# jhuldr/BrainFM

Measured on AMD Instinct MI355X. Metric: voxels/sec whole-volume multi-task inference, 256^3 tiled, higher is better.
Workload: dtype f16x3-split (fp32-grade); 1 GPU; 256^3 volume, reference tiling win160/stride80 -> 27 tiles, UNet3D f64 x6 levels, 9 heads (69 ch), fused tail + deformed atlas + on-device stitch of 17 keys; stitched_keys=17, mfma_passes=3, submission=hipGraph replay per tile shape, parallelism=tiles sharded over 1 rank(s), gather to rank 0, tiles_in_flight_per_gpu=2

## Files before the change

brainfm_amd/_lib.py:

```python
import ctypes as C
import os

_HERE = os.path.dirname(os.path.abspath(__file__))
LIB_PATH = os.path.join(_HERE, "libbrainfm_hip.so")

ERR = {0: "BFM_OK", -1: "BFM_E_ARG", -2: "BFM_E_SHAPE", -3: "BFM_E_WORKSPACE", -4: "BFM_E_LAUNCH"}

ROLE_PLAIN, ROLE_CT, ROLE_BIAS_LOG, ROLE_SEG, ROLE_DIST, ROLE_SR, ROLE_PATHOL = range(7)
(EW_EXP, EW_AFFINE, EW_CLAMP, EW_CLAMP_MIN, EW_GAMMA, EW_SIGMOID, EW_DIV, EW_NONZERO, EW_SUB_DIV, EW_GE,
 EW_NAN_TO_NUM) = range(11)
(EW_ADD, EW_MUL, EW_MUL_EXP, EW_AXPY_CLAMP0, EW_AXPY, EW_DIV2, EW_ZERO_WHERE_ZERO) = range(7)


class BfmError(RuntimeError):
    pass


class Upsample(C.Structure):
    _fields_ = [("d", C.c_int), ("h", C.c_int), ("w", C.c_int),
                ("mapD", C.c_void_p), ("mapH", C.c_void_p), ("mapW", C.c_void_p),
                ("repD", C.c_void_p), ("repH", C.c_void_p), ("repW", C.c_void_p)]


CLASS_STATS_BLOCKS = 1024
# ... 45 lines not shown
                ("D", C.c_void_p * 6), ("G", C.c_void_p * 3), ("divV", C.c_void_p)]


class AgeParams(C.Structure):
    _fields_ = [(n, C.c_void_p) for n in ("c1w", "c1b", "c2w", "c2b", "l1w", "l1b", "l2w", "l2b", "l3w", "l3b")]


class AgeGrads(C.Structure):
    _fields_ = [(n, C.c_void_p) for n in ("c1w", "c1b", "c2w", "c2b", "l1w", "l1b", "l2w", "l2b", "l3w", "l3b")]


GATHER_MAX_JOBS = 12


VERTEX_SETS_MAX = 4


class VertexSet(C.Structure):
    _fields_ = [("V", C.c_void_p), ("n", C.c_int64)]


class GatherJob(C.Structure):
    _fields_ = [("src", C.c_void_p), ("out", C.c_void_p), ("mean", C.c_float), ("scale", C.c_float), ("pre", C.c_int),
                ("default_max", C.c_int), ("post_div", C.c_float), ("clamp", C.c_int), ("clamp_lo", C.c_float),
                ("clamp_hi", C.c_float), ("sign", C.c_float), ("want_minmax", C.c_int)]


_P = C.c_void_p
_I = C.c_int
_F = C.c_float
_L = C.c_int64
_Z = C.c_size_t
_UP = C.POINTER(Upsample)

SIGNATURES = {
    "bfm_version": (C.c_char_p, []),
    "bfm_gn_stats_workspace": (_Z, [_I, _I, _I, _I, _I, _UP]),
    "bfm_gn_stats": (_I, [_P, _I, _P, _I, _I, _I, _I, _UP, _P, _P, _I, _F, _P, _P, _P, _P, _Z, _P]),
    "bfm_pack_conv_weights_direct": (_I, [_P, _I, _I, _P, _P]),
    "bfm_pack_conv_weights_mfma_bytes": (_Z, [_I, _I]),
    "bfm_pack_conv_weights_mfma": (_I, [_P, _I, _I, _F, _P, C.POINTER(_I), _P]),
    "bfm_pack_conv_weights_mfma16_bytes": (_Z, [_I, _I]),
    "bfm_pack_conv_weights_mfma16": (_I, [_P, _I, _I, _F, _P, C.POINTER(_I), _P]),
    "bfm_conv3x3x3_direct": (_I, [_P, _I, _P, _I, _I, _I, _I, _UP, _P, _P, _P, _I, _F, _P, _P]),
    "bfm_pack_conv_weights_upfold_bytes": (C.c_size_t, [_I, _I, _I]),
    "bfm_pack_conv_weights_upfold": (_I, [_P, _I, _I, _I, _F, _I, _P, _P, _P]),
    "bfm_conv3x3x3_upfold": (_I, [_P, _I, _I, _I, _I, _P, _P, _P, _I, _P, _I, _I, _I, _P, _P]),
    "bfm_conv3x3x3_upfold_workspace": (_Z, [_I, _I, _I, _I, _I]),
    "bfm_conv3x3x3_upfold_ex": (_I, [_P, _I, _I, _I, _I, _P, _P, _P, _I, _P, _I, _I, _I, _P, _P, _Z, _P]),
    "bfm_conv3x3x3_upfold_batch_workspace": (_Z, [_I, _I, _I, _I, _I, _I]),
    "bfm_conv3x3x3_upfold_batch": (_I, [_P, _I, _I, _I, _I, _I, _P, _P, _P, _I, _P, _I, _I, _I, _P, _P, _Z, _I, _P]),
    "bfm_conv3x3x3_tap_batch_workspace": (_Z, [_I, _I, _I, _I]),
    "bfm_conv3x3x3_tap_batch": (_I, [_P, _I, _I, _I, _P, _P, _P, _I, _P, _I, _I, _I, _I, _I, _P, _Z, _I, _P]),
    "bfm_tap_sum_rows": (_I, [_I, _I]),
    "bfm_tap_sum_batch": (_I, [_P, _I, _I, _I, _I, _P, _I, _F, _I, _I, _P, _P, _P]),
    "bfm_moment_rows_bytes": (_Z, [_I, _I]),
    "bfm_conv3x3x3_mfma_rows": (_I, [_I, _I, _I, _I, _I, C.POINTER(_I)]),
    "bfm_conv3x3x3_mfma_ex": (_I, [_P, _I, _P, _I, _I, _I, _I, _UP, _P, _P, _P, _I, _P, _I, _I, _F, _I,
                                   C.POINTER(_I), _P, _P, _Z, _P, _P]),
    "bfm_conv3x3x3_mfma_batch_workspace": (_Z, [_I, _I, _I, _I, _I, _I, _I]),
    "bfm_conv3x3x3_mfma_batch": (_I, [_P, _I, _P, _I, _I, _I, _I, _I, _UP, _P, _P, _P, _I, _P, _I, _I, _F, _I,
                                      C.POINTER(_I), _P, _P, _Z, _P, _I, _P]),
    "bfm_gn_stats_batch_workspace": (_Z, [_I, _I, _I, _I, _I, _I, _UP]),
    "bfm_gn_stats_batch": (_I, [_P, _I, _P, _I, _I, _I, _I, _I, _UP, _P, _P, _I, _F, _P, _P, _P, _P, _Z, _P]),
    "bfm_gn_stats_rows_batch": (_I, [_P, _I, _I, _P, _I, _I, C.c_double, _L, _I, _P, _P, _I, _F, _P, _P, _P, _P]),
    "bfm_conv3x3x3_stem_rows": (_I, [_I, _I, _I]),
    "bfm_conv3x3x3_stem_ex": (_I, [_P, _I, _I, _I, _P, _P, _P, _P, _I, _F, _P, _P, _P]),
    "bfm_conv3x3x3_stem_mc_ex": (_I, [_P, _I, _I, _I, _I, _P, _P, _P, _P, _I, _F, _P, _P, _P]),
    "bfm_gn_stats_rows_workspace": (_Z, [_I, _I, _I, _I]),
    "bfm_gn_stats_plan": (_I, [_I, _L, _I, C.POINTER(_I), C.POINTER(_I), C.POINTER(_L), C.POINTER(_I)]),
    "bfm_gn_stats_rows_route": (_I, [_I, _I, _I, _I, _I, _I]),
    "bfm_gn_stats_rows": (_I, [_P, _I, _I, _P, _I, _I, C.c_double, _L, _P, _P, _I, _F, _P, _P, _P, _P, _Z, _P, _P]),
    "bfm_gn_stats_rows_sliced": (_I, [_P, _I, _I, _I, _I, _P, _I, _I, _I, _I, C.c_double, _L, _P, _P, _I, _F, _P, _P, _P, _P, _Z,
                                      _P, _P]),
    "bfm_gn_stats_rows_train": (_I, [_P, _I, _I, _P, _I, _I, C.c_double, _L, _P, _P, _I, _F, _P, _P, _P, _P, _P, _P, _Z, _P, _P]),
    "bfm_crop3d": (_I, [_P, _I, _I, _I, _I, _I, _I, _I, _I, _I, _P, _P]),
    "bfm_pack_conv_weights_wino4_bytes": (_Z, [_I, _I, _I]),
    "bfm_pack_conv_weights_wino4": (_I, [_P, _I, _I, _F, _I, _P, C.POINTER(_I), _P]),
    "bfm_conv3x3x3_wino4_rows": (_I, [_I, _I, _I, _I]),
    "bfm_conv3x3x3_wino4_box": (_I, [_I, _I, _I, _I, _P]),
    "bfm_conv3x3x3_wino4_masked_workspace": (_Z, [_I, _I, _I, _I]),
    "bfm_conv3x3x3_wino4_uniform_scratch": (_Z, [_I]),
    "bfm_conv3x3x3_wino4_uniform": (_I, [_P, _I, _I, _I, _I, _P, _P, _P, _I, _P, _I, _I, _F, _I, _I, _P, _P, _P, _P, _P]),
    "bfm_conv3x3x3_wino4": (_I, [_P, _I, _I, _I, _I, _P, _P, _P, _I, _P, _I, _I, _F, _I, _I, _P, _P, _P]),
    "bfm_conv3x3x3_wino4_batch": (_I, [_P, _I, _I, _I, _I, _I, _P, _P, _P, _I, _P, _I, _I, _F, _I, _I, _P, _P, _I, _P]),
    "bfm_conv3x3x3_wino_b5_rows": (_I, [_I, _I, _I, _I]),
    "bfm_conv3x3x3_wino_b5_splitk": (_I, [_I, _I, _I, _I, _I]),
    "bfm_conv3x3x3_wino_b5_workspace": (_Z, [_I, _I, _I, _I, _I, _I]),
    "bfm_conv3x3x3_wino_b5_batch": (_I, [_P, _I, _I, _I, _I, _I, _P, _P, _P, _I, _P, _I, _I, _F, _I, _I, _P, _P, _I, _P, _Z,
                                         _P]),
    "bfm_conv3x3x3_wino4_masked": (_I, [_P, _I, _I, _I, _I, _P, _P, _P, _I, _P, _I, _I, _F, _I, _I, _P, _P, _P, _Z, _P]),
    "bfm_permute_flip3d": (_I, [_P, _I, _I, _I, C.POINTER(_I), C.POINTER(_I), _P, _P]),
    "bfm_bbox_nonzero": (_I, [_P, _I, _I, _I, _F, _P, _P]),
    "bfm_mean_lastdim": (_I, [_P, _L, _I, _P, _P]),
    "bfm_pack_conv_weights_wino_bytes": (_Z, [_I, _I, _I]),
    "bfm_pack_conv_weights_wino": (_I, [_P, _I, _I, _F, _I, _P, C.POINTER(_I), _P]),
    "bfm_bspline3_prefilter_axis": (_I, [_P, _I, _I, _I, _I, _I, _F, _F, _P, _F, _F, _F, _I, _P]),
    "bfm_bspline3_resample_axis": (_I, [_P, _I, _I, _I, _I, _P, _I, _I, _P, _P]),
    "bfm_conv3x3x3_wino_rows": (_I, [_I, _I, _I, _I]),
    "bfm_conv3x3x3_wino_ex": (_I, [_P, _I, _I, _I, _I, _P, _P, _P, _I, _P, _I, _I, _F, _I, _I, _P, _P, _P]),
    "bfm_conv3x3x3_wino_box": (_I, [_I, _I, _I, _I, _P]),
    "bfm_uniform_boxes": (_I, [_P, _I, _I, _I, _I, _I, _P, _P]),
    "bfm_uniform_boxes_level": (_I, [_P, _I, _I, _I, _I, _I, _I, _P, _P]),
    "bfm_uniform_boxes_levels": (_I, [_P, _I, _I, _I, _I, C.POINTER(_I), C.POINTER(_I), _I, C.POINTER(_P), _P, _P]),
    "bfm_uniform_boxes_bytes": (_Z, [_I, _I, _I, _I]),
    "bfm_conv3x3x3_wino_uniform_scratch": (_Z, [_I]),
    "bfm_conv3x3x3_wino_uniform": (_I, [_P, _I, _I, _I, _I, _P, _P, _P, _I, _P, _I, _I, _F, _I, _I, _P, _P, _P, _P, _P]),
    "bfm_conv3x3x3_wino_pool_ok": (_I, [_I, _I, _I, _I]),
    "bfm_conv3x3x3_wino_pool": (_I, [_P, _I, _I, _I, _I, _P, _P, _P, _I, _P, _I, _I, _F, _I, _I, _P, _P, _P, _P, _P]),
    "bfm_conv3x3x3_wino_uniform_pool": (_I, [_P, _I, _I, _I, _I, _P, _P, _P, _I, _P, _I, _I, _F, _I, _I, _P, _P, _P, _P, _P, _P,
                                             _P]),
    "bfm_conv3x3x3_wino_masked_workspace": (_Z, [_I, _I, _I, _I]),
    "bfm_conv3x3x3_wino_masked": (_I, [_P, _I, _I, _I, _I, _P, _P, _P, _I, _P, _I, _I, _F, _I, _I, _P, _P, _P, _Z, _P]),
    "bfm_maxpool2_rows": (_I, [_I, _I, _I, _I]),
    "bfm_maxpool2_ex": (_I, [_P, _I, _I, _I, _I, _P, _P, _P]),
    "bfm_maxpool2_batch_rows": (_I, [_I, _I, _I, _I]),
    "bfm_maxpool2_batch": (_I, [_P, _I, _I, _I, _I, _I, _P, _P, _P]),
    "bfm_grid_push3d_linear": (_I, [_P, _I, _I, _I, _I, _I, _P, _I, _I, _I, _I, C.POINTER(_I), _I, _P, _P]),
    "bfm_grid_grad3d_linear": (_I, [_P, _I, _I, _I, _I, _I, _P, _I, _I, _I, _I, C.POINTER(_I), _I, _P, _P]),
    "bfm_grid_pull3d_spline": (_I, [_P, _I, _I, _I, _I, _I, _P, _I, _I, _I, _I, C.POINTER(_I), C.POINTER(_I), _I, _P, _P]),
    "bfm_grid_push3d_spline": (_I, [_P, _I, _I, _I, _I, _I, _P, _I, _I, _I, _I, C.POINTER(_I), C.POINTER(_I), _I, _P, _P]),
    "bfm_grid_grad3d_spline": (_I, [_P, _I, _I, _I, _I, _I, _P, _I, _I, _I, _I, C.POINTER(_I), C.POINTER(_I), _I, _P, _P]),
    "bfm_grid_pull2d_spline": (_I, [_P, _I, _I, _I, _I, _P, _I, _I, _I, C.POINTER(_I), C.POINTER(_I), _I, _P, _P]),
    "bfm_grid_push2d_spline": (_I, [_P, _I, _I, _I, _I, _P, _I, _I, _I, C.POINTER(_I), C.POINTER(_I), _I, _P, _P]),
    "bfm_grid_grad2d_spline": (_I, [_P, _I, _I, _I, _I, _P, _I, _I, _I, C.POINTER(_I), C.POINTER(_I), _I, _P, _P]),
    "bfm_grid_hess3d": (_I, [_P, _I, _I, _I, _I, _I, _P, _I, _I, _I, _I, C.POINTER(_I), C.POINTER(_I), _I, _P, _P, _P]),
    "bfm_grid_pushgrad3d": (_I, [_P, _I, _I, _I, _I, _I, _P, _I, _I, _I, _I, C.POINTER(_I), C.POINTER(_I), _I, _P, _P]),
    "bfm_grid_push_fixed_bits": (_I, [_L, C.POINTER(_I), _I, _I]),
    "bfm_grid_push_fixed_workspace": (_Z, [_I, _I, _L]),
    "bfm_grid_push3d_spline_fixed": (_I, [_P, _I, _I, _I, _I, _I, _P, _I, _I, _I, _I, C.POINTER(_I), C.POINTER(_I), _I, _P,
                                          _P, _Z, _P]),
    "bfm_grid_push2d_spline_fixed": (_I, [_P, _I, _I, _I, _I, _P, _I, _I, _I, C.POINTER(_I), C.POINTER(_I), _I, _P, _P, _Z,
                                          _P]),
    "bfm_grid_push3d_linear_fixed": (_I, [_P, _I, _I, _I, _I, _I, _P, _I, _I, _I, _I, C.POINTER(_I), _I, _P, _P, _Z, _P]),
    "bfm_grid_pushgrad3d_fixed": (_I, [_P, _I, _I, _I, _I, _I, _P, _I, _I, _I, _I, C.POINTER(_I), C.POINTER(_I), _I, _P, _P,
                                       _Z, _P]),
    "bfm_spline_axis_table_workspace": (_Z, [_I, _I, _I]),
    "bfm_spline_axis_table": (_I, [_P, _I, _I, _I, _I, _I, _I, _I, _P, _P, _P, _P, _Z, _P]),
    "bfm_spline_axis_pass": (_I, [_P, _L, _I, _I, _I, _I, _P, _P, _P, _I, _P, _P]),
    "bfm_label_pull3d": (_I, [_P, _I, _I, _I, _I, _I, _I, _P, _I, _I, _I, _I, C.POINTER(_I), C.POINTER(_I), _I, _I, _P, _P]),
    "bfm_affine_grid3d": (_I, [_P, _I, _L, _I, _I, _I, _P, _P]),
    "bfm_add_identity_grid3d": (_I, [_P, _I, _L, _I, _I, _I, _P]),
    "bfm_affine_pull_multi": (_I, [_P, _L, _I, _I, _I, _I, C.POINTER(C.c_double), C.POINTER(_I), _I, _I, _I, _P, _P]),
    "bfm_affine_pull_argmax": (_I, [_P, _I, _I, _I, _I, _P, C.POINTER(C.c_double), _I, _I, _I, _I, _P, _P, _P]),
    "bfm_affine_pull_route": (_I, [_I]),
    "bfm_gn_stats_train": (_I, [_P, _I, _P, _I, _I, _I, _I, _UP, _P, _P, _I, _F, _P, _P, _P, _P, _P, _P, _Z, _P]),
    "bfm_lrelu_bwd": (_I, [_P, _P, _L, _F, _P, _P]),
    "bfm_lrelu_bwd_ex": (_I, [_P, _P, _L, _F, _P, _P, _P]),
    "bfm_conv3x3x3_wgrad_workspace": (_Z, [_I, _I, _I, _I, _I]),
    "bfm_conv3x3x3_wgrad_plan": (_I, [_I, _I, _I, _I, _I, _I, _I, _I, _I, _I, _I, C.POINTER(C.c_int64), C.POINTER(_Z)]),
    "bfm_conv3x3x3_wgrad": (_I, [_P, _I, _P, _I, _P, _I, _I, _I, _I, _UP, _P, _P, _P, _P, _Z, _P]),
    "bfm_conv3x3x3_wgrad_ex": (_I, [_P, _I, _P, _I, _P, _I, _I, _I, _I, _UP, _P, _P, _P, _P, _I, _I, _P, _P, _Z, _P]),
    "bfm_stem_mc_bwd_workspace": (_Z, [_I, _I, _I, _I, _I]),
    "bfm_stem_mc_bwd": (_I, [_P, _I, _P, _I, _I, _I, _I, _P, _P, _P, _P, _P, _P, _P, _P, _P, _Z, _P]),
    "bfm_stem_mc_dgrad": (_I, [_P, _I, _P, _I, _I, _I, _I, _P, _P, _P, _P, _P, _P, _I, _P, _P, _P, _P, _L, _L, _P]),
    "bfm_mask_chain_bwd": (_I, [_P, _L, _P, _P, _L, _P, _L, _L, _P]),
    "bfm_gn_bwd_workspace": (_Z, [_I, _I, _I, _I]),
    "bfm_gn_bwd": (_I, [_P, _P, _I, _P, _I, _I, _I, _I, _UP, _P, _P, _P, _P, _P, _P, _I, _P, _P, _P, _P, _P, _Z, _P]),
    "bfm_maxpool2_bwd": (_I, [_P, _P, _I, _I, _I, _I, _P, _P]),
    "bfm_transpose_mirror_weights": (_I, [_P, _I, _I, _I, _P, _P]),
    "bfm_loss_workspace": (_Z, [_I]),
    "bfm_loss_l1_multi_workspace": (_Z, []),
    "bfm_loss_l1_multi": (_I, [_P, _L, _L, _I, _L, _I, _P, _P, _P, _P, _P, _P, _P, _P, _P, _P, _Z, _P]),
    "bfm_loss_grad_l1_multi": (_I, [_P, _L, _L, _I, _I, _P, _P, _P, _P, _I, _I, _I, _P, _P, _P, _Z, _P]),
    "bfm_loss_seg": (_I, [_P, _L, _L, _I, _I, _I, _P, _P, _P, _L, _F, _F, _P, _P, _P, _P, _Z, _P]),
    "bfm_loss_pathol_workspace": (_Z, []),
    "bfm_loss_pathol": (_I, [_P, _L, _L, _P, _L, _F, _F, _P, _P, _P, _P, _Z, _P]),
    "bfm_loss_reg_workspace": (_Z, [_I, _I, _I, _I]),
    "bfm_loss_reg_smooth": (_I, [_P, _L, _L, _L, _I, _I, _I, _I, _F, _P, _P, _P, _Z, _P]),
    "bfm_loss_reg_hessian": (_I, [_P, _L, _L, _L, _I, _I, _I, _I, _F, _P, _P, _P, _Z, _P]),
    "bfm_loss_contrastive_workspace": (_Z, []),
    "bfm_loss_contrastive": (_I, [_P, _P, _I, _L, _I, _F, _F, _F, _F, _F, _P, _P, _P, _P, _P, _P, _Z, _P]),
    "bfm_head_bwd_workspace": (_Z, [_I, _I, _L]),
    "bfm_head_bwd": (_I, [_P, _P, _P, _I, _I, _L, _P, _P, _P, _P, _Z, _P]),
    "bfm_tail_raw_rows": (_I, [_P, _L, C.POINTER(TailDesc), _P, _P, _L, _P]),
    "bfm_head_bwd_rows": (_I, [_P, _L, _P, _P, _I, _I, _L, _P, _P, _P, _P, _Z, _P]),
    "bfm_head_wgrad_workspace": (_Z, [_I, _I, _L]),
    "bfm_head_wgrad": (_I, [_P, _P, _I, _I, _L, _P, _P, _P, _Z, _P]),
    "bfm_head_wgrad_rows": (_I, [_P, _L, _P, _I, _I, _L, _P, _P, _P, _Z, _P]),
    "bfm_normalize_bwd": (_I, [_P, _P, _I, _L, _F, _P, _P]),
    "bfm_adamw_step": (_I, [_P, _P, _P, _P, _L, _F, _F, _F, _F, _F, _I, _F, _P]),
    "bfm_grad_sumsq": (_I, [_P, _L, _P, _P, _P, _Z, _P]),
    "bfm_grad_sumsq_multi": (_I, [_P, _I, _P, _I, _L, _P, _P, _P, _Z, _P]),
    "bfm_adamw_step_multi": (_I, [_P, _I, _P, _I, _L, _F, _F, _F, _F, _F, _P]),
    "bfm_adam_step_multi": (_I, [_P, _I, _P, _I, _L, _F, C.c_double, C.c_double, _F, _F, _P]),
    "bfm_sgd_step_multi": (_I, [_P, _I, _P, _I, _L, _F, _F, _F, _P]),
    "bfm_lars_sums_multi": (_I, [_P, _I, _P, _I, _L, _P, _P, _P, _Z, _P]),
    "bfm_lars_step_multi": (_I, [_P, _I, _P, _I, _L, _F, _F, _P]),
# ... 184 lines not shown
```

brainfm_amd/csrc/conv3d_wino.hip:

```cpp
#include "wino_shared.h"
#include <cstdlib>
#include <type_traits>

namespace {

typedef _Float16 half8 __attribute__((ext_vector_type(8)));
typedef _Float16 half4 __attribute__((ext_vector_type(4)));
typedef float floatx16 __attribute__((ext_vector_type(16)));

constexpr int KC = 16;
constexpr int NTHR = 256;
constexpr int MLD = 33;

struct WinoParams {
    const float* A;
    int CA, D, H, W;
    const float *scale, *shift, *bound;
    int G;
    const uint4* wp;
    int wexp, Cout;
    float slope;
    float* out;
    int accum;
    int TD, TH, TW, HT, PW;
// ... 399 lines not shown
#pragma unroll
                for (int r = 0; r < 8; ++r) {
                    S += ls[r * 32 + tid]; Q += lq[r * 32 + tid];
                    MN = fminf(MN, lmn[r * 32 + tid]); MX = fmaxf(MX, lmx[r * 32 + tid]);
                }
                const size_t o = (size_t)mt * p.Cout + nt * 64 + nb * 32 + tid;
                p.rsum[o] = S; p.rsq[o] = Q; p.rmn[o] = MN; p.rmx[o] = MX;
            }
        }
        if constexpr (POOL == 1) {
            if (interior) {
            const int POOL_OFF = UNI ? 6144 : 0;
            float* xs = reinterpret_cast<float*>(lds + POOL_OFF);
            __syncthreads();
#pragma unroll
            for (int k = 0; k < 8; ++k) xs[k * NTHR + tid] = pm[k];
            __syncthreads();
            const int hb = (row0 >> 1) & 1;
            const int te = tid & ~64, to = tid | 64;
            float ps = 0.f, pq = 0.f, pmn = INFINITY, pmx = -INFINITY;
            const int H2 = p.H >> 1, W2 = p.W >> 1;
            float* pb = p.pool_out + nt * 64 + nb * 32 + col +
                        (((int64_t)(z0 >> 1) * H2 + (y0 >> 1) + (row0 >> 2) + 2 * hb) * W2 + (x0 >> 1) + (row0 & 1)) * p.Cout;
            const unsigned zstep = (unsigned)(H2 * W2 * p.Cout);
            const float* xe = xs + hb * 4 * NTHR + te;
            const float* xo = xs + hb * 4 * NTHR + to;
#pragma unroll
            for (int dp = 0; dp < 4; ++dp) {
                const float mv = pool_max(pool_max(-INFINITY, xe[dp * NTHR]), xo[dp * NTHR]);
                pb[dp * zstep] = mv;
                ps += mv; pq = fmaf(mv, mv, pq); pmn = fminf(pmn, mv); pmx = fmaxf(pmx, mv);
            }
            if (p.prsum != nullptr) {
                double* ls2 = reinterpret_cast<double*>(lds + POOL_OFF + 8 * NTHR * sizeof(float));
                double* lq2 = ls2 + 256;
                float* lmn2 = reinterpret_cast<float*>(lq2 + 256);
                float* lmx2 = lmn2 + 256;
                ls2[row0 * 32 + col] = (double)ps; lq2[row0 * 32 + col] = (double)pq;
                lmn2[row0 * 32 + col] = pmn; lmx2[row0 * 32 + col] = pmx;
                __syncthreads();
                if (tid < 32) {
                    double S = 0.0, Q = 0.0;
                    float MN = INFINITY, MX = -INFINITY;
#pragma unroll
                    for (int r = 0; r < 8; ++r) {
                        S += ls2[r * 32 + tid]; Q += lq2[r * 32 + tid];
                        MN = fminf(MN, lmn2[r * 32 + tid]); MX = fmaxf(MX, lmx2[r * 32 + tid]);
                    }
                    const size_t o = (size_t)mt * p.Cout + nt * 64 + nb * 32 + tid;
                    p.prsum[o] = S; p.prsq[o] = Q; p.prmn[o] = MN; p.prmx[o] = MX;
                }
            }
            }
        }
    }
}

template <int NPASS>
__global__ void __launch_bounds__(NTHR, 2) conv_wino(const WinoParams p) { conv_wino_body<NPASS, 0>(p); }
template <int NPASS>
__global__ void __launch_bounds__(NTHR, 2) conv_wino_pool(const WinoParams p) { conv_wino_body<NPASS, 0, 1>(p); }
template <int NPASS>
__global__ void __launch_bounds__(NTHR, 2) conv_wino_rest_pool(const WinoParams p) { conv_wino_body<NPASS, 2, 1>(p); }
template <int NPASS>
__global__ void __launch_bounds__(NTHR, 2) conv_wino_uniform_pool(const WinoParams p) { conv_wino_body<NPASS, 3, 1>(p); }

template <int NPASS>
__global__ void __launch_bounds__(NTHR, 2) conv_wino_masked(const WinoParams p) { conv_wino_body<NPASS, 1>(p); }

template <int NPASS>
__global__ void __launch_bounds__(NTHR, 2) conv_wino_rest(const WinoParams p) { conv_wino_body<NPASS, 2>(p); }
template <int NPASS>
__global__ void __launch_bounds__(NTHR, 2) conv_wino_uniform(const WinoParams p) { conv_wino_body<NPASS, 3>(p); }

struct FillParams {
    float* out;
    int D, H, W, Cout, NT;
    int TD, TH, TW, nTy, nTx;
    int tw_shift, thw_shift;
    const unsigned char* flags;
    const int* first;
    const int* list;
    const int* list_n;
    double *rsum, *rsq;
    float *rmn, *rmx;
    float* pool_out;
    double *prsum, *prsq;
    float *prmn, *prmx;
};

__global__ void __launch_bounds__(NTHR) class_fill(const FillParams p) {
    const int bid = blockIdx.x;
    if (bid >= p.list_n[0] * p.NT) return;
    const int tid = threadIdx.x;
    const int mt = p.list[bid / p.NT], nt = bid % p.NT;
    const int rp = p.first[p.flags[mt] - 1];
    const int z0 = (mt / (p.nTx * p.nTy)) * p.TD, y0 = ((mt / p.nTx) % p.nTy) * p.TH, x0 = (mt % p.nTx) * p.TW;
    const int rz0 = (rp / (p.nTx * p.nTy)) * p.TD, ry0 = ((rp / p.nTx) % p.nTy) * p.TH, rx0 = (rp % p.nTx) * p.TW;
    const int c4 = tid & 15;
    {
        const size_t dbase = (((size_t)z0 * p.H + y0) * p.W + x0) * p.Cout + nt * 64 + c4 * 4;
        const size_t sbase = (((size_t)rz0 * p.H + ry0) * p.W + rx0) * p.Cout + nt * 64 + c4 * 4;
        for (int r = 0; r < 4; ++r) {
            float4 v[4];
            size_t off[4];
            bool in[4];
#pragma unroll
            for (int k = 0; k < 4; ++k) {
                const int vox = (r * 4 + k) * 16 + (tid >> 4);
                const int w = vox & (p.TW - 1), h = (vox >> p.tw_shift) & (p.TH - 1), d = vox >> p.thw_shift;
                in[k] = z0 + d < p.D && y0 + h < p.H && x0 + w < p.W;
                off[k] = (((size_t)d * p.H + h) * p.W + w) * p.Cout;
                v[k] = make_float4(0.f, 0.f, 0.f, 0.f);
                if (in[k]) v[k] = *reinterpret_cast<const float4*>(p.out + sbase + off[k]);
            }
#pragma unroll
            for (int k = 0; k < 4; ++k)
                if (in[k]) *reinterpret_cast<float4*>(p.out + dbase + off[k]) = v[k];
        }
    }
    if (p.pool_out != nullptr) {
        const int H2 = p.H >> 1, W2 = p.W >> 1;
        const size_t dbase = (((size_t)(z0 >> 1) * H2 + (y0 >> 1)) * W2 + (x0 >> 1)) * p.Cout + nt * 64 + c4 * 4;
        const size_t sbase = (((size_t)(rz0 >> 1) * H2 + (ry0 >> 1)) * W2 + (rx0 >> 1)) * p.Cout + nt * 64 + c4 * 4;
        const int vox = tid >> 4;
        const size_t off0 = (((size_t)(vox >> 3) * H2 + ((vox >> 1) & 3)) * W2 + (vox & 1)) * p.Cout;
        const size_t off1 = off0 + (size_t)2 * H2 * W2 * p.Cout;
        const float4 v0 = *reinterpret_cast<const float4*>(p.pool_out + sbase + off0);
        const float4 v1 = *reinterpret_cast<const float4*>(p.pool_out + sbase + off1);
        *reinterpret_cast<float4*>(p.pool_out + dbase + off0) = v0;
        *reinterpret_cast<float4*>(p.pool_out + dbase + off1) = v1;
    }
    if (tid < 64) {
        const size_t d = (size_t)mt * p.Cout + nt * 64 + tid, s = (size_t)rp * p.Cout + nt * 64 + tid;
        if (p.rsum != nullptr) { p.rsum[d] = p.rsum[s]; p.rsq[d] = p.rsq[s]; p.rmn[d] = p.rmn[s]; p.rmx[d] = p.rmx[s]; }
        if (p.prsum != nullptr) { p.prsum[d] = p.prsum[s]; p.prsq[d] = p.prsq[s]; p.prmn[d] = p.prmn[s]; p.prmx[d] = p.prmx[s]; }
    }
}

template <class Pred>
__device__ __forceinline__ int wino_compact(int nMt, Pred pred, int* __restrict__ list, int* sh) {
    const int tid = threadIdx.x, lane = tid & 63, wv = tid >> 6;
    if (tid == 0) sh[16] = 0;
    __syncthreads();
    for (int b0 = 0; b0 < nMt; b0 += 1024) {
        const int mt = b0 + tid;
        const bool keep = mt < nMt && pred(mt);
        const unsigned long long bal = __ballot(keep);
        const int before = __popcll(bal & ((1ull << lane) - 1ull));
        if (lane == 0) sh[wv] = __popcll(bal);
        __syncthreads();
        int off = sh[16];
        for (int w = 0; w < wv; ++w) off += sh[w];
        if (keep) list[off + before] = mt;
        __syncthreads();
        if (tid == 0) {
            int t = 0;
            for (int w = 0; w < 16; ++w) t += sh[w];
            sh[16] += t;
        }
        __syncthreads();
    }
    return sh[16];
}

__global__ void __launch_bounds__(256) wino_box_active_kernel(const float* __restrict__ img, int D, int H, int W, int TD,
                                                               int TH, int TW, int nTy, int nTx, int nMt,
                                                               unsigned char* __restrict__ act) {
    const int mt = blockIdx.x * 4 + (threadIdx.x >> 6), lane = threadIdx.x & 63;
    if (mt >= nMt) return;
    const int tx = mt % nTx, ty = (mt / nTx) % nTy, tz = mt / (nTx * nTy);
    const int z0 = tz * TD, y0 = ty * TH, x0 = tx * TW;
    const int thw = TH * TW;
    bool nz = false;
    for (int q = lane; q < TD * thw; q += 64) {
        const int d = q / thw, r = q - d * thw, h = r / TW, w = r - h * TW;
        const int gz = z0 + d, gy = y0 + h, gx = x0 + w;
        if (gz < D && gy < H && gx < W) nz = nz || img[((int64_t)gz * H + gy) * W + gx] != 0.f;
    }
    const bool any = __any(nz);
    if (lane == 0) act[mt] = any ? 1 : 0;
}

__global__ void __launch_bounds__(1024) wino_mask_list_kernel(const unsigned char* __restrict__ act, int nMt,
                                                               int* __restrict__ list, int* __restrict__ n_out) {
    __shared__ int sh[17];
    const int n = wino_compact(nMt, [&](int mt) { return act[mt] != 0; }, list, sh);
    if (threadIdx.x == 0) n_out[0] = n;
}

__global__ void __launch_bounds__(256) uniform_boxes_kernel(const float* __restrict__ img, int D, int H, int W, int TD, int TH,
                                                            int TW, int nTz, int nTy, int nTx, int L, int R,
                                                            unsigned char* __restrict__ flags) {
    const int mt = blockIdx.x;
    const int tx = mt % nTx, ty = (mt / nTx) % nTy, tz = mt / (nTx * nTy);
    const int z0 = max(((tz * TD) << L) - R, 0), y0 = max(((ty * TH) << L) - R, 0), x0 = max(((tx * TW) << L) - R, 0);
    const int z1 = min((((tz + 1) * TD) << L) + R, D), y1 = min((((ty + 1) * TH) << L) + R, H);
    const int x1 = min((((tx + 1) * TW) << L) + R, W);
    const int ed = z1 - z0, eh = y1 - y0, ew = x1 - x0;
    int bad = 0;
    const unsigned ref = __float_as_uint(img[((int64_t)z0 * H + y0) * W + x0]);
    for (int q = threadIdx.x; q < ed * eh * ew; q += 256) {
        const int w = q % ew, r = q / ew, h = r % eh, d = r / eh;
        bad |= __float_as_uint(img[((int64_t)(z0 + d) * H + (y0 + h)) * W + (x0 + w)]) != ref ? 1 : 0;
    }
    bad = __syncthreads_or(bad);
    if (threadIdx.x == 0) {
        const int cz = tz == 0 ? 0 : (tz == nTz - 1 ? 2 : 1), cy = ty == 0 ? 0 : (ty == nTy - 1 ? 2 : 1);
        const int cx = tx == 0 ? 0 : (tx == nTx - 1 ? 2 : 1);
        const int dl = (D >> L) << L, hl = (H >> L) << L, wl = (W >> L) << L;
        const bool far = (tz != nTz - 1 && ((((tz + 1) * TD) << L) + R > dl)) ||
                         (ty != nTy - 1 && ((((ty + 1) * TH) << L) + R > hl)) ||
                         (tx != nTx - 1 && ((((tx + 1) * TW) << L) + R > wl));
        flags[mt] = bad || far ? 0 : (unsigned char)(1 + 9 * cz + 3 * cy + cx);
    }
}

template <bool AGENT>
__device__ __forceinline__ void uniform_lists_body(const unsigned char* flags, int n, int* __restrict__ first,
                                                   int* __restrict__ cnt, int* __restrict__ rest, int* __restrict__ uni,
                                                   int* sh, int* fst) {
    auto flag = [&](int i) -> int {
        if constexpr (AGENT) return __hip_atomic_load(flags + i, __ATOMIC_RELAXED, __HIP_MEMORY_SCOPE_AGENT);
        else return flags[i];
    };
    if (threadIdx.x < 27) fst[threadIdx.x] = n;
    __syncthreads();
    for (int i = threadIdx.x; i < n; i += 1024) {
        const int f = flag(i);
        if (f != 0) atomicMin(&fst[f - 1], i);
    }
    __syncthreads();
    if (threadIdx.x < 27) first[threadIdx.x] = fst[threadIdx.x];
    const int n0 = wino_compact(n, [&](int mt) { const int f = flag(mt); return f == 0 || fst[f - 1] == mt; }, rest, sh);
    if (threadIdx.x == 0) cnt[0] = n0;
    __syncthreads();
    const int n1 = wino_compact(n, [&](int mt) { const int f = flag(mt); return f != 0 && fst[f - 1] != mt; }, uni, sh);
    if (threadIdx.x == 0) cnt[1] = n1;
}

__global__ void __launch_bounds__(1024) uniform_lists_kernel(const unsigned char* __restrict__ flags, int n,
                                                             int* __restrict__ first, int* __restrict__ cnt,
                                                             int* __restrict__ rest, int* __restrict__ uni) {
    __shared__ int sh[17];
    __shared__ int fst[27];
    uniform_lists_body<false>(flags, n, first, cnt, rest, uni, sh, fst);
}

constexpr int UL_MAX = 4;
constexpr int UL_LOADS = 8;
struct UniLevel {
    int TD, TH, TW, nTz, nTy, nTx, L, R;
    int n, per, wg0;
    unsigned char* flags;
    int* first;
};
struct UniLevels {
    const float* img;
    int D, H, W, nlev, nwg;
    int* ticket;
    UniLevel lv[UL_MAX];
};

__global__ void __launch_bounds__(1024) uniform_levels_kernel(const UniLevels p) {
    __shared__ int sh[17];
    __shared__ int fst[27];
    __shared__ int bad_w[16];
    __shared__ int is_last;
    const int tid = threadIdx.x, grp = tid >> 8, t = tid & 255;
    int li = 0;
    for (int i = 1; i < p.nlev; ++i)
        if ((int)blockIdx.x >= p.lv[i].wg0) li = i;
    const UniLevel& v = p.lv[li];
    const int D = p.D, H = p.H, W = p.W, L = v.L, R = v.R;
    const int box0 = ((int)blockIdx.x - v.wg0) * 4 * v.per;
    for (int r = 0; r < v.per; ++r) {
        const int mt = box0 + r * 4 + grp;
        const bool live = mt < v.n;
        int bad = 0;
        int tx = 0, ty = 0, tz = 0;
        if (live) {
            tx = mt % v.nTx; ty = (mt / v.nTx) % v.nTy; tz = mt / (v.nTx * v.nTy);
            const int z0 = max(((tz * v.TD) << L) - R, 0), y0 = max(((ty * v.TH) << L) - R, 0);
            const int x0 = max(((tx * v.TW) << L) - R, 0);
            const int z1 = min((((tz + 1) * v.TD) << L) + R, D), y1 = min((((ty + 1) * v.TH) << L) + R, H);
            const int x1 = min((((tx + 1) * v.TW) << L) + R, W);
            const int eh = y1 - y0, ew = x1 - x0, nq = (z1 - z0) * eh * ew;
            const unsigned ref = __float_as_uint(p.img[((int64_t)z0 * H + y0) * W + x0]);
            int w = t % ew, h = (t / ew) % eh, d = (t / ew) / eh;
            const int sw = 256 % ew, sh_ = (256 / ew) % eh, sd = (256 / ew) / eh;
            const float* const base = p.img + ((int64_t)z0 * H + y0) * W + x0;
            for (int qb = 0; qb < nq && !bad; qb += UL_LOADS * 256) {
                unsigned val[UL_LOADS];
#pragma unroll
                for (int k = 0; k < UL_LOADS; ++k) {
                    val[k] = ref;
                    if (qb + k * 256 + t < nq) val[k] = __float_as_uint(base[(unsigned)(d * H + h) * (unsigned)W + (unsigned)w]);
                    w += sw;
                    if (w >= ew) { w -= ew; ++h; }
                    h += sh_;
                    if (h >= eh) { h -= eh; ++d; }
                    d += sd;
                }
                int diff = 0;
#pragma unroll
                for (int k = 0; k < UL_LOADS; ++k) diff |= val[k] != ref ? 1 : 0;
                bad = __any(diff) ? 1 : 0;
            }
        }
        if ((tid & 63) == 0) bad_w[tid >> 6] = bad;
        __syncthreads();
        if (live && t == 0) {
            const int any_bad = bad_w[grp * 4] | bad_w[grp * 4 + 1] | bad_w[grp * 4 + 2] | bad_w[grp * 4 + 3];
            const int cz = tz == 0 ? 0 : (tz == v.nTz - 1 ? 2 : 1), cy = ty == 0 ? 0 : (ty == v.nTy - 1 ? 2 : 1);
            const int cx = tx == 0 ? 0 : (tx == v.nTx - 1 ? 2 : 1);
            const int dl = (D >> L) << L, hl = (H >> L) << L, wl = (W >> L) << L;
            const bool far = (tz != v.nTz - 1 && ((((tz + 1) * v.TD) << L) + R > dl)) ||
                             (ty != v.nTy - 1 && ((((ty + 1) * v.TH) << L) + R > hl)) ||
                             (tx != v.nTx - 1 && ((((tx + 1) * v.TW) << L) + R > wl));
            __hip_atomic_store(v.flags + mt, any_bad || far ? (unsigned char)0 : (unsigned char)(1 + 9 * cz + 3 * cy + cx),
                               __ATOMIC_RELAXED, __HIP_MEMORY_SCOPE_AGENT);
        }
        __syncthreads();
    }
    asm volatile("s_waitcnt vmcnt(0)" ::: "memory");
    __syncthreads();
    if (tid == 0) {
        const int got = __hip_atomic_fetch_add(p.ticket, 1, __ATOMIC_RELEASE, __HIP_MEMORY_SCOPE_AGENT);
        is_last = got == p.nwg - 1;
        if (is_last) __hip_atomic_store(p.ticket, 0, __ATOMIC_RELAXED, __HIP_MEMORY_SCOPE_AGENT);
    }
    __syncthreads();
    if (!is_last) return;
    __builtin_amdgcn_fence(__ATOMIC_ACQUIRE, "agent");
    for (int i = 0; i < p.nlev; ++i) {
        const int n = p.lv[i].n;
        int* const first = p.lv[i].first;
        uniform_lists_body<true>(p.lv[i].flags, n, first, first + 27, first + 29, first + 29 + n, sh, fst);
        __syncthreads();
    }
}

__global__ void pack_wino(const float* __restrict__ w, int Cin, int Cout, int wexp, int npl, uint4* __restrict__ out) {
    const int KCN = Cin / KC;
    const int nf = 2 * npl;
    const int64_t n = (int64_t)(Cout / 64) * 4 * KCN * 9 * nf * 64;
    const float s = ldexpf(1.0f, wexp);
    for (int64_t i = (int64_t)blockIdx.x * blockDim.x + threadIdx.x; i < n; i += (int64_t)gridDim.x * blockDim.x) {
        const int lane = (int)(i & 63);
        int64_t r = i >> 6;
        const int f = (int)(r % nf); r /= nf;
        const int t = (int)(r % 9); r /= 9;
        const int kc = (int)(r % KCN); r /= KCN;
        const int ps = (int)(r & 3); r >>= 2;
        const int ntile = (int)r;
        const int nb = f / npl, hl = f - nb * npl;
        const int co = ntile * 64 + nb * 32 + (lane & 31);
        const int ci0 = kc * KC + 8 * (lane >> 5);
        half8 v;
#pragma unroll
        for (int j = 0; j < 8; ++j) {
            const float* g = w + ((size_t)co * Cin + ci0 + j) * 27 + t * 3;
            const float g0 = g[0], g1 = g[1], g2 = g[2];
            const float u = ps == 0 ? g0 : ps == 1 ? ((g0 + g1) + g2) * 0.5f : ps == 2 ? ((g0 - g1) + g2) * 0.5f : g2;
            const float x = u * s;
            const _Float16 hh = (_Float16)x;
            v[j] = hl == 0 ? hh : (_Float16)(x - (float)hh);
        }
        out[i] = __builtin_bit_cast(uint4, v);
    }
}

constexpr int PKW_ROW = KC * 27 + 1;
__global__ void __launch_bounds__(256) pack_wino_tiled(const float* __restrict__ w, int Cin, int Cout, int wexp, int npl,
                                                       uint4* __restrict__ out) {
    extern __shared__ float pkw_lds[];
    const int KCN = Cin / KC;
    const int nf = 2 * npl;
    const int nb = blockIdx.x & 1;
    const int kc = (blockIdx.x >> 1) % KCN, ntile = (blockIdx.x >> 1) / KCN;
    const float s = ldexpf(1.0f, wexp);
    const float* src0 = w + ((int64_t)(ntile * 64 + nb * 32) * Cin + kc * KC) * 27;
    bfm_stage_rows<32, KC * 27, PKW_ROW, 256>(src0, (int64_t)Cin * 27, pkw_lds, 1.0f,
                                              ((reinterpret_cast<uintptr_t>(w) & 15) == 0) && (Cin & 3) == 0);
    __syncthreads();
    const int lane = threadIdx.x & 63, wave = threadIdx.x >> 6;
    for (int q = wave; q < 4 * 9; q += 4) {
        const int t = q % 9;
        const int ps = q / 9;
        const float* src = pkw_lds + (lane & 31) * PKW_ROW + (8 * (lane >> 5)) * 27 + t * 3;
        half8 vh, vl;
#pragma unroll
        for (int j = 0; j < 8; ++j) {
            const float g0 = src[j * 27], g1 = src[j * 27 + 1], g2 = src[j * 27 + 2];
            const float u = ps == 0 ? g0 : ps == 1 ? ((g0 + g1) + g2) * 0.5f : ps == 2 ? ((g0 - g1) + g2) * 0.5f : g2;
            const float x = u * s;
            const _Float16 hh = (_Float16)x;
            vh[j] = hh;
            vl[j] = (_Float16)(x - (float)hh);
        }
        uint4* dst = out + ((((int64_t)(ntile * 4 + ps) * KCN + kc) * 9 + t) * nf + nb * npl) * 64 + lane;
        dst[0] = __builtin_bit_cast(uint4, vh);
        if (npl == 2) dst[64] = __builtin_bit_cast(uint4, vl);
    }
}

int ilog2i(int v) { int r = 0; while ((1 << r) < v) ++r; return r; }

bool choose_box(int D, int H, int W, int npl, int& TD, int& TH, int& TW) {
    static const int opts[][3] = {{4, 4, 16}, {4, 8, 8}, {8, 4, 8}, {8, 8, 4}, {2, 4, 32}, {4, 2, 32}, {2, 8, 16},
                                  {8, 2, 16}, {16, 4, 4}, {4, 16, 4}};
    int64_t best = -1;
    for (auto& o : opts) {
        const int pw = o[2] / 2;
        const int64_t npos = (int64_t)(o[0] + 2) * (o[1] + 2) * pw;
        if (npos * 4 > 5 * NTHR) continue;
        const int64_t plane = ((npos * 16 + 255) / 256) * 256 + 16;
        if (8 * npl * plane > 80 * 1024) continue;
        int64_t cost = (int64_t)bfm_cdiv(D, o[0]) * bfm_cdiv(H, o[1]) * bfm_cdiv(W, o[2]);
        cost = cost * 1024 + npos;
        if (best < 0 || cost < best) { best = cost; TD = o[0]; TH = o[1]; TW = o[2]; }
// ... 10 lines not shown
    const MaskListBuf b{ws, (size_t)nMt};
    hipLaunchKernelGGL(wino_box_active_kernel, dim3((unsigned)bfm_cdiv(nMt, 4)), dim3(256), 0, bfm_s(stream), mask_img, D, H, W,
                       TD, TH, TW, nTy, nTx, nMt, b.act());
    hipLaunchKernelGGL(wino_mask_list_kernel, dim3(1), dim3(1024), 0, bfm_s(stream), b.act(), nMt, b.list(), b.count());
    return bfm_launch_status();
}

extern "C" size_t bfm_pack_conv_weights_wino_bytes(int Cin, int Cout, int passes) {
    if (Cin <= 0 || Cout <= 0 || Cin % KC || Cout % 64) return 0;
    const int npl = passes == 3 ? 2 : 1;
    return (size_t)(Cout / 64) * 4 * (Cin / KC) * 9 * 2 * npl * 64 * sizeof(uint4);
}

extern "C" int bfm_pack_conv_weights_wino(const float* w_oidhw, int Cin, int Cout, float wmax_abs_host, int passes,
                                          void* wpacked, int* wexp_host, bfm_stream_t stream) {
    if (!w_oidhw || !wpacked || !wexp_host || Cin <= 0 || Cout <= 0) return BFM_E_ARG;
    if (Cin % KC || Cout % 64 || (passes != 1 && passes != 3)) return BFM_E_SHAPE;
    int wexp = 0;
    if (wmax_abs_host > 0.f && wmax_abs_host < INFINITY) {
        int ex;
        (void)frexpf(2.f * wmax_abs_host, &ex);
        wexp = 14 - ex;
        wexp = wexp > 60 ? 60 : (wexp < -60 ? -60 : wexp);
    }
    *wexp_host = wexp;
    const int npl = passes == 3 ? 2 : 1;
    const int64_t nblk = (int64_t)(Cout / 64) * (Cin / KC) * 2;
    const size_t smem = (size_t)32 * PKW_ROW * sizeof(float);
    static bool attr = false;
    if (const int rc = bfm_raise_lds_limit(attr, {bfm_kernel(&pack_wino_tiled)}, (int)smem)) return rc;
    if (nblk <= 0x7fffffff) {
        hipLaunchKernelGGL(pack_wino_tiled, dim3((unsigned)nblk), dim3(256), smem, bfm_s(stream), w_oidhw, Cin, Cout, wexp, npl,
                           static_cast<uint4*>(wpacked));
    } else {
        const int64_t n = (nblk / 2) * 4 * 9 * 2 * npl * 64;
        int nb = (int)std::min<int64_t>(4096, bfm_cdiv64(n, 256));
        hipLaunchKernelGGL(pack_wino, dim3(nb), dim3(256), 0, bfm_s(stream), w_oidhw, Cin, Cout, wexp, npl,
                           static_cast<uint4*>(wpacked));
    }
    return bfm_launch_status();
}

extern "C" int bfm_conv3x3x3_wino_rows(int D, int H, int W, int passes) {
    int TD, TH, TW;
    if (D <= 0 || H <= 0 || W <= 0 || !choose_box(D, H, W, passes == 3 ? 2 : 1, TD, TH, TW)) return 0;
    return (int)bfm_box_count(D, H, W, TD, TH, TW);
}

extern "C" int bfm_conv3x3x3_wino_box(int D, int H, int W, int passes, int* box) {
    int TD, TH, TW;
    if (!box || D <= 0 || H <= 0 || W <= 0 || !choose_box(D, H, W, passes == 3 ? 2 : 1, TD, TH, TW)) return BFM_E_ARG;
    box[0] = TD; box[1] = TH; box[2] = TW;
    return BFM_OK;
}

static bool pool_ok_box(int TD, int TH, int TW, int D, int H, int W) {
    return TD == 8 && TH == 8 && TW == 4 && D % 8 == 0 && H % 8 == 0 && W % 4 == 0;
}

extern "C" int bfm_conv3x3x3_wino_pool_ok(int D, int H, int W, int passes) {
    int TD, TH, TW;
    if (D <= 0 || H <= 0 || W <= 0 || !choose_box(D, H, W, passes == 3 ? 2 : 1, TD, TH, TW)) return 0;
    return pool_ok_box(TD, TH, TW, D, H, W) ? 1 : 0;
}

extern "C" size_t bfm_uniform_boxes_bytes(int D, int H, int W, int passes) {
    int TD, TH, TW;
    if (D <= 0 || H <= 0 || W <= 0 || !choose_box(D, H, W, passes == 3 ? 2 : 1, TD, TH, TW)) return 0;
    return UniformFlagBuf::bytes((size_t)bfm_box_count(D, H, W, TD, TH, TW));
}

extern "C" int bfm_uniform_boxes_level(const float* image, int D, int H, int W, int level, int radius, int passes,
                                       unsigned char* flags, bfm_stream_t stream) {
    if (!image || !flags || D <= 0 || H <= 0 || W <= 0 || radius < 0 || radius > 64 || level < 0 || level > 4) return BFM_E_ARG;
    if (reinterpret_cast<uintptr_t>(flags) & 3) return BFM_E_ARG;
    const int d = D >> level, h = H >> level, w = W >> level;
    int TD, TH, TW;
    if (d <= 0 || h <= 0 || w <= 0 || !choose_box(d, h, w, passes == 3 ? 2 : 1, TD, TH, TW)) return BFM_E_SHAPE;
    const int nTz = bfm_cdiv(d, TD), nTy = bfm_cdiv(h, TH), nTx = bfm_cdiv(w, TW);
    const UniformFlagBuf fb{flags, (size_t)nTz * nTy * nTx};
    if ((TD << level) < radius || (TH << level) < radius || (TW << level) < radius) return BFM_E_SHAPE;
    hipLaunchKernelGGL(uniform_boxes_kernel, dim3((unsigned)fb.n), dim3(256), 0, bfm_s(stream), image, D, H, W, TD, TH, TW, nTz,
                       nTy, nTx, level, radius, flags);
    hipLaunchKernelGGL(uniform_lists_kernel, dim3(1), dim3(1024), 0, bfm_s(stream), flags, (int)fb.n, fb.first(), fb.counts(),
                       fb.rest_list(), fb.uniform_list());
    return bfm_launch_status();
}

extern "C" int bfm_uniform_boxes(const float* image, int D, int H, int W, int radius, int passes, unsigned char* flags,
                                 bfm_stream_t stream) {
    return bfm_uniform_boxes_level(image, D, H, W, 0, radius, passes, flags, stream);
}

extern "C" int bfm_uniform_boxes_levels(const float* image, int D, int H, int W, int nlevels, const int* levels,
                                        const int* radii, int passes, unsigned char* const* flags, int* ticket,
                                        bfm_stream_t stream) {
    if (!image || !levels || !radii || !flags || !ticket || D <= 0 || H <= 0 || W <= 0 || nlevels < 1 || nlevels > UL_MAX)
        return BFM_E_ARG;
    if (reinterpret_cast<uintptr_t>(ticket) & 3) return BFM_E_ARG;
    if ((int64_t)D * H * W > 0x7fffffffLL) return BFM_E_SHAPE;
    UniLevels p{};
    p.img = image; p.D = D; p.H = H; p.W = W; p.nlev = nlevels; p.ticket = ticket;
    int64_t nwg = 0;
    for (int i = 0; i < nlevels; ++i) {
        const int level = levels[i], radius = radii[i];
        if (!flags[i] || radius < 0 || radius > 64 || level < 0 || level > 4) return BFM_E_ARG;
        if (reinterpret_cast<uintptr_t>(flags[i]) & 3) return BFM_E_ARG;
        const int d = D >> level, h = H >> level, w = W >> level;
        UniLevel& v = p.lv[i];
        if (d <= 0 || h <= 0 || w <= 0 || !choose_box(d, h, w, passes == 3 ? 2 : 1, v.TD, v.TH, v.TW)) return BFM_E_SHAPE;
        if ((v.TD << level) < radius || (v.TH << level) < radius || (v.TW << level) < radius) return BFM_E_SHAPE;
        v.nTz = bfm_cdiv(d, v.TD); v.nTy = bfm_cdiv(h, v.TH); v.nTx = bfm_cdiv(w, v.TW);
        v.L = level; v.R = radius; v.flags = flags[i];
        const int64_t n = (int64_t)v.nTz * v.nTy * v.nTx;
        if (n > 0x7fffffff) return BFM_E_SHAPE;
        v.n = (int)n;
        v.first = UniformFlagBuf{flags[i], (size_t)n}.first();
        v.per = level == 0 ? 4 : 1;
        v.wg0 = (int)nwg;
        nwg += bfm_cdiv64(n, 4 * v.per);
    }
    p.nwg = (int)nwg;
    hipStream_t st = bfm_s(stream);
    hipLaunchKernelGGL(uniform_levels_kernel, dim3((unsigned)nwg), dim3(1024), 0, st, p);
    const int rc = bfm_launch_status();
    if (rc != BFM_OK) (void)hipMemsetAsync(ticket, 0, sizeof(int), st);
    return rc;
}

extern "C" size_t bfm_conv3x3x3_wino_uniform_scratch(int Cout) {
    return Cout > 0 && Cout % 64 == 0 ? (size_t)27 * (Cout / 64) * 2 * 16 * NTHR * 2 * sizeof(float) : 0;
}

extern "C" size_t bfm_conv3x3x3_wino_masked_workspace(int D, int H, int W, int passes) {
    int TD, TH, TW;
    if (D <= 0 || H <= 0 || W <= 0 || !choose_box(D, H, W, passes == 3 ? 2 : 1, TD, TH, TW)) return 0;
    return MaskListBuf::bytes((size_t)bfm_box_count(D, H, W, TD, TH, TW));
}

static int wino_launch(const WinoLaunch& a) {
    if (const int rc = bfm_wino_check(a, KC)) return rc;
    const int D = a.D, H = a.H, W = a.W, Cout = a.Cout, passes = a.passes;
    const int npl = passes == 3 ? 2 : 1;
    WinoParams p{};
    p.A = a.A; p.CA = a.CA; p.D = D; p.H = H; p.W = W;
    p.scale = a.scale; p.shift = a.shift; p.bound = a.bound; p.G = a.G;
    p.wp = static_cast<const uint4*>(a.wpacked);
    p.wexp = a.wexp; p.Cout = Cout; p.slope = a.slope; p.out = a.out; p.accum = a.flags & 1;
    p.mask_img = a.mask.img;
    p.uni_flags = a.uniform.flags;
    p.uni_acc = a.uniform.scratch;
    if (!choose_box(D, H, W, npl, p.TD, p.TH, p.TW)) return BFM_E_SHAPE;
    p.HT = p.TH + 2; p.PW = p.TW / 2;
    p.pw_shift = ilog2i(p.PW); p.thp_shift = ilog2i(p.TH * p.PW);
    const int nTz = bfm_cdiv(D, p.TD);
    p.nTy = bfm_cdiv(H, p.TH); p.nTx = bfm_cdiv(W, p.TW);
    p.nMt = nTz * p.nTy * p.nTx;
    const UniformFlagBuf fb{a.uniform.flags, (size_t)p.nMt};
    p.uni_first = fb.flags ? fb.first() : nullptr;
    p.NT = Cout / 64;
    p.KCN = a.CA / KC;
    p.npos_lds = (p.TD + 2) * p.HT * p.PW;
    p.plane_stride = ((p.npos_lds * 16 + 255) / 256) * 256 + 16;
    size_t smem = (size_t)8 * npl * p.plane_stride;
    const size_t epi = (size_t)4 * 128 * MLD * sizeof(float) + 6144;
    if (smem < epi) smem = epi;
    MomentRows rows, prows;
    if (a.moment_rows && !rows.carve(a.moment_rows, (size_t)p.nMt * Cout)) return BFM_E_ARG;
    rows.into(p);
    if (a.pool.out) {
        if (a.mask.img || !pool_ok_box(p.TD, p.TH, p.TW, D, H, W)) return BFM_E_SHAPE;
        if (reinterpret_cast<uintptr_t>(a.pool.out) & 15) return BFM_E_ARG;
        p.pool_out = a.pool.out;
        if (a.pool.rows && !prows.carve(a.pool.rows, (size_t)p.nMt * Cout)) return BFM_E_ARG;
        p.prsum = prows.rsum; p.prsq = prows.rsq; p.prmn = prows.rmn; p.prmx = prows.rmx;
    } else if (a.pool.rows) return BFM_E_ARG;
    if ((int64_t)p.nMt * p.NT > 0x7fffffff) return BFM_E_SHAPE;
    if (smem > 80 * 1024) return BFM_E_SHAPE;
    static bool attr_done = false;
    if (const int rc = bfm_raise_lds_limit(
            attr_done,
            {bfm_kernel(&conv_wino_pool<3>), bfm_kernel(&conv_wino_pool<1>), bfm_kernel(&conv_wino_rest_pool<3>),
             bfm_kernel(&conv_wino_rest_pool<1>), bfm_kernel(&conv_wino<3>), bfm_kernel(&conv_wino<1>),
             bfm_kernel(&conv_wino_masked<3>), bfm_kernel(&conv_wino_masked<1>), bfm_kernel(&conv_wino_uniform<3>),
             bfm_kernel(&conv_wino_uniform<1>), bfm_kernel(&conv_wino_rest<3>), bfm_kernel(&conv_wino_rest<1>)},
            80 * 1024))
        return rc;
    const dim3 grid((unsigned)(p.nMt * p.NT)), block(NTHR);
    hipStream_t st = bfm_s(a.stream);
    if (a.mask.img) {
        if (!a.mask.ws) return BFM_E_ARG;
        const MaskListBuf mb{a.mask.ws, (size_t)p.nMt};
        if (const int rc = bfm_wino_mask_list(a.mask.img, D, H, W, p.TD, p.TH, p.TW, p.nTy, p.nTx, p.nMt, a.mask.ws, a.stream))
            return rc;
        p.list = mb.list(); p.list_n = mb.count();
        bfm_launch_by_passes(passes, conv_wino_masked<3>, conv_wino_masked<1>, grid, block, smem, st, p);
        return bfm_launch_status();
    }
    if (fb.flags) {
        p.list = fb.rest_list(); p.list_n = fb.counts();
        if (a.pool.out) bfm_launch_by_passes(passes, conv_wino_rest_pool<3>, conv_wino_rest_pool<1>, grid, block, smem, st, p);
        else bfm_launch_by_passes(passes, conv_wino_rest<3>, conv_wino_rest<1>, grid, block, smem, st, p);
        p.list = fb.uniform_list(); p.list_n = fb.counts() + 1;
        if (!p.accum) {
            FillParams f{};
            f.out = p.out; f.D = D; f.H = H; f.W = W; f.Cout = Cout; f.NT = p.NT;
            f.TD = p.TD; f.TH = p.TH; f.TW = p.TW; f.nTy = p.nTy; f.nTx = p.nTx;
            f.tw_shift = ilog2i(p.TW); f.thw_shift = ilog2i(p.TH * p.TW);
            f.flags = fb.flags; f.first = fb.first(); f.list = p.list; f.list_n = p.list_n;
            f.rsum = p.rsum; f.rsq = p.rsq; f.rmn = p.rmn; f.rmx = p.rmx;
            f.pool_out = p.pool_out; f.prsum = p.prsum; f.prsq = p.prsq; f.prmn = p.prmn; f.prmx = p.prmx;
            hipLaunchKernelGGL(class_fill, grid, block, 0, st, f);
            return bfm_launch_status();
        }
        if (a.pool.out) bfm_launch_by_passes(passes, conv_wino_uniform_pool<3>, conv_wino_uniform_pool<1>, grid, block, 20480, st, p);
        else bfm_launch_by_passes(passes, conv_wino_uniform<3>, conv_wino_uniform<1>, grid, block, 6144, st, p);
        return bfm_launch_status();
    }
    if (a.pool.out) bfm_launch_by_passes(passes, conv_wino_pool<3>, conv_wino_pool<1>, grid, block, smem, st, p);
    else bfm_launch_by_passes(passes, conv_wino<3>, conv_wino<1>, grid, block, smem, st, p);
    return bfm_launch_status();
}

extern "C" int bfm_conv3x3x3_wino_ex(const float* A, int CA, int D, int H, int W, const float* scale,
                                     const float* shift, const float* bound, int G, const void* wpacked, int wexp,
                                     int Cout, float slope, int passes, int flags, float* out, void* moment_rows,
                                     bfm_stream_t stream) {
    return wino_launch({A, CA, D, H, W, scale, shift, bound, G, wpacked, wexp, Cout, slope, passes, flags, out, moment_rows, stream});
}

extern "C" int bfm_conv3x3x3_wino_pool(const float* A, int CA, int D, int H, int W, const float* scale, const float* shift,
                                       const float* bound, int G, const void* wpacked, int wexp, int Cout, float slope,
                                       int passes, int flags, float* out, void* moment_rows, float* pooled,
                                       void* pooled_rows, bfm_stream_t stream) {
    if (!pooled) return BFM_E_ARG;
    WinoLaunch a{A, CA, D, H, W, scale, shift, bound, G, wpacked, wexp, Cout, slope, passes, flags, out, moment_rows, stream};
    a.pool = {pooled, pooled_rows};
    return wino_launch(a);
}

extern "C" int bfm_conv3x3x3_wino_uniform(const float* A, int CA, int D, int H, int W, const float* scale,
                                          const float* shift, const float* bound, int G, const void* wpacked, int wexp,
                                          int Cout, float slope, int passes, int flags, float* out, void* moment_rows,
                                          const unsigned char* uniform_flags, void* scratch, bfm_stream_t stream) {
    if (!uniform_flags || !scratch || (flags & ~1)) return BFM_E_ARG;
    if ((reinterpret_cast<uintptr_t>(uniform_flags) & 3) || (reinterpret_cast<uintptr_t>(scratch) & 15)) return BFM_E_ARG;
    WinoLaunch a{A, CA, D, H, W, scale, shift, bound, G, wpacked, wexp, Cout, slope, passes, flags, out, moment_rows, stream};
    a.uniform = {uniform_flags, static_cast<float*>(scratch)};
    return wino_launch(a);
}

extern "C" int bfm_conv3x3x3_wino_uniform_pool(const float* A, int CA, int D, int H, int W, const float* scale,
                                               const float* shift, const float* bound, int G, const void* wpacked,
                                               int wexp, int Cout, float slope, int passes, int flags, float* out,
                                               void* moment_rows, const unsigned char* uniform_flags, void* scratch,
                                               float* pooled, void* pooled_rows, bfm_stream_t stream) {
    if (!uniform_flags || !scratch || !pooled || (flags & ~1)) return BFM_E_ARG;
    if ((reinterpret_cast<uintptr_t>(uniform_flags) & 3) || (reinterpret_cast<uintptr_t>(scratch) & 15)) return BFM_E_ARG;
    WinoLaunch a{A, CA, D, H, W, scale, shift, bound, G, wpacked, wexp, Cout, slope, passes, flags, out, moment_rows, stream};
    a.uniform = {uniform_flags, static_cast<float*>(scratch)};
    a.pool = {pooled, pooled_rows};
    return wino_launch(a);
}

extern "C" int bfm_conv3x3x3_wino_masked(const float* A, int CA, int D, int H, int W, const float* scale,
                                         const float* shift, const float* bound, int G, const void* wpacked, int wexp,
                                         int Cout, float slope, int passes, int flags, float* out,
                                         const float* mask_image, void* workspace, size_t workspace_bytes,
                                         bfm_stream_t stream) {
    if (!mask_image || (flags & ~1)) return BFM_E_ARG;
    if (!workspace || (reinterpret_cast<uintptr_t>(workspace) & 3) ||
        workspace_bytes < bfm_conv3x3x3_wino_masked_workspace(D, H, W, passes))
        return BFM_E_ARG;
    WinoLaunch a{A, CA, D, H, W, scale, shift, bound, G, wpacked, wexp, Cout, slope, passes, flags, out, nullptr, stream};
    a.mask = {mask_image, workspace};
    return wino_launch(a);
}
```

brainfm_amd/csrc/conv3d_wino4.hip:

```cpp
#include "wino_shared.h"
#include <cstdlib>
#include <type_traits>

namespace {

typedef _Float16 half8 __attribute__((ext_vector_type(8)));
typedef float floatx16 __attribute__((ext_vector_type(16)));
typedef __fp16 fp16x2_t __attribute__((ext_vector_type(2)));

constexpr int KC = 16;
constexpr int NPOS = 6;
constexpr int NTHR = 256;
constexpr int NRG = NTHR / 32;
constexpr int MLD = 33;

struct W4Params {
    const float* A;
    int CA, D, H, W;
    const float *scale, *shift, *bound;
    int G;
    const uint4* wp;
    int wexp, Cout;
    float slope;
    float* out;
    int accum;
    int TD, TH, TW, HT, QW;
    int qw_shift, thq_shift;
    int nTy, nTx, nMt, NT, KCN;
    int npos_lds, plane_stride;
    double *rsum, *rsq;
    float *rmn, *rmx;
    const int* list;
    const int* list_n;
    const unsigned char* uni_flags;
    float* uni_acc;
    int nMtS, saff;
    int64_t sA, sO;
    int dbg_sleep;
};

__device__ __forceinline__ void quad_coords(const W4Params& p, int q, int& d, int& h, int& j) {
    d = q >> p.thq_shift;
    const int rem = q & ((1 << p.thq_shift) - 1);
    h = rem >> p.qw_shift;
    j = rem & ((1 << p.qw_shift) - 1);
}

template <bool LO>
__device__ __forceinline__ void split_store4(const float (&t)[4], unsigned char* dp, int plane_stride) {
    const fp16x2_t h01 = __builtin_amdgcn_cvt_pkrtz(t[0], t[1]);
    const fp16x2_t h23 = __builtin_amdgcn_cvt_pkrtz(t[2], t[3]);
    uint2 hv;
    hv.x = __builtin_bit_cast(unsigned, h01);
    hv.y = __builtin_bit_cast(unsigned, h23);
    *reinterpret_cast<uint2*>(dp) = hv;
    if constexpr (LO) {
        const fp16x2_t l01 = __builtin_amdgcn_cvt_pkrtz(t[0] - (float)h01[0], t[1] - (float)h01[1]);
        const fp16x2_t l23 = __builtin_amdgcn_cvt_pkrtz(t[2] - (float)h23[0], t[3] - (float)h23[1]);
        uint2 lv;
        lv.x = __builtin_bit_cast(unsigned, l01);
        lv.y = __builtin_bit_cast(unsigned, l23);
        *reinterpret_cast<uint2*>(dp + plane_stride) = lv;
    }
}

template <int NPASS, int MODE, int ABL = 0>
__device__ __forceinline__ void conv_wino4_body(const W4Params& pin) {
    W4Params p = pin;
    constexpr bool LIST = MODE != 0;
    constexpr int NPL = (NPASS == 3) ? 2 : 1;
    constexpr int NF = 2 * NPL;
    extern __shared__ __attribute__((aligned(16))) unsigned char lds[];

    const int tid = threadIdx.x;
    const int lane = tid & 63;
    const int wv = __builtin_amdgcn_readfirstlane(tid >> 6);
    const int posA = wv;
    const int posB = 4 + (wv >> 1), mbB = wv & 1;
    const int l32 = lane & 31, khalf = lane >> 5;
    int item;
    {
        const int nblk = LIST ? p.list_n[0] * p.NT : p.nMt * p.NT;
        const int bid = blockIdx.x;
        if (LIST && bid >= nblk) return;
        const int q = nblk >> 3, r = nblk & 7;
        const int xcd = bid & 7, idx = bid >> 3;
        item = (xcd < r ? xcd * (q + 1) : r * (q + 1) + (xcd - r) * q) + idx;
    }
    const int mt = LIST ? p.list[item / p.NT] : item / p.NT;
    const int nt = item % p.NT;
    int mtl = mt;
    if (!LIST && p.nMtS > 0) {
        const int smp = mt / p.nMtS;
        mtl = mt - smp * p.nMtS;
        p.A += smp * p.sA;
        p.out += smp * p.sO;
        p.scale += smp * p.saff;
        p.shift += smp * p.saff;
        p.bound += smp * p.G;
    }
    const int tx = mtl % p.nTx;
    const int ty = (mtl / p.nTx) % p.nTy;
    const int tz = mtl / (p.nTx * p.nTy);
    const int z0 = tz * p.TD, y0 = ty * p.TH, x0 = tx * p.TW;

    float bmax = 0.f;
    for (int g = 0; g < p.G; ++g) bmax = fmaxf(bmax, p.bound[g]);
    int aexp = 0;
    if (bmax > 0.f && bmax < INFINITY) {
        int ex;
        (void)frexpf(bmax, &ex);
        aexp = 10 - ex;
        aexp = aexp > 60 ? 60 : (aexp < -60 ? -60 : aexp);
    }
    const float a_scale = ldexpf(1.0f, aexp);
    const float dq = ldexpf(1.0f, -(aexp + p.wexp));

    int a_off[3];
// ... 289 lines not shown
__global__ void __launch_bounds__(NTHR, 2) conv_wino4_masked(const W4Params p) { conv_wino4_body<NPASS, 1>(p); }

constexpr int DB_TD = 8, DB_TH = 8, DB_HT = 10, DB_NROW = 100;
constexpr int DB_PLANE = DB_NROW * 16;
constexpr int DB_RAWROW = 6 * 64;
constexpr int DB_RAW = DB_NROW * DB_RAWROW;
constexpr int DB_NDMA = DB_NROW / 2;
constexpr int DB_NDMA_WAVE = (DB_NDMA + 3) / 4;

template <bool LO>
__device__ __forceinline__ void split_store4_mix(const float (&t)[4], unsigned char* dp, int plane_stride) {
    const fp16x2_t h01 = __builtin_amdgcn_cvt_pkrtz(t[0], t[1]);
    const fp16x2_t h23 = __builtin_amdgcn_cvt_pkrtz(t[2], t[3]);
    uint2 hv;
    hv.x = __builtin_bit_cast(unsigned, h01);
    hv.y = __builtin_bit_cast(unsigned, h23);
    *reinterpret_cast<uint2*>(dp) = hv;
    if constexpr (LO) {
        uint2 lv;
        asm("v_fma_mixlo_f16 %0, %1, -1.0, %2 op_sel_hi:[1,0,0]" : "=v"(lv.x) : "v"(hv.x), "v"(t[0]));
        asm("v_fma_mixhi_f16 %0, %1, -1.0, %2 op_sel:[1,0,0] op_sel_hi:[1,0,0]" : "+v"(lv.x) : "v"(hv.x), "v"(t[1]));
        asm("v_fma_mixlo_f16 %0, %1, -1.0, %2 op_sel_hi:[1,0,0]" : "=v"(lv.y) : "v"(hv.y), "v"(t[2]));
        asm("v_fma_mixhi_f16 %0, %1, -1.0, %2 op_sel:[1,0,0] op_sel_hi:[1,0,0]" : "+v"(lv.y) : "v"(hv.y), "v"(t[3]));
        *reinterpret_cast<uint2*>(dp + plane_stride) = lv;
    }
}

template <int NPASS, int MODE, int ABL = 0>
__device__ __forceinline__ void conv_wino4d_body(const W4Params& pin) {
    W4Params p = pin;
    constexpr bool LIST = MODE != 0;
    constexpr bool UNI = MODE == 3;
    constexpr bool BY_FLAG = MODE == 2 || MODE == 3;
    constexpr int NPL = (NPASS == 3) ? 2 : 1;
    constexpr int NF = 2 * NPL;
    constexpr int NWF = 3 * NPL;
    constexpr int RAW_OFF = 2 * NPOS * NPL * DB_PLANE;
    extern __shared__ __attribute__((aligned(16))) unsigned char lds[];

    const int tid = threadIdx.x;
    const int lane = tid & 63;
    const int wv = __builtin_amdgcn_readfirstlane(tid >> 6);
    const int posA = wv;
    const int posB = 4 + (wv >> 1), nbB = wv & 1;
    const int l32 = lane & 31, khalf = lane >> 5;
#ifdef BFM_W4_ABLATE
    if (p.dbg_sleep > 0 && blockIdx.x < 512) {
        unsigned hwid;
        asm volatile("s_getreg_b32 %0, hwreg(HW_REG_HW_ID)" : "=s"(hwid));
        if (hwid & 1)
            for (int i = 0; i < p.dbg_sleep; ++i) __builtin_amdgcn_s_sleep(16);
    }
#endif
    int item;
    {
        const int nblk = LIST ? p.list_n[0] * p.NT : p.nMt * p.NT;
        const int bid = blockIdx.x;
        if (LIST && bid >= nblk) return;
        const int q = nblk >> 3, r = nblk & 7;
        const int xcd = bid & 7, idx = bid >> 3;
        item = (xcd < r ? xcd * (q + 1) : r * (q + 1) + (xcd - r) * q) + idx;
    }
    const int mt = LIST ? p.list[item / p.NT] : item / p.NT;
    const int nt = item % p.NT;
    int mtl = mt;
    if (!LIST && p.nMtS > 0) {
        const int smp = mt / p.nMtS;
        mtl = mt - smp * p.nMtS;
        p.A += smp * p.sA;
        p.out += smp * p.sO;
        p.scale += smp * p.saff;
        p.shift += smp * p.saff;
        p.bound += smp * p.G;
    }
    const int tx = mtl % p.nTx;
    const int ty = (mtl / p.nTx) % p.nTy;
    const int tz = mtl / (p.nTx * p.nTy);
    const int z0 = tz * DB_TD, y0 = ty * DB_TH, x0 = tx * 4;
    int cls = 0;
    if constexpr (BY_FLAG) cls = __builtin_amdgcn_readfirstlane((int)p.uni_flags[mt]);
    const bool rep = MODE == 2 && cls != 0;
    float4* const ybuf = BY_FLAG && cls ? reinterpret_cast<float4*>(p.uni_acc) + ((size_t)(cls - 1) * p.NT + nt) * (2 * 8 * NTHR) + tid
                                        : nullptr;

    float bmax = 0.f;
    for (int g = 0; g < p.G; ++g) bmax = fmaxf(bmax, p.bound[g]);
    int aexp = 0;
    if (bmax > 0.f && bmax < INFINITY) {
        int ex;
        (void)frexpf(bmax, &ex);
        aexp = 10 - ex;
        aexp = aexp > 60 ? 60 : (aexp < -60 ? -60 : aexp);
    }
    const float a_scale = ldexpf(1.0f, aexp);
    const float dq = ldexpf(1.0f, -(aexp + p.wexp));

    floatx16 acc[2][2];
    floatx16 accB[2];
    if constexpr (!UNI) {
    int a_off[4];
#pragma unroll
    for (int u = 0; u < 4; ++u) {
        const int pos = u < 2 ? posA : posB, mb = u & 1;
        const int pr = row_perm(l32);
        const int d = mb * 2 + (pr >> 4) + 4 * ((pr & 15) >> 3), h = pr & 7;
        a_off[u] = ((pos * 2 + khalf) * NPL) * DB_PLANE + (d * DB_HT + h) * 16;
    }

    const int q4 = tid & 3;
    int msk[2];
#pragma unroll
    for (int it = 0; it < 2; ++it) {
        const int r = (tid >> 2) + 64 * it;
        msk[it] = -1;
        if (r < DB_NROW) {
            const int hz = r / DB_HT, hy = r - hz * DB_HT;
            const int gz = z0 + hz - 1, gy = y0 + hy - 1;
            int m = 0;
            if (gz >= 0 && gz < p.D && gy >= 0 && gy < p.H) {
#pragma unroll
                for (int i = 0; i < 6; ++i)
                    if (x0 - 1 + i >= 0 && x0 - 1 + i < p.W) m |= 1 << i;
            }
            msk[it] = m;
        }
    }
    const bool inner = z0 >= 1 && z0 + DB_TD < p.D && y0 >= 1 && y0 + DB_TH < p.H && x0 >= 1 && x0 + 4 < p.W;
    const int st_plane = ((q4 >> 1) * NPL) * DB_PLANE + (q4 & 1) * 8;

    const int slot = lane >> 2;
    const int sb = slot >= 6 ? 1 : 0;
    int gxc = x0 + (slot - 6 * sb) - 1;
    gxc = gxc < 0 ? 0 : (gxc > p.W - 1 ? p.W - 1 : gxc);
    const int lane_el = gxc * p.CA + (lane & 3) * 4;
    const bool dma_lane = slot < 12;
    const unsigned raw_lds = (unsigned)(__UINTPTR_TYPE__)((__attribute__((address_space(3))) unsigned char*)(lds + RAW_OFF));
    const int zs = z0 > 0 ? z0 - 1 : 0;
    const float* slab = p.A + (int64_t)zs * p.H * p.W * p.CA;
    auto issue_dma = [&](int kc) __attribute__((always_inline)) {
        if constexpr ((ABL & 8) != 0) return;
        if (dma_lane) {
            int wvo = wv;
            asm volatile("" : "+s"(wvo));
#pragma unroll
            for (int n = 0; n < DB_NDMA_WAVE; ++n) {
                const int i = wvo + 4 * n;
                if (n < DB_NDMA_WAVE - 1 || i < DB_NDMA) {
                    const int hz = i / 5, hp = i - 5 * hz;
                    int gz = z0 + hz - 1;
                    gz = gz < 0 ? 0 : (gz > p.D - 1 ? p.D - 1 : gz);
                    int gy0 = y0 + 2 * hp - 1, gy1 = gy0 + 1;
                    gy0 = gy0 < 0 ? 0 : (gy0 > p.H - 1 ? p.H - 1 : gy0);
                    gy1 = gy1 > p.H - 1 ? p.H - 1 : gy1;
                    const unsigned ro0 = (unsigned)((((gz - zs) * p.H + gy0) * p.W) * p.CA);
                    const unsigned ro1 = (unsigned)((((gz - zs) * p.H + gy1) * p.W) * p.CA);
                    const unsigned vo = ((sb ? ro1 : ro0) + (unsigned)lane_el) * 4u;
                    const unsigned la = raw_lds + (unsigned)(i * (2 * DB_RAWROW));
                    asm volatile("s_mov_b32 m0, %2\n\ts_nop 0\n\tglobal_load_lds_dwordx4 %0, %1" ::"v"(vo), "s"(slab + kc * KC), "s"(la)
                                 : "memory");
                }
            }
        }
    };

#pragma unroll
    for (int u = 0; u < 2; ++u) {
// ... 142 lines not shown
    if constexpr ((ABL & 16) != 0) {
        float sm = 0.f;
#pragma unroll
        for (int u = 0; u < 2; ++u)
#pragma unroll
            for (int i = 0; i < 16; ++i) sm += acc[u][0][i] + acc[u][1][i] + accB[u][i];
        if (sm == 12345.678f) p.out[tid] = sm;
        return;
    }
    float* m = reinterpret_cast<float*>(lds);
    const int col = tid & 31, rg = tid >> 5;
    const bool interior = z0 + DB_TD <= p.D && y0 + DB_TH <= p.H && x0 + 4 <= p.W;
    int un[4];
#pragma unroll
    for (int c = 0; c < 4; ++c) un[c] = row_unperm(16 * (c >> 1) + 8 * (c & 1) + rg);
    const unsigned off_t = (unsigned)((rg * p.W) * p.Cout + col);
#pragma unroll
    for (int nb = 0; nb < 2; ++nb) {
        if constexpr (!UNI && (ABL & 256) == 0) {
        __syncthreads();
#pragma unroll
        for (int u = 0; u < 2; ++u) {
            float* mw = m + (posA * 64 + u * 32 + khalf * 4) * MLD + l32;
#pragma unroll
            for (int i = 0; i < 16; ++i)
                mw[((i >> 2) * 8 + (i & 3)) * MLD] = acc[u][nb][i];
        }
        if (nbB == nb) {
#pragma unroll
            for (int u = 0; u < 2; ++u) {
                float* mw = m + (posB * 64 + u * 32 + khalf * 4) * MLD + l32;
#pragma unroll
                for (int i = 0; i < 16; ++i)
                    mw[((i >> 2) * 8 + (i & 3)) * MLD] = accB[u][i];
            }
        }
        __syncthreads();
        } else if (nb == 1 && p.rsum != nullptr) __syncthreads();
        float fs = 0.f, fq = 0.f, fmn = INFINITY, fmx = -INFINITY;
        float* ob = p.out + nt * 64 + nb * 32 + ((int64_t)(z0 * p.H + y0) * p.W + x0) * p.Cout;
        if constexpr ((ABL & 512) != 0) ob = p.out + nt * 64 + nb * 32 + (mt & 127) * 16384;
        const float* mc = m + col;
        if (interior) {
            float prev[8][4];
            if (p.accum) {
#pragma unroll
                for (int it = 0; it < 8; ++it) {
                    const float* o = ob + (int64_t)it * p.H * p.W * p.Cout;
#pragma unroll
                    for (int k = 0; k < 4; ++k) prev[it][k] = o[off_t + (unsigned)(k * p.Cout)];
                }
            }
#pragma unroll
            for (int it = 0; it < 8; ++it) {
                float* o = ob + (int64_t)it * p.H * p.W * p.Cout;
                if constexpr ((ABL & 512) != 0) o = ob + it * 2048 - (int)off_t + (rg * 256 + col);
                float y[4];
                if constexpr (UNI) {
                    const float4 yy = ybuf[(nb * 8 + it) * NTHR];
                    y[0] = yy.x; y[1] = yy.y; y[2] = yy.z; y[3] = yy.w;
                } else {
                    const int qr = 32 * ((it & 3) >> 1) + un[2 * (it & 1) + (it >> 2)];
                    const float* mr = mc + qr * MLD;
                    float m0, m1, m2, m3, m4, m5;
                    if constexpr ((ABL & 256) != 0) {
                        m0 = acc[0][nb][it]; m1 = acc[1][nb][it]; m2 = accB[0][it]; m3 = accB[1][it];
                        m4 = acc[0][nb][it + 8]; m5 = acc[1][nb][it + 8];
                    } else {
                        m0 = mr[0 * 64 * MLD]; m1 = mr[1 * 64 * MLD]; m2 = mr[2 * 64 * MLD];
                        m3 = mr[3 * 64 * MLD]; m4 = mr[4 * 64 * MLD]; m5 = mr[5 * 64 * MLD];
                    }
                    const float s1 = m1 + m2, d1 = m1 - m2, s2 = m3 + m4, d2 = m3 - m4;
                    y[0] = ((m0 + s1) + s2) * dq;
                    y[1] = fmaf(2.f, d2, d1) * dq;
                    y[2] = fmaf(4.f, s2, s1) * dq;
                    y[3] = (fmaf(8.f, d2, d1) + m5) * dq;
                    if (MODE == 2 && rep) ybuf[(nb * 8 + it) * NTHR] = make_float4(y[0], y[1], y[2], y[3]);
                }
#pragma unroll
                for (int k = 0; k < 4; ++k) {
                    float r = y[k];
                    if (p.accum) r = r + prev[it][k];
                    r = r >= 0.f ? r : r * p.slope;
                    if constexpr ((ABL & 128) == 0) o[off_t + (unsigned)(k * p.Cout)] = r;
                    fs += r; fq = fmaf(r, r, fq); fmn = fminf(fmn, r); fmx = fmaxf(fmx, r);
                }
            }
            if constexpr ((ABL & 128) != 0) { if (fs == 12345.678f) p.out[tid] = fs + fq + fmn + fmx; }
        } else if (y0 + rg < p.H) {
#pragma unroll 2
            for (int it = 0; it < 8; ++it) {
                if (z0 + it >= p.D) break;
                float* o = ob + (int64_t)it * p.H * p.W * p.Cout;
                float y[4];
                if constexpr (UNI) {
                    const float4 yy = ybuf[(nb * 8 + it) * NTHR];
                    y[0] = yy.x; y[1] = yy.y; y[2] = yy.z; y[3] = yy.w;
                } else {
                    const int qr = 32 * ((it & 3) >> 1) + row_unperm(16 * (it & 1) + 8 * (it >> 2) + rg);
                    const float* mr = mc + qr * MLD;
                    const float m0 = mr[0 * 64 * MLD], m1 = mr[1 * 64 * MLD], m2 = mr[2 * 64 * MLD];
                    const float m3 = mr[3 * 64 * MLD], m4 = mr[4 * 64 * MLD], m5 = mr[5 * 64 * MLD];
                    const float s1 = m1 + m2, d1 = m1 - m2, s2 = m3 + m4, d2 = m3 - m4;
                    y[0] = ((m0 + s1) + s2) * dq;
                    y[1] = fmaf(2.f, d2, d1) * dq;
                    y[2] = fmaf(4.f, s2, s1) * dq;
                    y[3] = (fmaf(8.f, d2, d1) + m5) * dq;
                    if (MODE == 2 && rep) ybuf[(nb * 8 + it) * NTHR] = make_float4(y[0], y[1], y[2], y[3]);
                }
#pragma unroll
                for (int k = 0; k < 4; ++k) {
                    if (x0 + k < p.W) {
                        float r = y[k];
                        if (p.accum) r = r + o[off_t + (unsigned)(k * p.Cout)];
                        r = r >= 0.f ? r : r * p.slope;
                        o[off_t + (unsigned)(k * p.Cout)] = r;
                        fs += r; fq = fmaf(r, r, fq); fmn = fminf(fmn, r); fmx = fmaxf(fmx, r);
                    }
                }
            }
        }
        if (p.rsum != nullptr) {
            double* ls = reinterpret_cast<double*>(lds + (UNI ? (size_t)0 : (size_t)NPOS * 64 * MLD * sizeof(float)));
            double* lq = ls + NRG * 32;
            float* lmn = reinterpret_cast<float*>(lq + NRG * 32);
            float* lmx = lmn + NRG * 32;
            ls[rg * 32 + col] = (double)fs; lq[rg * 32 + col] = (double)fq;
            lmn[rg * 32 + col] = fmn; lmx[rg * 32 + col] = fmx;
            __syncthreads();
            if (tid < 32) {
                double Ssum = 0.0, Q = 0.0;
                float MN = INFINITY, MX = -INFINITY;
#pragma unroll
                for (int r = 0; r < NRG; ++r) {
                    Ssum += ls[r * 32 + tid]; Q += lq[r * 32 + tid];
                    MN = fminf(MN, lmn[r * 32 + tid]); MX = fmaxf(MX, lmx[r * 32 + tid]);
                }
                const size_t o = (size_t)mt * p.Cout + nt * 64 + nb * 32 + tid;
                p.rsum[o] = Ssum; p.rsq[o] = Q; p.rmn[o] = MN; p.rmx[o] = MX;
            }
        }
    }
}

template <int NPASS>
__global__ void __launch_bounds__(NTHR, 2) conv_wino4d(const W4Params p) { conv_wino4d_body<NPASS, 0>(p); }
template <int NPASS>
__global__ void __launch_bounds__(NTHR, 2) conv_wino4d_masked(const W4Params p) { conv_wino4d_body<NPASS, 1>(p); }
template <int NPASS>
__global__ void __launch_bounds__(NTHR, 2) conv_wino4d_rest(const W4Params p) { conv_wino4d_body<NPASS, 2>(p); }
template <int NPASS>
__global__ void __launch_bounds__(NTHR, 2) conv_wino4d_uniform(const W4Params p) { conv_wino4d_body<NPASS, 3>(p); }
#ifdef BFM_W4_ABLATE
template <int ABL>
__global__ void __launch_bounds__(NTHR, 2) conv_wino4d_abl(const W4Params p) { conv_wino4d_body<3, 0, ABL>(p); }
#endif

__global__ void pack_wino4(const float* __restrict__ w, int Cin, int Cout, int wexp, int npl, uint4* __restrict__ out) {
    const int KCN = Cin / KC;
    const int nf = 2 * npl;
    const int64_t n = (int64_t)(Cout / 64) * NPOS * KCN * 9 * nf * 64;
    const double s = ldexp(1.0, wexp);
    for (int64_t i = (int64_t)blockIdx.x * blockDim.x + threadIdx.x; i < n; i += (int64_t)gridDim.x * blockDim.x) {
        const int lane = (int)(i & 63);
        int64_t r = i >> 6;
        const int f = (int)(r % nf); r /= nf;
        const int t = (int)(r % 9); r /= 9;
        const int kc = (int)(r % KCN); r /= KCN;
        const int ps = (int)(r % NPOS); r /= NPOS;
        const int ntile = (int)r;
        const int nb = f / npl, hl = f - nb * npl;
        const int co = ntile * 64 + nb * 32 + (lane & 31);
        const int ci0 = kc * KC + 8 * (lane >> 5);
        half8 v;
#pragma unroll
        for (int j = 0; j < 8; ++j) {
            const float* g = w + ((size_t)co * Cin + ci0 + j) * 27 + t * 3;
            const double g0 = g[0], g1 = g[1], g2 = g[2];
            const double u = ps == 0 ? g0 / 4.0
                           : ps == 1 ? -((g0 + g1) + g2) / 6.0
                           : ps == 2 ? -((g0 - g1) + g2) / 6.0
                           : ps == 3 ? g0 / 24.0 + g1 / 12.0 + g2 / 6.0
                           : ps == 4 ? g0 / 24.0 - g1 / 12.0 + g2 / 6.0
                                     : g2;
            const float x = (float)(u * s);
            const _Float16 hh = (_Float16)x;
            v[j] = hl == 0 ? hh : (_Float16)(x - (float)hh);
        }
        out[i] = __builtin_bit_cast(uint4, v);
    }
}

int ilog2i(int v) { int r = 0; while ((1 << r) < v) ++r; return r; }

bool choose_box4(int D, int H, int W, int npl, int& TD, int& TH, int& TW) {
    if (!bfm_wino_choose_box(D, H, W, npl, TD, TH, TW)) return false;
    if (TW % 4 || TD * TH * (TW / 4) != 64) return false;
    const int64_t npos = (int64_t)(TD + 2) * (TH + 2) * (TW / 4);
    if (npos * 4 > 3 * NTHR) return false;
// ... 21 lines not shown
    return (size_t)(Cout / 64) * NPOS * (Cin / KC) * 9 * 2 * npl * 64 * sizeof(uint4);
}

extern "C" int bfm_pack_conv_weights_wino4(const float* w_oidhw, int Cin, int Cout, float wmax_abs_host, int passes,
                                           void* wpacked, int* wexp_host, bfm_stream_t stream) {
    if (!w_oidhw || !wpacked || !wexp_host || Cin <= 0 || Cout <= 0) return BFM_E_ARG;
    if (Cin % KC || Cout % 64 || (passes != 1 && passes != 3)) return BFM_E_SHAPE;
    int wexp = 0;
    if (wmax_abs_host > 0.f && wmax_abs_host < INFINITY) {
        int ex;
        (void)frexpf(wmax_abs_host, &ex);
        wexp = 14 - ex;
        wexp = wexp > 60 ? 60 : (wexp < -60 ? -60 : wexp);
    }
    *wexp_host = wexp;
    const int npl = passes == 3 ? 2 : 1;
    const int64_t n = (int64_t)(Cout / 64) * NPOS * (Cin / KC) * 9 * 2 * npl * 64;
    const int nb = (int)std::min<int64_t>(8192, bfm_cdiv64(n, 256));
    hipLaunchKernelGGL(pack_wino4, dim3(nb), dim3(256), 0, bfm_s(stream), w_oidhw, Cin, Cout, wexp, npl,
                       static_cast<uint4*>(wpacked));
    return bfm_launch_status();
}

extern "C" int bfm_conv3x3x3_wino4_rows(int D, int H, int W, int passes) {
    int TD, TH, TW;
    if (D <= 0 || H <= 0 || W <= 0 || !choose_box_any(D, H, W, passes == 3 ? 2 : 1, TD, TH, TW)) return 0;
    return (int)bfm_box_count(D, H, W, TD, TH, TW);
}

extern "C" int bfm_conv3x3x3_wino4_box(int D, int H, int W, int passes, int* box) {
    int TD, TH, TW;
    if (!box || D <= 0 || H <= 0 || W <= 0 || !choose_box_any(D, H, W, passes == 3 ? 2 : 1, TD, TH, TW)) return BFM_E_ARG;
    box[0] = TD; box[1] = TH; box[2] = TW;
    return BFM_OK;
}

extern "C" size_t bfm_conv3x3x3_wino4_masked_workspace(int D, int H, int W, int passes) {
    const int n = bfm_conv3x3x3_wino4_rows(D, H, W, passes);
    if (n <= 0) return 0;
    return MaskListBuf::bytes((size_t)n);
}

static int w4_launch(const WinoLaunch& a) {
    if (const int rc = bfm_wino_check(a, KC)) return rc;
    const int D = a.D, H = a.H, W = a.W, CA = a.CA, Cout = a.Cout, passes = a.passes;
    const int S = a.batch.S, affine_stride = a.batch.affine_stride;
    const int npl = passes == 3 ? 2 : 1;
    W4Params p{};
    p.A = a.A; p.CA = CA; p.D = D; p.H = H; p.W = W;
    p.scale = a.scale; p.shift = a.shift; p.bound = a.bound; p.G = a.G;
    p.wp = static_cast<const uint4*>(a.wpacked);
    p.wexp = a.wexp; p.Cout = Cout; p.slope = a.slope; p.out = a.out; p.accum = a.flags & 1;
    if (!choose_box_any(D, H, W, npl, p.TD, p.TH, p.TW)) return BFM_E_SHAPE;
    const bool dma = use_dma_kernel(D, H, W);
    if (dma && (int64_t)(DB_TD + 2) * H * W * CA >= (int64_t)1 << 30) return BFM_E_SHAPE;
    p.HT = p.TH + 2; p.QW = p.TW / 4;
    p.qw_shift = ilog2i(p.QW); p.thq_shift = ilog2i(p.TH * p.QW);
    const int nTz = bfm_cdiv(D, p.TD);
    p.nTy = bfm_cdiv(H, p.TH); p.nTx = bfm_cdiv(W, p.TW);
    p.nMt = nTz * p.nTy * p.nTx;
    if (S > 1 || affine_stride > 0) {
        if (a.mask.img || S < 1 || (affine_stride != 0 && (affine_stride < CA || (affine_stride & 3)))) return BFM_E_ARG;
        p.nMtS = p.nMt;
        p.nMt = S * p.nMtS;
        p.saff = affine_stride > 0 ? affine_stride : CA;
        p.sA = (int64_t)D * H * W * CA;
        p.sO = (int64_t)D * H * W * Cout;
    }
    p.NT = Cout / 64;
    p.KCN = CA / KC;
    p.npos_lds = (p.TD + 2) * p.HT * p.QW;
    p.plane_stride = ((p.npos_lds * 16 + 255) / 256) * 256 + 16;
    size_t smem = dma ? (size_t)2 * NPOS * npl * DB_PLANE + DB_RAW : (size_t)2 * NPOS * npl * p.plane_stride;
    const size_t epi = (size_t)NPOS * 64 * MLD * sizeof(float) + (size_t)NRG * 32 * 24;
    if (smem < epi) smem = epi;
    if (smem > (dma ? 80u : 64u) * 1024) return BFM_E_SHAPE;
    const UniformFlagBuf fb{a.uniform.flags, (size_t)p.nMt};
    if (fb.flags) {
        int bd, bh, bw;
        if (!dma || a.mask.img || S > 1 || affine_stride > 0 || !a.uniform.scratch) return BFM_E_ARG;
        if (!bfm_wino_choose_box(D, H, W, npl, bd, bh, bw) || bd != p.TD || bh != p.TH || bw != p.TW) return BFM_E_SHAPE;
        p.uni_flags = fb.flags;
        p.uni_acc = a.uniform.scratch;
    }
    if (dma) {
        static bool attr = false;
        if (const int rc = bfm_raise_lds_limit(
                attr,
                {bfm_kernel(&conv_wino4d_rest<3>), bfm_kernel(&conv_wino4d_rest<1>), bfm_kernel(&conv_wino4d<3>),
                 bfm_kernel(&conv_wino4d<1>), bfm_kernel(&conv_wino4d_masked<3>), bfm_kernel(&conv_wino4d_masked<1>)},
                80 * 1024))
            return rc;
    }
    MomentRows rows;
    if (a.moment_rows && !rows.carve(a.moment_rows, (size_t)p.nMt * Cout)) return BFM_E_ARG;
    rows.into(p);
    if ((int64_t)p.nMt * p.NT > 0x7fffffff) return BFM_E_SHAPE;
    const dim3 grid((unsigned)(p.nMt * p.NT)), block(NTHR);
    hipStream_t st = bfm_s(a.stream);
    if (a.mask.img) {
        if (!a.mask.ws) return BFM_E_ARG;
        const MaskListBuf mb{a.mask.ws, (size_t)p.nMt};
        if (const int rc = bfm_wino_mask_list(a.mask.img, D, H, W, p.TD, p.TH, p.TW, p.nTy, p.nTx, p.nMt, a.mask.ws, a.stream))
            return rc;
        p.list = mb.list(); p.list_n = mb.count();
        if (dma) bfm_launch_by_passes(passes, conv_wino4d_masked<3>, conv_wino4d_masked<1>, grid, block, smem, st, p);
        else bfm_launch_by_passes(passes, conv_wino4_masked<3>, conv_wino4_masked<1>, grid, block, smem, st, p);
        return bfm_launch_status();
    }
    if (fb.flags) {
        p.list = fb.rest_list(); p.list_n = fb.counts();
        bfm_launch_by_passes(passes, conv_wino4d_rest<3>, conv_wino4d_rest<1>, grid, block, smem, st, p);
        p.list = fb.uniform_list(); p.list_n = fb.counts() + 1;
        bfm_launch_by_passes(passes, conv_wino4d_uniform<3>, conv_wino4d_uniform<1>, grid, block, 6144, st, p);
        return bfm_launch_status();
    }
#ifdef BFM_W4_ABLATE
    if (const char* e = getenv("BFM_W4_SLEEP")) p.dbg_sleep = atoi(e);
    if (const char* e = getenv("BFM_W4_ABL")) {
        const int abl = atoi(e);
        if (dma) {
#define W4D_ATTR(N) (void)hipFuncSetAttribute(reinterpret_cast<const void*>(&conv_wino4d_abl<N>), hipFuncAttributeMaxDynamicSharedMemorySize, 80 * 1024)
            W4D_ATTR(0); W4D_ATTR(1); W4D_ATTR(2); W4D_ATTR(3); W4D_ATTR(4); W4D_ATTR(8); W4D_ATTR(12); W4D_ATTR(15); W4D_ATTR(16); W4D_ATTR(31); W4D_ATTR(64); W4D_ATTR(28); W4D_ATTR(128); W4D_ATTR(256); W4D_ATTR(384); W4D_ATTR(512);
            switch (abl) {
#define W4D_CASE(N) case N: hipLaunchKernelGGL(conv_wino4d_abl<N>, grid, dim3(NTHR), smem, st, p); return bfm_launch_status()
                W4D_CASE(0); W4D_CASE(1); W4D_CASE(2); W4D_CASE(3); W4D_CASE(4); W4D_CASE(8); W4D_CASE(12); W4D_CASE(15); W4D_CASE(16); W4D_CASE(31); W4D_CASE(64); W4D_CASE(28); W4D_CASE(128); W4D_CASE(256); W4D_CASE(384); W4D_CASE(512);
                default: return BFM_E_ARG;
            }
        }
    }
#endif
    if (dma) bfm_launch_by_passes(passes, conv_wino4d<3>, conv_wino4d<1>, grid, block, smem, st, p);
    else bfm_launch_by_passes(passes, conv_wino4<3>, conv_wino4<1>, grid, block, smem, st, p);
    return bfm_launch_status();
}

extern "C" int bfm_conv3x3x3_wino4(const float* A, int CA, int D, int H, int W, const float* scale, const float* shift,
                                   const float* bound, int G, const void* wpacked, int wexp, int Cout, float slope,
                                   int passes, int flags, float* out, void* moment_rows, bfm_stream_t stream) {
    return w4_launch({A, CA, D, H, W, scale, shift, bound, G, wpacked, wexp, Cout, slope, passes, flags, out, moment_rows, stream});
}

extern "C" int bfm_conv3x3x3_wino4_batch(const float* A, int CA, int S, int D, int H, int W, const float* scale,
                                         const float* shift, const float* bound, int G, const void* wpacked, int wexp,
                                         int Cout, float slope, int passes, int flags, float* out, void* moment_rows,
                                         int affine_stride, bfm_stream_t stream) {
    if (S < 1) return BFM_E_ARG;
    WinoLaunch a{A, CA, D, H, W, scale, shift, bound, G, wpacked, wexp, Cout, slope, passes, flags, out, moment_rows, stream};
    a.batch = {S, affine_stride > 0 ? affine_stride : CA};
    return w4_launch(a);
}

extern "C" int bfm_conv3x3x3_wino4_masked(const float* A, int CA, int D, int H, int W, const float* scale, const float* shift,
                                          const float* bound, int G, const void* wpacked, int wexp, int Cout, float slope,
                                          int passes, int flags, float* out, const float* mask_image, void* workspace,
                                          size_t workspace_bytes, bfm_stream_t stream) {
    if (!mask_image || (flags & ~1)) return BFM_E_ARG;
    if (!workspace || (reinterpret_cast<uintptr_t>(workspace) & 3) ||
        workspace_bytes < bfm_conv3x3x3_wino4_masked_workspace(D, H, W, passes))
        return BFM_E_ARG;
    WinoLaunch a{A, CA, D, H, W, scale, shift, bound, G, wpacked, wexp, Cout, slope, passes, flags, out, nullptr, stream};
    a.mask = {mask_image, workspace};
    return w4_launch(a);
}

extern "C" size_t bfm_conv3x3x3_wino4_uniform_scratch(int Cout) {
    if (Cout <= 0 || Cout % 64) return 0;
    return (size_t)27 * (Cout / 64) * 2 * 8 * NTHR * sizeof(float4);
}

extern "C" int bfm_conv3x3x3_wino4_uniform(const float* A, int CA, int D, int H, int W, const float* scale, const float* shift,
                                           const float* bound, int G, const void* wpacked, int wexp, int Cout, float slope,
                                           int passes, int flags, float* out, void* moment_rows,
                                           const unsigned char* uniform_flags, void* scratch, bfm_stream_t stream) {
    if (!uniform_flags || !scratch || (reinterpret_cast<uintptr_t>(uniform_flags) & 3) || (reinterpret_cast<uintptr_t>(scratch) & 15))
        return BFM_E_ARG;
    WinoLaunch a{A, CA, D, H, W, scale, shift, bound, G, wpacked, wexp, Cout, slope, passes, flags, out, moment_rows, stream};
    a.uniform = {uniform_flags, static_cast<float*>(scratch)};
    return w4_launch(a);
}
```

brainfm_amd/csrc/wino_shared.h:

```cpp
#pragma once
#include "conv_shared.h"

bool bfm_wino_choose_box(int D, int H, int W, int npl, int& TD, int& TH, int& TW);

static inline size_t bfm_pad4(size_t n) { return (n + 3) & ~(size_t)3; }

struct MaskListBuf {
    void* ws;
    size_t n;
    static size_t bytes(size_t n) { return bfm_pad4(n) + 4 + n * 4; }
    unsigned char* act() const { return static_cast<unsigned char*>(ws); }
    int* count() const { return reinterpret_cast<int*>(act() + bfm_pad4(n)); }
    int* list() const { return count() + 1; }
};

struct UniformFlagBuf {
    const unsigned char* flags;
    size_t n;
    static size_t bytes(size_t n) { return bfm_pad4(n) + 27 * 4 + 2 * 4 + 2 * n * 4; }
    int* first() const { return reinterpret_cast<int*>(const_cast<unsigned char*>(flags) + bfm_pad4(n)); }
    int* counts() const { return first() + 27; }
    int* rest_list() const { return counts() + 2; }
    int* uniform_list() const { return rest_list() + n; }
};

int bfm_wino_mask_list(const float* mask_img, int D, int H, int W, int TD, int TH, int TW, int nTy, int nTx, int nMt, void* ws,
                       bfm_stream_t stream);

struct WinoLaunch {
    const float* A;
    int CA, D, H, W;
    const float *scale, *shift, *bound;
    int G;
    const void* wpacked;
    int wexp, Cout;
    float slope;
    int passes, flags;
    float* out;
    void* moment_rows;
    bfm_stream_t stream;
    struct { const float* img = nullptr; void* ws = nullptr; } mask;
    struct { const unsigned char* flags = nullptr; float* scratch = nullptr; } uniform;
    struct { float* out = nullptr; void* rows = nullptr; } pool;
    struct { int S = 1, affine_stride = 0; } batch;
};

static inline int bfm_wino_check(const WinoLaunch& a, int KC) {
    if (a.flags & ~1) return BFM_E_ARG;
    if (!a.A || a.CA <= 0 || a.D <= 0 || a.H <= 0 || a.W <= 0 || !a.scale || !a.shift || !a.bound || a.G <= 0 || !a.wpacked ||
        !a.out)
        return BFM_E_ARG;
    if (a.CA % KC || a.Cout % 64 || a.Cout <= 0) return BFM_E_SHAPE;
    if (a.passes != 1 && a.passes != 3) return BFM_E_ARG;
    if ((reinterpret_cast<uintptr_t>(a.A) & 15) || (reinterpret_cast<uintptr_t>(a.scale) & 15) ||
        (reinterpret_cast<uintptr_t>(a.shift) & 15) || (reinterpret_cast<uintptr_t>(a.wpacked) & 15) ||
        (reinterpret_cast<uintptr_t>(a.out) & 15))
        return BFM_E_ARG;
    if ((int64_t)a.D * a.H * a.W * a.CA > 0x7fffffffLL) return BFM_E_SHAPE;
    return BFM_OK;
}
```

brainfm_amd/engine.py:

```python
import ctypes as C
import os
from collections import OrderedDict, namedtuple

import numpy as np
import torch

from . import _lib as L

LABELS_LEFT = [0, 1, 2, 3, 4, 7, 8, 9, 10, 14, 15, 17, 31, 34, 36, 38, 40, 42]
LABELS_FULL = [0, 11, 12, 13, 16, 31, 32, 33, 34, 35, 36, 37, 38, 39, 40, 41, 42, 43, 44, 46,
               1, 2, 3, 4, 5, 6, 7, 8, 9, 10, 14, 15, 17, 47, 49, 51, 53, 55,
               18, 19, 20, 21, 22, 23, 24, 25, 26, 27, 28, 29, 30, 48, 50, 52, 54, 56]


def features_per_level(f_maps, num_levels):
    return [f_maps * 2 ** k for k in range(num_levels)]


def nearest_index_map(n_in, n_out):
    scale = np.float32(n_in) / np.float32(n_out)
    idx = np.floor(np.arange(n_out, dtype=np.float32) * scale).astype(np.int64)
    return np.minimum(idx, n_in - 1).astype(np.int32)


# ... 301 lines not shown
                    if wm is None:
                        wm = absmax(ly.w_raw)
                    visit(dg, wm)
                elif layout == "upfold":
                    jobs.append((ly, layout, absmax(ly.w_raw[:, ly.skip.cin:])))
                elif layout == "direct":
                    jobs.append((ly, layout, None))
                else:
                    if wm is None:
                        wm = absmax(ly.w_raw)
                    jobs.append((ly, layout, wm))
            ly.used = set()
            ly.wpacked, ly.kind = None, None
            if ly.skip is not None:
                ly.skip.w_raw.copy_(ly.w_raw[:, :ly.skip.cin])
                visit(ly.skip)

        for pair in (self.enc + self.dec if backbone else []) + [hidden]:
            for ly in pair:
                visit(ly)
        host = slots[:nslot[0]].cpu().tolist() if nslot[0] else []
        for ly, layout, m in jobs:
            wmax = host[m] if m is not None else None
            if layout == "upfold":
                self._make_upfold_pack(ly, ly.skip.cin, ly.cin - ly.skip.cin, wmax)
            else:
                self._make_pack(ly, layout, wmax)

    def _upsample_desc(self, lo, hi):
        key = (tuple(lo), tuple(hi))
        if key not in self._up_cache:
            maps = [nearest_index_map(lo[a], hi[a]) for a in range(3)]
            reps = [np.bincount(maps[a], minlength=lo[a]).astype(np.int32) for a in range(3)]
            dev = [torch.from_numpy(m).to(self.device) for m in maps + reps]
            up = L.Upsample(lo[0], lo[1], lo[2], *[t.data_ptr() for t in dev])
            self._up_cache[key] = (up, dev)
        return self._up_cache[key][0]

    def _tap_table(self, lo, hi):
        key = (tuple(lo), tuple(hi))
        if self._tap_cache is None:
            self._tap_cache = {}
        if key not in self._tap_cache:
            self._tap_cache[key] = torch.from_numpy(tap_row_table(key[0], key[1])).to(self.device)
        return self._tap_cache[key]

    def _workspace(self, nbytes):
        nbytes = max(int(nbytes), 256)
        if self._ws_lanes is None:
            self._ws_lanes, self._ws_retired = {}, []
        ws = self._ws_lanes.get(self.lane)
        if ws is None or ws.numel() < nbytes:
            if ws is not None:
                self._ws_retired.append(ws)
            ws = self._ws_lanes[self.lane] = torch.empty(int(nbytes * 1.25) + 1024, dtype=torch.uint8, device=self.device)
        return ws

    def _uf_ticket(self):
        t = self._uf_tickets
        if self.lane not in t:
            t[self.lane] = torch.zeros(1, dtype=torch.int32, device=self.device)
        return t[self.lane]

    def _gn_ticket(self):
        t = self._gn_tickets
        if self.lane not in t:
            t[self.lane] = torch.zeros(16, dtype=torch.int32, device=self.device)
        return t[self.lane]

    def _plan(self, cin, cout, dims, two_src=False, accum=False):
        key = (cin, cout, tuple(dims), bool(two_src), bool(accum))
        if key not in self._plan_cache:
            cfg = (C.c_int * 8)()
            L.check(self.lib.bfm_conv3x3x3_mfma_plan(cin, cout, dims[0], dims[1], dims[2], cfg), "mfma_plan")
            if two_src and cfg[6] in (3, 4):
                cfg[6] = 0
            if cfg[6] == 5:
                cfg[6] = 0
            self._plan_cache[key] = cfg
        return self._plan_cache[key]

    def _autotune(self, ly, key, launch, vers=None):
        cfg = self._plan_cache[key]
        if key in self._tuned or os.environ.get("BFM_CONV_VER") or os.environ.get("BFM_CONV_TUNE", "1") == "0":
            return cfg
        gkey = (torch.cuda.current_device(), getattr(self, "passes", None), key)
        if gkey not in _TUNE_CHOICES:
            saved = _tune_lookup(gkey[0], gkey[1], key)
            if saved is not None and not (key[3] and saved in (3, 4)) and (vers is None or saved in vers):
                _TUNE_CHOICES[gkey] = int(saved)
        if gkey in _TUNE_CHOICES and (vers is None or _TUNE_CHOICES[gkey] in vers or (_TUNE_CHOICES[gkey] == 4 and 3 in vers)):
            c = _TUNE_CHOICES[gkey]
            if vers is None or c in vers:
                cfg[6] = c
                self._tuned.add(key)
                return cfg
            narrowed = (C.c_int * 8)(*list(cfg))
            narrowed[6] = 3
            return narrowed
        best, best_ms = cfg[6], None
        single = (0, 1, 2, 3, 4) if os.environ.get("BFM_CONV_TUNE", "1") == "retune" else (0, 1, 2, 3)
        if hasattr(self, "enc") and self._needs_f23(ly):
            single = (0, 1, 2, 3)
        for ver in (vers if vers is not None else ((0, 1, 2) if key[3] else single)):
            if ver == 4 and 4 not in single and cfg[6] != 4:
                continue
            trial = (C.c_int * 8)(*list(cfg))
            trial[6] = ver
            try:
                self._pack(ly, True, ver)
                launch(trial)
                ms = None
                for _ in range(2):
                    ev = [torch.cuda.Event(enable_timing=True) for _ in range(2)]
                    ev[0].record()
                    launch(trial)
                    launch(trial)
                    launch(trial)
                    ev[1].record()
                    ev[1].synchronize()
                    t = ev[0].elapsed_time(ev[1])
                    ms = t if ms is None else min(ms, t)
            except L.BfmError:
                continue
            if ver == 4:
                ms = ms / 0.97
            if ver == 5:
                ms = ms / 0.97
            if best_ms is None or ms < best_ms:
                best, best_ms = ver, ms
        cfg[6] = best
        self._tuned.add(key)
        _TUNE_CHOICES[gkey] = best
        _tune_store(gkey[0], gkey[1], key, best)
        return cfg

    def conv_choices(self):
        dev, ps = torch.cuda.current_device(), getattr(self, "passes", None)
        return {k[2]: v for k, v in _TUNE_CHOICES.items() if k[0] == dev and k[1] == ps}

    def adopt_conv_choices(self, table):
        dev, ps = torch.cuda.current_device(), getattr(self, "passes", None)
        changed = False
        for key, ver in table.items():
            _TUNE_CHOICES[(dev, ps, key)] = ver
            if key in self._tuned and self._plan_cache[key][6] != ver:
                self._plan_cache[key][6] = ver
                changed = True
        return changed

    def _gn_stats(self, ly, A, ca, B, cb, dims, lo_dims, upp, scale, shift, bound, ws_min):
        D, H, W = dims
        st = L.stream_ptr()
        ra = getattr(A, "_bfm_rows", None) if self.fuse_stats else None
        rb = getattr(B, "_bfm_rows", None) if (self.fuse_stats and B is not None) else None
        if self.tape is not None and ((ra is not None and len(ra) > 2) or (rb is not None and len(rb) > 2)):
            ra = rb = None
        exact2 = B is None or tuple(dims) == tuple(2 * v for v in lo_dims)
        mean = rstd = None
        if self.tape is not None:
            mean = torch.empty(ly.groups, dtype=torch.float32, device=self.device)
            rstd = torch.empty(ly.groups, dtype=torch.float32, device=self.device)
            self._last_moments = (mean, rstd)
        if ra is not None and (B is None or (rb is not None and exact2)):
            need = self.lib.bfm_gn_stats_rows_workspace(ra[1], ca, rb[1] if rb is not None else 0, cb)
            ws = self._workspace(max(need, ws_min))
            if (len(ra) > 2 or (rb is not None and len(rb) > 2)) and self.tape is None:
                ta, fa = (ra[2], ra[3]) if len(ra) > 2 else (ra[1], 0)
                tb, fb = ((rb[2], rb[3]) if len(rb) > 2 else (rb[1], 0)) if rb is not None else (0, 0)
                L.check(self.lib.bfm_gn_stats_rows_sliced(L.ptr(ra[0]), ta, fa, ra[1], ca,
                                                          L.ptr(rb[0]) if rb is not None else None, tb, fb,
                                                          rb[1] if rb is not None else 0, cb, 8.0, D * H * W, L.ptr(ly.gamma),
                                                          L.ptr(ly.beta), ly.groups, self.eps, L.ptr(scale), L.ptr(shift),
                                                          L.ptr(bound), L.ptr(ws), ws.numel(),
                                                          L.ptr(self._gn_ticket()) if self.gn_one_launch else None, st),
                        "gn_stats_rows(slice) " + ly.name)
                return ws
            L.check(self.lib.bfm_gn_stats_rows_train(L.ptr(ra[0]), ra[1], ca, L.ptr(rb[0]) if rb is not None else None,
                                                     rb[1] if rb is not None else 0, cb, 8.0, D * H * W, L.ptr(ly.gamma),
                                                     L.ptr(ly.beta), ly.groups, self.eps, L.ptr(scale), L.ptr(shift),
                                                     L.ptr(bound), L.ptr(mean), L.ptr(rstd), L.ptr(ws), ws.numel(),
                                                     L.ptr(self._gn_ticket()) if self.gn_one_launch else None, st),
                    "gn_stats_rows " + ly.name)
            return ws
        wsb = self.lib.bfm_gn_stats_workspace(ca, cb, D, H, W, upp)
        ws = self._workspace(max(wsb, ws_min))
        L.check(self.lib.bfm_gn_stats_train(L.ptr(A), ca, L.ptr(B), cb, D, H, W, upp, L.ptr(ly.gamma), L.ptr(ly.beta),
                                            ly.groups, self.eps, L.ptr(scale), L.ptr(shift), L.ptr(bound), L.ptr(mean),
                                            L.ptr(rstd), L.ptr(ws), ws.numel(), st), "gn_stats " + ly.name)
        return ws

    def _record(self, ly, A, B, dims, lo_dims, scale, shift, bound, out):
        if self.tape is not None:
            mean, rstd = self._last_moments
            self.tape.append(dict(ly=ly, A=A, B=B, dims=tuple(dims), lo_dims=tuple(lo_dims) if lo_dims is not None else None,
                                  scale=scale, shift=shift, bound=bound, mean=mean, rstd=rstd, out=out))

    def _conv_launch(self, ly, A, ca, B, cb, dims, upp, scale, shift, bound, groups, cfg, out, ws, rows=None, slope=None,
                     mask_img=None, uni_flags=None, pool=None):
        D, H, W = dims
        st = L.stream_ptr()
        slope = self.slope if slope is None else float(slope)
        self._pack(ly, True, cfg[6])
        v = self._variant(cfg[6])
        if mask_img is not None:
            if v.masked is None or cb or rows is not None:
                raise L.BfmError("a masked launch is a one-source Winograd kernel without moment rows")
            nws = v.masked_workspace(D, H, W, self.passes)
            mws = torch.empty(nws, dtype=torch.uint8, device=self.device)
            L.check(v.masked(L.ptr(A), ca, D, H, W, L.ptr(scale), L.ptr(shift), L.ptr(bound), groups, L.ptr(ly.wpacked),
                             ly.wexp, ly.cout, slope, self.passes, cfg[7] & 1, L.ptr(out), L.ptr(mask_img), L.ptr(mws), nws,
                             st), "conv_wino(masked) " + ly.name)
            return
        if pool is not None:
            if cfg[6] != 3 or cb or mask_img is not None:
                raise L.BfmError("the fused pooling is the one-source F(2,3) kernel's")
            pooled, prow = pool
            if uni_flags is not None:
                scratch = torch.empty(self.lib.bfm_conv3x3x3_wino_uniform_scratch(ly.cout), dtype=torch.uint8,
                                      device=self.device)
                L.check(self.lib.bfm_conv3x3x3_wino_uniform_pool(
                    L.ptr(A), ca, D, H, W, L.ptr(scale), L.ptr(shift), L.ptr(bound), groups, L.ptr(ly.wpacked), ly.wexp,
                    ly.cout, slope, self.passes, cfg[7] & 1, L.ptr(out), L.ptr(rows[0]) if rows is not None else None,
                    L.ptr(uni_flags), L.ptr(scratch), L.ptr(pooled), L.ptr(prow[0]) if prow is not None else None, st),
                        "conv_wino(uniform, pool) " + ly.name)
            else:
                L.check(self.lib.bfm_conv3x3x3_wino_pool(
                    L.ptr(A), ca, D, H, W, L.ptr(scale), L.ptr(shift), L.ptr(bound), groups, L.ptr(ly.wpacked), ly.wexp,
                    ly.cout, slope, self.passes, cfg[7] & 1, L.ptr(out), L.ptr(rows[0]) if rows is not None else None,
                    L.ptr(pooled), L.ptr(prow[0]) if prow is not None else None, st), "conv_wino(pool) " + ly.name)
            return
        if uni_flags is not None and cfg[6] == 4 and not self._same_boxes(dims):
            uni_flags = None
        if uni_flags is not None and v.uniform is not None and not cb:
            scratch = torch.empty(v.uniform_scratch(ly.cout), dtype=torch.uint8, device=self.device)
            L.check(v.uniform(L.ptr(A), ca, D, H, W, L.ptr(scale), L.ptr(shift), L.ptr(bound), groups, L.ptr(ly.wpacked),
                              ly.wexp, ly.cout, slope, self.passes, cfg[7] & 1, L.ptr(out),
                              L.ptr(rows[0]) if rows is not None else None, L.ptr(uni_flags), L.ptr(scratch), st),
                    "conv_wino(uniform) " + ly.name)
            return
        if v.dense is not None:
            if cb:
                raise L.BfmError("the Winograd variant takes one source" if cfg[6] == 3 else
                                 "the Winograd variants take one source")
            L.check(v.dense(L.ptr(A), ca, D, H, W, L.ptr(scale), L.ptr(shift), L.ptr(bound), groups, L.ptr(ly.wpacked),
                            ly.wexp, ly.cout, slope, self.passes, cfg[7] & 1, L.ptr(out),
                            L.ptr(rows[0]) if rows is not None else None, st), "conv_%s %s" % (v.layout, ly.name))
            return
        L.check(self.lib.bfm_conv3x3x3_mfma_ex(L.ptr(A), ca, L.ptr(B) if cb else None, cb, D, H, W, upp if cb else None,
                                               L.ptr(scale), L.ptr(shift), L.ptr(bound), groups, L.ptr(ly.wpacked),
                                               ly.wexp, ly.cout, slope, self.passes, cfg, L.ptr(out), L.ptr(ws),
                                               ws.numel(), L.ptr(rows[0]) if rows is not None else None, st),
                "conv_mfma " + ly.name)

    def _needs_f23(self, ly):
        if self._f23_ids is None:
            self._f23_ids = {id(self.enc[i][j]) for i, j in ((0, 1), (1, 0), (1, 1)) if i < len(self.enc)}
        return id(ly) in self._f23_ids

    def _same_boxes(self, dims):
        if self._same_box_cache is None:
            self._same_box_cache = {}
        cache, key = self._same_box_cache, tuple(dims)
        if key not in cache:
            b3, b4 = (C.c_int * 3)(), (C.c_int * 3)()
            ok = (self._variant(3).box(dims[0], dims[1], dims[2], self.passes, b3) == 0 and
                  self._variant(4).box(dims[0], dims[1], dims[2], self.passes, b4) == 0)
            cache[key] = ok and list(b3) == list(b4)
        return cache[key]

    def _f23_cfg(self, ly, cfg):
        if cfg[6] == 4 and ((self.tape is not None and not TRAIN_F43) or self._needs_f23(ly)):
            cfg = (C.c_int * 8)(*list(cfg))
            cfg[6] = 3
        return cfg

    def _rows_for(self, cin, cout, dims, cfg, S=1):
        v = self._variant(cfg[6])
        if v.rows is not None:
            return self._rows_buf(cout, S, v.rows, dims[0], dims[1], dims[2], self.passes)
        return self._rows_buf(cout, S, self.lib.bfm_conv3x3x3_mfma_rows, cin, cout, dims[0], dims[1], dims[2], cfg)

    def _rows_buf(self, cout, S, rows_fn, *args):
        if not self.fuse_stats:
            return None
        n = rows_fn(*args)
        if n <= 0:
            return None
        return (torch.empty(self.lib.bfm_moment_rows_bytes(S * n, cout), dtype=torch.uint8, device=self.device), n)

    @staticmethod
    def _tag(ly):
        return ly.name.replace("backbone.", "").replace(".basic_module.SingleConv", ".")

    def _bracket(self, launch, record):
        if self.prof is None:
            launch()
            return
        reps = max(1, int(self.prof_reps))
        ev = (torch.cuda.Event(enable_timing=True), torch.cuda.Event(enable_timing=True))
        ev[0].record()
        for _ in range(reps):
            launch()
        ev[1].record()
        flops, nbytes, tag, cin, cout, dims, cfg = record()
        self.prof.append((ev[0], ev[1], flops, nbytes, reps, (tag, cin, cout, tuple(dims), tuple(cfg))))

    def single_conv(self, ly, A, dims, B=None, lo_dims=None, mask_img=None, uni_flags=None, pool=False):
        D, H, W = dims
        ca = A.shape[-1]
        cb = 0 if B is None else B.shape[-1]
        assert ca + cb == ly.cin, (ly.name, ca, cb, ly.cin)
        st = L.stream_ptr()
        up = self._upsample_desc(lo_dims, dims) if B is not None else None
        upp = C.byref(up) if up is not None else None
        scale = torch.empty(ly.cin, dtype=torch.float32, device=self.device)
        shift = torch.empty(ly.cin, dtype=torch.float32, device=self.device)
        bound = torch.empty(ly.groups, dtype=torch.float32, device=self.device)
        mfma = self._mfma_ok(ly, ca, cb)
        if (mfma and B is not None and self.use_upfold and tuple(dims) == tuple(2 * v for v in lo_dims)
                and lo_dims[0] * lo_dims[1] * lo_dims[2] >= self.upfold_min):
            return self._single_conv_upfold(ly, A, dims, B, lo_dims, upp, scale, shift, bound, uni_flags=uni_flags)
        cfg = None
        wsc = 0
        if mfma:
            cfg = self._plan(ly.cin, ly.cout, dims, B is not None)
            wsc = self.lib.bfm_conv3x3x3_mfma_workspace(ly.cin, ly.cout, D, H, W, cfg[5])
        ws = self._gn_stats(ly, A, ca, B, cb, dims, lo_dims, upp, scale, shift, bound, wsc)
        out = torch.empty((D, H, W, ly.cout), dtype=torch.float32, device=self.device)
        if mfma:
            def _launch(c):
                self._conv_launch(ly, A, ca, B, cb, dims, upp, scale, shift, bound, ly.groups, c, out, ws)
            cfg = self._f23_cfg(ly, self._autotune(ly, (ly.cin, ly.cout, tuple(dims), B is not None, False), _launch))
        self._pack(ly, mfma, cfg[6] if cfg is not None else 0)
        if mfma:
            if mask_img is not None and not (cfg[6] in (3, 4) and B is None and self.tape is None):
                mask_img = None
            if uni_flags is not None and not (cfg[6] in (3, 4) and B is None and mask_img is None):
                uni_flags = None
            rows = self._rows_for(ly.cin, ly.cout, dims, cfg) if mask_img is None else None
            pl = None
            if (pool and cfg[6] == 3 and B is None and mask_img is None and self.tape is None and self.fuse_pool
                    and min(dims) >= 2 and self.lib.bfm_conv3x3x3_wino_pool_ok(D, H, W, self.passes)):
                pooled = torch.empty((D // 2, H // 2, W // 2, ly.cout), dtype=torch.float32, device=self.device)
                pl = (pooled, self._rows_buf(ly.cout, 1, self.lib.bfm_conv3x3x3_wino_rows, D, H, W, self.passes))

            def _record():
                nv = D * H * W
                if mask_img is not None:
                    nv = self.masked_voxels(mask_img, dims, cfg[6])
                if uni_flags is not None:
                    nv = self.uniform_voxels(uni_flags, dims)
                lo = 0 if B is None else lo_dims[0] * lo_dims[1] * lo_dims[2]
                return (2.0 * 27 * ly.cin * ly.cout * nv, 4.0 * (nv * ca + lo * cb + nv * ly.cout + 27 * ly.cin * ly.cout),
                        self._tag(ly) + ("[masked]" if mask_img is not None else "[uniform]" if uni_flags is not None else ""),
                        ly.cin, ly.cout, dims, cfg)
            self._bracket(lambda: self._conv_launch(ly, A, ca, B, cb, dims, upp, scale, shift, bound, ly.groups, cfg, out, ws,
                                                    rows, mask_img=mask_img, uni_flags=uni_flags, pool=pl), _record)
            if rows is not None:
                out._bfm_rows = rows
            if pl is not None:
                if pl[1] is not None:
                    pl[0]._bfm_rows = pl[1]
                out._bfm_pooled = (pl[0], (D // 2, H // 2, W // 2))
        elif ca == 1 and cb == 0 and ly.cout in (32, 64) and not self.force_direct:
            rows = self._rows_buf(ly.cout, 1, self.lib.bfm_conv3x3x3_stem_rows, D, H, W)
            L.check(self.lib.bfm_conv3x3x3_stem_ex(L.ptr(A), D, H, W, L.ptr(scale), L.ptr(shift), L.ptr(bound),
                                                   L.ptr(ly.wpacked), ly.cout, self.slope, L.ptr(out),
                                                   L.ptr(rows[0]) if rows is not None else None, st),
                    "conv_stem " + ly.name)
            if rows is not None:
                out._bfm_rows = rows
        elif ca in (2, 3, 4) and cb == 0 and ly.cout in (32, 64) and not self.force_direct and self.stem_mc:
            rows = self._rows_buf(ly.cout, 1, self.lib.bfm_conv3x3x3_stem_rows, D, H, W)
            L.check(self.lib.bfm_conv3x3x3_stem_mc_ex(L.ptr(A), ca, D, H, W, L.ptr(scale), L.ptr(shift), L.ptr(bound),
                                                      L.ptr(ly.wpacked), ly.cout, self.slope, L.ptr(out),
                                                      L.ptr(rows[0]) if rows is not None else None, st),
                    "conv_stem_mc " + ly.name)
            ly.kind = "stem_mc"
            if rows is not None:
                out._bfm_rows = rows
        else:
            L.check(self.lib.bfm_conv3x3x3_direct(L.ptr(A), ca, L.ptr(B), cb, D, H, W, upp, L.ptr(scale),
                                                  L.ptr(shift), L.ptr(ly.wpacked), ly.cout, self.slope, L.ptr(out),
                                                  st), "conv_direct " + ly.name)
        self._record(ly, A, B, dims, lo_dims, scale, shift, bound, out)
        return out

    def masked_voxels(self, mask_img, dims, ver=None):
        D, H, W = dims
        if ver is None:
            ly = self.dec[-1][-1] if self.dec else self.enc[0][-1]
            key = (ly.cin, ly.cout, tuple(dims), False, False)
            ver = _TUNE_CHOICES.get((torch.cuda.current_device(), getattr(self, "passes", None), key))
            if ver is None:
                ver = _tune_lookup(torch.cuda.current_device(), getattr(self, "passes", None), key)
            if os.environ.get("BFM_CONV_VER"):
                ver = int(os.environ["BFM_CONV_VER"])
        box = (C.c_int * 3)()
        L.check(self._variant(4 if ver == 4 else 3).box(D, H, W, self.passes, box), "wino_box")
        td, th, tw = box[0], box[1], box[2]
        m = (mask_img.reshape(D, H, W) != 0)
        m = torch.nn.functional.pad(m, (0, -W % tw, 0, -H % th, 0, -D % td))
        m = m.reshape(m.shape[0] // td, td, m.shape[1] // th, th, m.shape[2] // tw, tw)
        act = m.any(dim=5, keepdim=True).any(dim=3, keepdim=True).any(dim=1, keepdim=True).expand_as(m)
        act = act.reshape(m.shape[0] * td, m.shape[2] * th, m.shape[4] * tw)[:D, :H, :W]
        n = int(act.sum().item())
        self.last_mask_fraction = n / float(D * H * W)
        return n

    def uniform_flags(self, x_cl, dims, radius, level=0):
        if not self.uniform_skip or x_cl is None or x_cl.shape[-1] != 1 or self.tape is not None:
            return None
        radius = max([radius] + [r for k, r in self.UNIFORM_RADIUS.items() if k[1] == level])
        ckey = (x_cl.data_ptr(), tuple(dims), int(level), int(radius), torch.cuda.current_stream(self.device).cuda_stream)
        if self._uf_cache is None:
            self._uf_cache = {}
        cache = self._uf_cache
        if ckey in cache:
            return cache[ckey]
        D, H, W = dims
        lv = sorted({k[1] for k in self.UNIFORM_RADIUS})
        rad = [max(r for k, r in self.UNIFORM_RADIUS.items() if k[1] == l) for l in lv]
        if level in lv and radius == rad[lv.index(level)]:
            nb = [self.lib.bfm_uniform_boxes_bytes(D >> l, H >> l, W >> l, self.passes) for l in lv]
            if min(nb) > 0:
                bufs = [torch.empty(n, dtype=torch.uint8, device=self.device) for n in nb]
                rc = self.lib.bfm_uniform_boxes_levels(L.ptr(x_cl), D, H, W, len(lv), (C.c_int * len(lv))(*lv),
                                                       (C.c_int * len(lv))(*rad), self.passes,
                                                       (C.c_void_p * len(lv))(*[b.data_ptr() for b in bufs]),
                                                       L.ptr(self._uf_ticket()), L.stream_ptr())
                if rc != -2:
                    L.check(rc, "uniform_boxes_levels")
                    for l, r, b in zip(lv, rad, bufs):
                        cache[ckey[:2] + (int(l), int(r)) + ckey[4:]] = b
                    return cache[ckey]
        n = self.lib.bfm_uniform_boxes_bytes(D >> level, H >> level, W >> level, self.passes)
        if n <= 0:
            return None
        flags = torch.empty(n, dtype=torch.uint8, device=self.device)
        rc = self.lib.bfm_uniform_boxes_level(L.ptr(x_cl), D, H, W, int(level), int(radius), self.passes, L.ptr(flags),
                                              L.stream_ptr())
        if rc == -2:
            flags = None
        else:
            L.check(rc, "uniform_boxes")
        cache[ckey] = flags
        return flags

    UNIFORM_RADIUS = {("enc", 0, 1): 2, ("dec", 0): 3}
    if os.environ.get("BFM_UNIFORM_LEVELS", "1") != "0":
        UNIFORM_RADIUS.update({("enc", 1, 0): 4, ("enc", 1, 1): 6, ("dec", 1): 8})

    def uniform_voxels(self, flags, dims):
        nb = self.lib.bfm_conv3x3x3_wino_rows(dims[0], dims[1], dims[2], self.passes)
        f = flags[:nb]
        k = int((f != 0).sum().item())
        reused = k - int(torch.unique(f[f != 0]).numel())
        self.last_uniform_fraction = k / float(nb)
        return int(round(dims[0] * dims[1] * dims[2] * (1.0 - max(reused, 0) / float(nb))))

    def _skip_layer(self, ly, ca):
        if ly.skip is None:
            sk = _Layer()
            sk.name, sk.cin, sk.cout, sk.groups = ly.name + "[skip]", ca, ly.cout, ly.groups
            sk.gamma, sk.beta = ly.gamma, ly.beta
            sk.w_raw = ly.w_raw[:, :ca].contiguous()
            sk.kind, sk.wpacked, sk.wexp, sk.packs, sk.skip = None, None, 0, {}, None
            ly.skip = sk
        return ly.skip

    def _single_conv_upfold(self, ly, A, dims, B, lo_dims, upp, scale, shift, bound, uni_flags=None):
        D, H, W = dims
        ca, cb = A.shape[-1], B.shape[-1]
        st = L.stream_ptr()
        sk = self._skip_layer(ly, ca)
        key = (ca, ly.cout, tuple(dims), False, True)
        cfg0 = self._plan(ca, ly.cout, dims, False, True)
        cfg0[7] = 1
        wsc = self.lib.bfm_conv3x3x3_mfma_workspace(ca, ly.cout, D, H, W, cfg0[5])
        wsu = self.lib.bfm_conv3x3x3_upfold_workspace(cb, lo_dims[0], lo_dims[1], lo_dims[2], ly.cout)
        ws = self._gn_stats(ly, A, ca, B, cb, dims, lo_dims, upp, scale, shift, bound, max(wsc, wsu))
        out = torch.empty((D, H, W, ly.cout), dtype=torch.float32, device=self.device)
        if "upfold" not in ly.packs:
            self._make_upfold_pack(ly, ca, cb)
        ly.touch("upfold")
        wup, wexp_up = ly.packs["upfold"]

        def _launch_skip(c):
            self._conv_launch(sk, A, ca, None, 0, dims, None, scale, shift, bound, ly.groups, c, out, ws)
        cfg = self._f23_cfg(ly, self._autotune(sk, key, _launch_skip))
        self._pack(sk, True, cfg[6])
        sc_b, sh_b = scale[ca:], shift[ca:]
        nv = D * H * W
        lo = lo_dims[0] * lo_dims[1] * lo_dims[2]

        def _launch_up():
            L.check(self.lib.bfm_conv3x3x3_upfold_ex(L.ptr(B), cb, lo_dims[0], lo_dims[1], lo_dims[2], L.ptr(sc_b),
                                                     L.ptr(sh_b), L.ptr(bound), ly.groups, L.ptr(wup), wexp_up, ly.cout,
                                                     self.passes, L.ptr(out), L.ptr(ws) if wsu else None, ws.numel(), st),
                    "conv_upfold " + ly.name)
        self._bracket(_launch_up, lambda: (2.0 * 27 * cb * ly.cout * nv, 4.0 * (lo * cb + nv * ly.cout),
                                           self._tag(ly) + "up", cb, ly.cout, dims, (0,) * 8))
        rows = self._rows_for(ca, ly.cout, dims, cfg)
        if uni_flags is not None and (cfg[6] not in (3, 4) or (cfg[6] == 4 and not self._same_boxes(dims))):
            uni_flags = None
        self._bracket(lambda: self._conv_launch(sk, A, ca, None, 0, dims, None, scale, shift, bound, ly.groups, cfg, out, ws,
                                                rows, uni_flags=uni_flags),
                      lambda: (2.0 * 27 * ca * ly.cout * (nv if uni_flags is None else self.uniform_voxels(uni_flags, dims)),
                               4.0 * (nv * ca + 2 * nv * ly.cout),
                               self._tag(ly) + ("sk[uniform]" if uni_flags is not None else "sk"), ca, ly.cout, dims, cfg))
        if rows is not None:
            out._bfm_rows = rows
        self._record(ly, A, B, dims, lo_dims, scale, shift, bound, out)
        return out

    def maxpool(self, X, dims, out=None):
        D, H, W = dims
        c = X.shape[-1]
        fused = getattr(X, "_bfm_pooled", None)
        if fused is not None and out is None and self.tape is None:
            return fused
        if out is None:
            out = torch.empty((D // 2, H // 2, W // 2, c), dtype=torch.float32, device=self.device)
        rows = self._rows_buf(c, 1, self.lib.bfm_maxpool2_rows, c, D, H, W)
        L.check(self.lib.bfm_maxpool2_ex(L.ptr(X), c, D, H, W, L.ptr(out), L.ptr(rows[0]) if rows is not None else None,
                                         L.stream_ptr()), "maxpool2")
        if rows is not None:
            out._bfm_rows = rows
        if self.tape is not None:
            self.tape.append(dict(pool_in=X, pool_dims=tuple(dims)))
        return out, (D // 2, H // 2, W // 2)

    def maxpool_batch(self, X, dims):
        S, (D, H, W), c = X.shape[0], dims, X.shape[-1]
        out = torch.empty((S, D // 2, H // 2, W // 2, c), dtype=torch.float32, device=self.device)
        if c % 4 or self.tape is not None:
            for s_ in range(S):
                self.maxpool(X[s_], dims, out=out[s_])
            return out
        rows = self._rows_buf(c, S, self.lib.bfm_maxpool2_batch_rows, c, D, H, W)
        L.check(self.lib.bfm_maxpool2_batch(L.ptr(X), c, S, D, H, W, L.ptr(out), L.ptr(rows[0]) if rows is not None else None,
                                            L.stream_ptr()), "maxpool2_batch")
        if rows is not None:
            out._bfm_rows = rows
        return out

    deep_from = int(os.environ.get("BFM_DEEP_FROM", "3"))
    deep_batch = os.environ.get("BFM_DEEP_BATCH", "1") != "0"
    DEEP_VERS = (0, 2)
    DEEP_VERS_1SRC = (0, 2, 4)
    use_wino_b5 = os.environ.get("BFM_WINO_B5", "1")
    deep_upfold = os.environ.get("BFM_DEEP_UPFOLD", "1") != "0"
    deep_upfold_min = int(os.environ.get("BFM_DEEP_UPFOLD_MIN", "100"))
    use_tap = os.environ.get("BFM_TAP", "1") != "0"
    tap_max = 64
    mask_skip = os.environ.get("BFM_MASK_SKIP", "1") != "0"
    uniform_skip = os.environ.get("BFM_UNIFORM_SKIP", "1") != "0"

    deep_vox = int(os.environ.get("BFM_DEEP_VOX", "16000"))

    def _region_ok(self, df):
        if self._deep_ok is None:
            self._deep_ok = {}
        cache = self._deep_ok
        if df not in cache:
            ndeep = len(self.enc) - 1 - df
            layers = [ly for pair in self.enc[df:] + self.dec[:ndeep] for ly in pair]
            cache[df] = all(ly.cin % 16 == 0 and ly.cout % 64 == 0 for ly in layers) and \
                self.enc[df - 1][1].cout % 16 == 0
        return cache[df]

    def has_deep_region(self):
        if not (self.deep_batch and self.tape is None and not self.force_direct and len(self.fm) > self.deep_from >= 1):
            return False
        return self._region_ok(self.deep_from)

    def region_start(self, dims):
        df = self.deep_from
        while df - 1 >= 2:
            lv = [v >> (df - 1) for v in dims]
            if min(lv) < 1 or lv[0] * lv[1] * lv[2] > self.deep_vox or not self._region_ok(df - 1):
                break
            df -= 1
        return df

    def _batch_stats(self, ly, A, ca, B, cb, S, dims, lo_dims, upp, scale, shift, bound):
        D, H, W = dims
        st = L.stream_ptr()
        ra = getattr(A, "_bfm_rows", None) if self.fuse_stats else None
        rb = getattr(B, "_bfm_rows", None) if (self.fuse_stats and B is not None) else None
        exact2 = B is None or tuple(dims) == tuple(2 * v for v in lo_dims)
        if ra is not None and ra[1] <= 128 and (B is None or (rb is not None and exact2 and rb[1] <= 128)):
            L.check(self.lib.bfm_gn_stats_rows_batch(L.ptr(ra[0]), ra[1], ca, L.ptr(rb[0]) if rb is not None else None,
                                                     rb[1] if rb is not None else 0, cb, 8.0, D * H * W, S,
                                                     L.ptr(ly.gamma), L.ptr(ly.beta), ly.groups, self.eps, L.ptr(scale),
                                                     L.ptr(shift), L.ptr(bound), st), "gn_stats_rows_batch " + ly.name)
            return
        need = self.lib.bfm_gn_stats_batch_workspace(ca, cb, S, D, H, W, upp)
        ws = self._workspace(need)
        L.check(self.lib.bfm_gn_stats_batch(L.ptr(A), ca, L.ptr(B), cb, S, D, H, W, upp, L.ptr(ly.gamma), L.ptr(ly.beta),
                                            ly.groups, self.eps, L.ptr(scale), L.ptr(shift), L.ptr(bound), L.ptr(ws),
                                            ws.numel(), st), "gn_stats_batch " + ly.name)

    def batch_conv(self, ly, A, dims, B=None, lo_dims=None, stats=None):
        S = A.shape[0]
        D, H, W = dims
        ca = A.shape[-1]
        cb = 0 if B is None else B.shape[-1]
        assert ca + cb == ly.cin, (ly.name, ca, cb, ly.cin)
        if not self._mfma_ok(ly, ca, cb):
            raise L.BfmError("%s: the batched levels need channel counts that are multiples of 16 / 64" % ly.name)
        up = self._upsample_desc(lo_dims, dims) if B is not None else None
        upp = C.byref(up) if up is not None else None
        if stats is None:
            scale = torch.empty((S, ly.cin), dtype=torch.float32, device=self.device)
            shift = torch.empty((S, ly.cin), dtype=torch.float32, device=self.device)
            bound = torch.empty((S, ly.groups), dtype=torch.float32, device=self.device)
            self._batch_stats(ly, A, ca, B, cb, S, dims, lo_dims, upp, scale, shift, bound)
        else:
            scale, shift, bound = stats
        if self.use_tap and (lo_dims[0] * lo_dims[1] * lo_dims[2] if B is not None else D * H * W) <= self.tap_max:
            return self._batch_conv_tap(ly, A, dims, B, lo_dims, scale, shift, bound)
        if (B is not None and self.use_upfold and self.deep_upfold and tuple(dims) == tuple(2 * v for v in lo_dims)
                and lo_dims[0] * lo_dims[1] * lo_dims[2] >= self.deep_upfold_min):
            return self._batch_conv_upfold(ly, A, dims, B, lo_dims, scale, shift, bound)
        key = (ly.cin, ly.cout, tuple(dims), B is not None, False, 1)
        vers = self.DEEP_VERS if B is not None else self.DEEP_VERS_1SRC
        cfg = self._batch_plan(key, vers)
        out = torch.empty((S, D, H, W, ly.cout), dtype=torch.float32, device=self.device)
        if key not in self._tuned:
            cfg = self._autotune(ly, key, lambda c: self._batch_launch(ly, c, A[0:1], B[0:1] if B is not None else None, upp, dims,
                                                                       scale[0:1], shift[0:1], bound[0:1], out[0:1]),
                                 vers=vers)
        if B is None:
            cfg = self._deep_b5(ly, key, cfg, A, dims, scale, shift, bound)
        self._pack(ly, True, cfg[6])
        rows = self._rows_for(ly.cin, ly.cout, dims, cfg, S)
        nv = D * H * W
        lo = 0 if B is None else lo_dims[0] * lo_dims[1] * lo_dims[2]
        self._bracket(lambda: self._batch_launch(ly, cfg, A, B, upp, dims, scale, shift, bound, out, rows),
# ... 143 lines not shown
                                               L.ptr(rows[0]) if rows is not None else None, st),
                    "tap_sum_batch " + ly.name)
        self._bracket(_launch_tap, lambda: (2.0 * 27 * cx * ly.cout * nv * S,
                                            4.0 * (S * (n_lo * cx + nv * ly.cout) + 27 * cx * ly.cout),
                                            self._tag(ly) + "x%dtap" % S, cx, ly.cout, dims, (0,) * 8))
        if B is not None:
            sk = self._skip_layer(ly, ca)
            sc_a, sh_a = scale[:, :ca], shift[:, :ca]
            key = (ca, ly.cout, tuple(dims), False, True, 1, "tap")
            cfg = self._batch_plan(key, (0,))
            self._pack(sk, True, 0)
            rows = self._rows_for(ca, ly.cout, dims, cfg, S)
            self._bracket(lambda: self._batch_launch(sk, cfg, A, None, None, dims, sc_a, sh_a, bound, out, rows, aff),
                          lambda: (2.0 * 27 * ca * ly.cout * nv * S, 4.0 * S * (nv * ca + 2 * nv * ly.cout),
                                   self._tag(ly) + "x%dsk" % S, ca, ly.cout, dims, cfg))
        if rows is not None:
            out._bfm_rows = rows
        return out

    def deep_region(self, tops, df=None):
        S = len(tops)
        df = self.deep_from if df is None else df
        dims0 = tuple(tops[0][1])
        assert all(tuple(d) == dims0 for _, d in tops)
        c0 = tops[0][0].shape[-1]
        d = tuple(v // 2 for v in dims0)
        if min(dims0) < 2:
            raise L.BfmError("volume too small for %d pooling levels" % (len(self.enc) - 1))
        l1, l2 = self.enc[df]
        P = torch.empty((S,) + d + (c0,), dtype=torch.float32, device=self.device)
        scale = torch.empty((S, l1.cin), dtype=torch.float32, device=self.device)
        shift = torch.empty((S, l1.cin), dtype=torch.float32, device=self.device)
        bound = torch.empty((S, l1.groups), dtype=torch.float32, device=self.device)
        for s_, (x, dd) in enumerate(tops):
            ps, _ = self.maxpool(x, dd, out=P[s_])
            self._gn_stats(l1, ps, c0, None, 0, d, None, None, scale[s_], shift[s_], bound[s_], 0)
        x = self.batch_conv(l1, P, d, stats=(scale, shift, bound))
        x = self.batch_conv(l2, x, d)
        skips = [(x, d)]
        for i in range(df + 1, len(self.enc)):
            l1, l2 = self.enc[i]
            if min(d) < 2:
                raise L.BfmError("volume too small for %d pooling levels" % (len(self.enc) - 1))
            d2 = tuple(v // 2 for v in d)
            P = self.maxpool_batch(x, d)
            d = d2
            x = self.batch_conv(l1, P, d)
            x = self.batch_conv(l2, x, d)
            skips.insert(0, (x, d))
        feats = [(x, d)]
        skips = skips[1:]
        ndeep = len(self.enc) - 1 - df
        for (l1, l2), (skip, sd_) in zip(self.dec[:ndeep], skips):
            y = self.batch_conv(l1, skip, sd_, B=x, lo_dims=d)
            x = self.batch_conv(l2, y, sd_)
            d = sd_
            feats.append((x, d))
        return x, d, feats

    def backbone_cl(self, x_cl, dims, mask_last=False):
        if self.has_deep_region():
            return self.backbone_batch([x_cl], dims, mask_last=mask_last)[0]
        self._uf_cache = {}
        mask_last = mask_last and not self.dense_last
        mask_img = x_cl if (mask_last and self.mask_skip and x_cl.shape[-1] == 1) else None
        skips = self.encoder_top(x_cl, dims, len(self.enc))
        x, d = skips.pop()
        return [(x, d)] + self.decoder_top(skips, x, d, mask_img=mask_img, df=len(self.enc) - 1, image=x_cl)

    def _layer_flags(self, key, image, dims):
        if key not in self.UNIFORM_RADIUS:
            return None
        return self.uniform_flags(image, dims, self.UNIFORM_RADIUS[key], key[1])

    def encoder_top(self, x_cl, dims, df=None):
        skips = []
        x, d = x_cl, tuple(dims)
        nlev = self.deep_from if df is None else df
        for i, (l1, l2) in enumerate(self.enc[:nlev]):
            if i > 0:
                if min(d) < 2:
                    raise L.BfmError("volume %s too small for %d pooling levels" % (dims, len(self.enc) - 1))
                x, d = self.maxpool(x, d)
            x = self.single_conv(l1, x, d, uni_flags=self._layer_flags(("enc", i, 0), x_cl, dims))
            x = self.single_conv(l2, x, d, uni_flags=self._layer_flags(("enc", i, 1), x_cl, dims),
                                 pool=i + 1 < nlev)
            skips.append((x, d))
        return skips

    def decoder_top(self, skips, x, d, mask_img=None, df=None, image=None):
        ndeep = len(self.enc) - 1 - (self.deep_from if df is None else df)
        feats = []
        nd = len(self.dec) - ndeep
        for k, ((l1, l2), (skip, sd_)) in enumerate(zip(self.dec[ndeep:], reversed(skips))):
            lvl = nd - 1 - k
            uf = self._layer_flags(("dec", lvl), image, tuple(image.shape[:3])) if image is not None else None
            y = self.single_conv(l1, skip, sd_, B=x, lo_dims=d, uni_flags=uf)
            x = self.single_conv(l2, y, sd_, mask_img=mask_img if k == nd - 1 else None)
            d = sd_
            feats.append((x, d))
        return feats

    def backbone_batch(self, xs, dims, mask_last=False):
        self._uf_cache = {}
        mask_last = mask_last and not self.dense_last
        df = self.region_start(dims)
        tops = [self.encoder_top(x, dims, df) for x in xs]
        out, d, deep_feats = self.deep_region([t[-1] for t in tops], df)
        res = []
        for s_, skips in enumerate(tops):
            feats = [(f[s_], fd) for f, fd in deep_feats]
            mask_img = xs[s_] if (mask_last and self.mask_skip and xs[s_].shape[-1] == 1) else None
            o_s = out[s_]
            rws = getattr(out, "_bfm_rows", None)
            if rws is not None:
                o_s._bfm_rows = (rws[0], rws[1], len(tops) * rws[1], s_ * rws[1])
            feats += self.decoder_top(skips, o_s, d, mask_img=mask_img, df=df, image=xs[s_])
            res.append(feats)
        return res

    @staticmethod
    def as_ncdhw(buf):
        return buf.permute(3, 0, 1, 2).unsqueeze(0)

    def to_cl(self, x):
        if x.dim() != 5 or x.shape[0] != 1:
            raise L.BfmError("expected a (1,C,D,H,W) tensor, got %s" % (tuple(x.shape),))
        x = x.to(device=self.device, dtype=torch.float32)
        return x[0].permute(1, 2, 3, 0).contiguous()

    def head_layers(self, widths):
        key = tuple(int(w) for w in widths)
        if self._head_layers is None or self._head_layers[0] != key:
            layers = []
            for i in range(len(key) - 1):
                name = "head.layers.%d.main" % i
                hl = _HeadLayer()
                hl.name, hl.cin, hl.cout, hl.groups = name, key[i], key[i + 1], 1
                if hl.cin % 4 or hl.cout % 4:
                    raise L.BfmError("task_f_maps %s: the hidden head layers take widths that are multiples of 4" % (list(key),))
                hl.gamma = hl.beta = None
                hl.w_raw = self._dev(self.sd[name + ".weight"])
                hl.bias = self._dev(self.sd[name + ".bias"])
                if tuple(hl.w_raw.shape) != (hl.cout, hl.cin, 3, 3, 3) or tuple(hl.bias.shape) != (hl.cout,):
                    raise L.BfmError("%s has shapes %s / %s, expected %s / %s" % (name, tuple(hl.w_raw.shape), tuple(hl.bias.shape),
                                                                                 (hl.cout, hl.cin, 3, 3, 3), (hl.cout,)))
                hl.kind, hl.wpacked, hl.wexp, hl.packs, hl.skip = None, None, 0, {}, None
                layers.append(hl)
            self._head_layers = (key, layers)
        return self._head_layers[1]

    def _head_cfg(self, hl, dims):
        key = ("head", hl.cin, hl.cout, tuple(dims))
        if key not in self._plan_cache:
            cfg = (C.c_int * 8)()
            L.check(self.lib.bfm_conv3x3x3_mfma_plan(hl.cin, hl.cout, dims[0], dims[1], dims[2], cfg), "mfma_plan")
            box = (C.c_int * 3)()
            f43 = (dims[0] >= 8 and dims[1] >= 8 and dims[2] >= 4
                   and self.lib.bfm_conv3x3x3_wino4_box(dims[0], dims[1], dims[2], self.passes, box) == 0
                   and list(box) == [8, 8, 4]
                   and self.lib.bfm_pack_conv_weights_wino4_bytes(hl.cin, hl.cout, self.passes) > 0)
            cfg[6], cfg[7] = (4 if f43 else 0), 0
            self._plan_cache[key] = cfg
        return self._plan_cache[key]

    def unit_bound(self):
        if self._unit_bound is None:
            self._unit_bound = torch.ones(1, dtype=torch.float32, device=self.device)
        return self._unit_bound

    def absmax(self, x):
        out = torch.zeros(1, dtype=torch.float32, device=self.device)
        L.check(self.lib.bfm_absmax_f32(L.ptr(x), 1, x.numel(), x.numel(), L.ptr(out), L.stream_ptr()), "absmax")
        return out

    def normalize(self, feat_cl, dims):
        D, H, W = dims
        c = feat_cl.shape[-1]
        if c > 64 or c % 8:
            raise L.BfmError("unit_feat needs c_feat <= 64 and a multiple of 8 (got %d)" % c)
        if self._no_heads is None:
# ... 195 lines not shown
```

include/brainfm_hip.h:

```cpp
#ifndef BRAINFM_HIP_H
#define BRAINFM_HIP_H

#include <stddef.h>
#include <stdint.h>

#ifdef __cplusplus
extern "C" {
#endif

typedef void* bfm_stream_t;

#define BFM_OK 0
#define BFM_E_ARG (-1)
#define BFM_E_SHAPE (-2)
#define BFM_E_WORKSPACE (-3)
#define BFM_E_LAUNCH (-4)

typedef struct {
    int d, h, w;
    const int32_t* mapD; const int32_t* mapH; const int32_t* mapW;
    const int32_t* repD; const int32_t* repH; const int32_t* repW;
} bfm_upsample_t;

const char* bfm_version(void);

size_t bfm_gn_stats_workspace(int CA, int CB, int D, int H, int W, const bfm_upsample_t* up);
#define BFM_GN_ROUTE_ROWS_VEC4 0
#define BFM_GN_ROUTE_ROWS_SCALAR 1
#define BFM_GN_ROUTE_WIDE_VEC4 2
#define BFM_GN_ROUTE_WIDE_SCALAR 3
int bfm_gn_stats_plan(int C, int64_t nvox, int aligned, int* route, int* nblocks, int64_t* vox_per_block,
                      int* rows_in_flight);
int bfm_gn_stats(const float* A, int CA, const float* B, int CB, int D, int H, int W,
                 const bfm_upsample_t* up, const float* gamma, const float* beta, int G, float eps,
                 float* scale, float* shift, float* bound, void* workspace, size_t workspace_bytes,
                 bfm_stream_t stream);
int bfm_gn_stats_train(const float* A, int CA, const float* B, int CB, int D, int H, int W, const bfm_upsample_t* up,
                       const float* gamma, const float* beta, int G, float eps, float* scale, float* shift,
                       float* bound, float* mean_out, float* rstd_out, void* workspace, size_t workspace_bytes,
                       bfm_stream_t stream);

int bfm_pack_conv_weights_direct(const float* w_oidhw, int Cin, int Cout, float* wpacked, bfm_stream_t stream);
size_t bfm_pack_conv_weights_mfma_bytes(int Cin, int Cout);
int bfm_pack_conv_weights_mfma(const float* w_oidhw, int Cin, int Cout, float wmax_abs_host, void* wpacked,
                               int* wexp_host, bfm_stream_t stream);

size_t bfm_pack_conv_weights_mfma16_bytes(int Cin, int Cout);
int bfm_pack_conv_weights_mfma16(const float* w_oidhw, int Cin, int Cout, float wmax_abs_host, void* wpacked,
                                 int* wexp_host, bfm_stream_t stream);

int bfm_conv3x3x3_direct(const float* A, int CA, const float* B, int CB, int D, int H, int W,
                         const bfm_upsample_t* up, const float* scale, const float* shift,
                         const float* wpacked, int Cout, float slope, float* out, bfm_stream_t stream);


size_t bfm_pack_conv_weights_wino_bytes(int Cin, int Cout, int passes);
int bfm_pack_conv_weights_wino(const float* w_oidhw, int Cin, int Cout, float wmax_abs_host, int passes, void* wpacked,
                               int* wexp_host, bfm_stream_t stream);
int bfm_conv3x3x3_wino_rows(int D, int H, int W, int passes);
int bfm_conv3x3x3_wino_ex(const float* A, int CA, int D, int H, int W, const float* scale, const float* shift,
                          const float* bound, int G, const void* wpacked, int wexp, int Cout, float slope, int passes,
                          int flags, float* out, void* moment_rows , bfm_stream_t stream);

size_t bfm_uniform_boxes_bytes(int D, int H, int W, int passes);
int bfm_uniform_boxes(const float* image, int D, int H, int W, int radius, int passes, unsigned char* flags,
                      bfm_stream_t stream);
int bfm_uniform_boxes_level(const float* image, int D, int H, int W, int level, int radius, int passes, unsigned char* flags,
                            bfm_stream_t stream);
int bfm_uniform_boxes_levels(const float* image, int D, int H, int W, int nlevels, const int* levels, const int* radii,
                             int passes, unsigned char* const* flags, int* ticket, bfm_stream_t stream);
size_t bfm_conv3x3x3_wino_uniform_scratch(int Cout);
int bfm_conv3x3x3_wino_uniform(const float* A, int CA, int D, int H, int W, const float* scale, const float* shift,
                               const float* bound, int G, const void* wpacked, int wexp, int Cout, float slope, int passes,
                               int flags, float* out, void* moment_rows, const unsigned char* uniform_flags, void* scratch,
                               bfm_stream_t stream);
int bfm_conv3x3x3_wino_pool_ok(int D, int H, int W, int passes);
int bfm_conv3x3x3_wino_pool(const float* A, int CA, int D, int H, int W, const float* scale, const float* shift,
                            const float* bound, int G, const void* wpacked, int wexp, int Cout, float slope, int passes,
                            int flags, float* out, void* moment_rows, float* pooled, void* pooled_rows ,
                            bfm_stream_t stream);
int bfm_conv3x3x3_wino_uniform_pool(const float* A, int CA, int D, int H, int W, const float* scale, const float* shift,
                                    const float* bound, int G, const void* wpacked, int wexp, int Cout, float slope,
                                    int passes, int flags, float* out, void* moment_rows,
                                    const unsigned char* uniform_flags, void* scratch, float* pooled,
                                    void* pooled_rows , bfm_stream_t stream);
int bfm_conv3x3x3_wino_box(int D, int H, int W, int passes, int* box );
size_t bfm_conv3x3x3_wino_masked_workspace(int D, int H, int W, int passes);
int bfm_conv3x3x3_wino_masked(const float* A, int CA, int D, int H, int W, const float* scale, const float* shift,
                              const float* bound, int G, const void* wpacked, int wexp, int Cout, float slope, int passes,
                              int flags, float* out, const float* mask_image, void* workspace, size_t workspace_bytes,
                              bfm_stream_t stream);

size_t bfm_moment_rows_bytes(int nrows, int C);
int bfm_conv3x3x3_mfma_rows(int Cin, int Cout, int D, int H, int W, const int* cfg);
int bfm_conv3x3x3_mfma_ex(const float* A, int CA, const float* B, int CB, int D, int H, int W,
                          const bfm_upsample_t* up, const float* scale, const float* shift, const float* bound,
                          int G, const void* wpacked, int wexp, int Cout, float slope, int passes, const int* cfg,
                          float* out, void* workspace, size_t workspace_bytes, void* moment_rows ,
                          bfm_stream_t stream);
size_t bfm_conv3x3x3_mfma_batch_workspace(int Cin, int Cout, int S, int D, int H, int W, int splitk);
int bfm_conv3x3x3_mfma_batch(const float* A, int CA, const float* B, int CB, int S, int D, int H, int W,
                             const bfm_upsample_t* up, const float* scale, const float* shift, const float* bound, int G,
                             const void* wpacked, int wexp, int Cout, float slope, int passes, const int* cfg, float* out,
                             void* workspace, size_t workspace_bytes, void* moment_rows, int affine_stride,
                             bfm_stream_t stream);
size_t bfm_gn_stats_batch_workspace(int CA, int CB, int S, int D, int H, int W, const bfm_upsample_t* up);
int bfm_gn_stats_batch(const float* A, int CA, const float* B, int CB, int S, int D, int H, int W,
                       const bfm_upsample_t* up, const float* gamma, const float* beta, int G, float eps, float* scale,
                       float* shift, float* bound, void* workspace, size_t workspace_bytes, bfm_stream_t stream);
int bfm_gn_stats_rows_batch(const void* rowsA, int nrowsA_per_sample, int CA, const void* rowsB, int nrowsB_per_sample,
                            int CB, double weightB, int64_t nvox, int S, const float* gamma, const float* beta, int G,
                            float eps, float* scale, float* shift, float* bound, bfm_stream_t stream);

int bfm_maxpool2_rows(int C, int D, int H, int W);
int bfm_maxpool2_ex(const float* in, int C, int D, int H, int W, float* out, void* moment_rows ,
                    bfm_stream_t stream);
int bfm_maxpool2_batch_rows(int C, int D, int H, int W);
int bfm_maxpool2_batch(const float* in, int C, int S, int D, int H, int W, float* out, void* moment_rows ,
                       bfm_stream_t stream);
int bfm_conv3x3x3_stem_rows(int D, int H, int W);
int bfm_conv3x3x3_stem_ex(const float* A, int D, int H, int W, const float* scale, const float* shift,
                          const float* bound, const float* wpacked_direct, int Cout, float slope, float* out,
                          void* moment_rows , bfm_stream_t stream);
int bfm_conv3x3x3_stem_mc_ex(const float* A, int Cin, int D, int H, int W, const float* scale, const float* shift,
                             const float* bound, const float* wpacked_direct, int Cout, float slope, float* out,
                             void* moment_rows , bfm_stream_t stream);
size_t bfm_gn_stats_rows_workspace(int nrowsA, int CA, int nrowsB, int CB);
#define BFM_GN_TICKETS 16
#define BFM_GN_ROWS_DIRECT 0
#define BFM_GN_ROWS_FOLD 1
#define BFM_GN_ROWS_ONE_LAUNCH 2
int bfm_gn_stats_rows_route(int nrowsA, int CA, int nrowsB, int CB, int G, int has_ticket);
int bfm_gn_stats_rows(const void* rowsA, int nrowsA, int CA, const void* rowsB, int nrowsB, int CB, double weightB,
                      int64_t nvox, const float* gamma, const float* beta, int G, float eps, float* scale,
                      float* shift, float* bound, void* workspace, size_t workspace_bytes, void* ticket,
                      bfm_stream_t stream);
int bfm_gn_stats_rows_train(const void* rowsA, int nrowsA, int CA, const void* rowsB, int nrowsB, int CB, double weightB,
                            int64_t nvox, const float* gamma, const float* beta, int G, float eps, float* scale,
                            float* shift, float* bound, float* mean_out, float* rstd_out, void* workspace,
                            size_t workspace_bytes, void* ticket, bfm_stream_t stream);

int bfm_gn_stats_rows_sliced(const void* rowsA, int totalA, int firstA, int nrowsA, int CA, const void* rowsB, int totalB,
                             int firstB, int nrowsB, int CB, double weightB, int64_t nvox, const float* gamma,
                             const float* beta, int G, float eps, float* scale, float* shift, float* bound,
                             void* workspace, size_t workspace_bytes, void* ticket, bfm_stream_t stream);

size_t bfm_pack_conv_weights_wino4_bytes(int Cin, int Cout, int passes);
int bfm_pack_conv_weights_wino4(const float* w_oidhw, int Cin, int Cout, float wmax_abs_host, int passes, void* wpacked,
                                int* wexp_host, bfm_stream_t stream);
int bfm_conv3x3x3_wino4_rows(int D, int H, int W, int passes);
int bfm_conv3x3x3_wino4_box(int D, int H, int W, int passes, int* box );
int bfm_conv3x3x3_wino4(const float* A, int CA, int D, int H, int W, const float* scale, const float* shift,
                        const float* bound, int G, const void* wpacked, int wexp, int Cout, float slope, int passes,
                        int flags, float* out, void* moment_rows , bfm_stream_t stream);
int bfm_conv3x3x3_wino4_batch(const float* A, int CA, int S, int D, int H, int W, const float* scale, const float* shift,
                              const float* bound, int G, const void* wpacked, int wexp, int Cout, float slope, int passes,
                              int flags, float* out, void* moment_rows, int affine_stride, bfm_stream_t stream);
int bfm_conv3x3x3_wino_b5_rows(int D, int H, int W, int passes);
int bfm_conv3x3x3_wino_b5_splitk(int Cin, int Cout, int D, int H, int W);
size_t bfm_conv3x3x3_wino_b5_workspace(int Cin, int Cout, int S, int D, int H, int W);
int bfm_conv3x3x3_wino_b5_batch(const float* A, int CA, int S, int D, int H, int W, const float* scale, const float* shift,
                                const float* bound, int G, const void* wpacked, int wexp, int Cout, float slope, int passes,
                                int flags, float* out, void* moment_rows, int affine_stride, void* workspace,
                                size_t workspace_bytes, bfm_stream_t stream);
size_t bfm_conv3x3x3_wino4_masked_workspace(int D, int H, int W, int passes);
size_t bfm_conv3x3x3_wino4_uniform_scratch(int Cout);
int bfm_conv3x3x3_wino4_uniform(const float* A, int CA, int D, int H, int W, const float* scale, const float* shift,
                                const float* bound, int G, const void* wpacked, int wexp, int Cout, float slope, int passes,
                                int flags, float* out, void* moment_rows, const unsigned char* uniform_flags, void* scratch,
                                bfm_stream_t stream);
int bfm_conv3x3x3_wino4_masked(const float* A, int CA, int D, int H, int W, const float* scale, const float* shift,
                               const float* bound, int G, const void* wpacked, int wexp, int Cout, float slope, int passes,
                               int flags, float* out, const float* mask_image, void* workspace, size_t workspace_bytes,
                               bfm_stream_t stream);

size_t bfm_conv3x3x3_mfma_workspace(int Cin, int Cout, int D, int H, int W, int splitk);
int bfm_conv3x3x3_mfma_plan(int Cin, int Cout, int D, int H, int W, int* cfg_out );

size_t bfm_pack_conv_weights_upfold_bytes(int CB, int Cout, int passes);
int bfm_pack_conv_weights_upfold(const float* w_oidhw , int CA, int CB, int Cout,
                                 float wmax_abs_host, int passes, void* wpacked, int* wexp_host, bfm_stream_t stream);
int bfm_conv3x3x3_upfold(const float* B, int CB, int d, int h, int w, const float* scale_b, const float* shift_b,
                         const float* bound, int G, const void* wpacked, int wexp, int Cout, int passes, float* out,
                         bfm_stream_t stream);
size_t bfm_conv3x3x3_upfold_workspace(int CB, int d, int h, int w, int Cout);
int bfm_conv3x3x3_upfold_ex(const float* B, int CB, int d, int h, int w, const float* scale_b, const float* shift_b,
                            const float* bound, int G, const void* wpacked, int wexp, int Cout, int passes, float* out,
                            void* workspace, size_t workspace_bytes, bfm_stream_t stream);
size_t bfm_conv3x3x3_upfold_batch_workspace(int CB, int S, int d, int h, int w, int Cout);
int bfm_conv3x3x3_upfold_batch(const float* B, int CB, int S, int d, int h, int w, const float* scale_b,
                               const float* shift_b, const float* bound, int G, const void* wpacked, int wexp, int Cout,
                               int passes, float* out, void* workspace, size_t workspace_bytes, int affine_stride,
                               bfm_stream_t stream);

size_t bfm_conv3x3x3_tap_batch_workspace(int Cin, int Cout, int S, int n_lo);
int bfm_conv3x3x3_tap_batch(const float* X, int Cin, int S, int n_lo, const float* scale, const float* shift,
                            const float* bound, int G, const void* wpacked, int wexp, int Cout, int kc_first, int kc_pack,
                            int passes, void* workspace, size_t workspace_bytes, int affine_stride, bfm_stream_t stream);
int bfm_tap_sum_rows(int n_hi, int Cout);
int bfm_tap_sum_batch(const void* workspace, int Cin, int Cout, int S, int n_lo, const int* table ,
                      int n_hi, float slope, int activation, int accumulate, float* out, void* moment_rows ,
                      bfm_stream_t stream);

int bfm_conv3x3x3_mfma(const float* A, int CA, const float* B, int CB, int D, int H, int W,
                       const bfm_upsample_t* up, const float* scale, const float* shift, const float* bound,
                       int G, const void* wpacked, int wexp, int Cout, float slope, int passes,
                       const int* cfg , float* out, void* workspace,
                       size_t workspace_bytes, bfm_stream_t stream);

int bfm_maxpool2(const float* in, int C, int D, int H, int W, float* out, bfm_stream_t stream);

enum {
    BFM_ROLE_PLAIN = 0,
    BFM_ROLE_CT = 1,
    BFM_ROLE_BIAS_LOG = 2,
    BFM_ROLE_SEG = 3,
    BFM_ROLE_DIST = 4,
    BFM_ROLE_SR = 5,
    BFM_ROLE_PATHOL = 6
};
typedef struct {
    int n_out;
    int c_feat;
    const float* head_w;
    const float* head_b;
    const int32_t* roles;
    const int32_t* out_slot;
    int seg_first, n_seg;
    const int32_t* seg_lut;
    int n_dist;
    int dist_first;
    float max_dist;
    int unit_feat;
    int slot_high_res;
    int slot_fake_cortical;
    int n_maps;
    float head_wmax;
    int skip_zero_input;
} bfm_tail_desc_t;

int bfm_tail_heads(const float* feat, const float* input , int64_t nvox,
                   const bfm_tail_desc_t* desc, float* feat_norm ,
                   float* const* maps ,
                   float* seg_prob , int64_t* label ,
                   float* raw_out ,
                   bfm_stream_t stream);
int bfm_tail_heads_rows(const float* feat, const float* input , int64_t nvox,
                        const bfm_tail_desc_t* desc, float* feat_norm , float* maps_rows, int64_t row_stride,
                        float* seg_prob , int64_t* label , int flags, bfm_stream_t stream);
int bfm_tail_route(const bfm_tail_desc_t* desc);

int bfm_stitch_accumulate(const float* tile, const int64_t* tile_label, const float* tile_input,
                          int td, int th, int tw, float* full, int D, int H, int W,
// ... 436 lines not shown
```

Baseline: 213.5 million voxels/s.

## Skip writing uniform-tile conv outputs that no downstream reader needs

```diff
diff --git a/brainfm_amd/_lib.py b/brainfm_amd/_lib.py
--- a/brainfm_amd/_lib.py
+++ b/brainfm_amd/_lib.py
@@ -151,6 +151,7 @@
     "bfm_conv3x3x3_wino4_masked_workspace": (_Z, [_I, _I, _I, _I]),
     "bfm_conv3x3x3_wino4_uniform_scratch": (_Z, [_I]),
     "bfm_conv3x3x3_wino4_uniform": (_I, [_P, _I, _I, _I, _I, _P, _P, _P, _I, _P, _I, _I, _F, _I, _I, _P, _P, _P, _P, _P]),
+    "bfm_conv3x3x3_wino4_uniform_keep": (_I, [_P, _I, _I, _I, _I, _P, _P, _P, _I, _P, _I, _I, _F, _I, _I, _P, _P, _P, _P, _P, _P]),
     "bfm_conv3x3x3_wino4": (_I, [_P, _I, _I, _I, _I, _P, _P, _P, _I, _P, _I, _I, _F, _I, _I, _P, _P, _P]),
     "bfm_conv3x3x3_wino4_batch": (_I, [_P, _I, _I, _I, _I, _I, _P, _P, _P, _I, _P, _I, _I, _F, _I, _I, _P, _P, _I, _P]),
     "bfm_conv3x3x3_wino_b5_rows": (_I, [_I, _I, _I, _I]),
@@ -173,6 +174,7 @@
     "bfm_uniform_boxes_level": (_I, [_P, _I, _I, _I, _I, _I, _I, _P, _P]),
     "bfm_uniform_boxes_levels": (_I, [_P, _I, _I, _I, _I, C.POINTER(_I), C.POINTER(_I), _I, C.POINTER(_P), _P, _P]),
     "bfm_uniform_boxes_bytes": (_Z, [_I, _I, _I, _I]),
+    "bfm_uniform_fill": (_I, [_P, _I, _I, _I, _I, _I, _P, _P]),
     "bfm_conv3x3x3_wino_uniform_scratch": (_Z, [_I]),
     "bfm_conv3x3x3_wino_uniform": (_I, [_P, _I, _I, _I, _I, _P, _P, _P, _I, _P, _I, _I, _F, _I, _I, _P, _P, _P, _P, _P]),
     "bfm_conv3x3x3_wino_pool_ok": (_I, [_I, _I, _I, _I]),
diff --git a/brainfm_amd/csrc/conv3d_wino.hip b/brainfm_amd/csrc/conv3d_wino.hip
--- a/brainfm_amd/csrc/conv3d_wino.hip
+++ b/brainfm_amd/csrc/conv3d_wino.hip
@@ -505,6 +505,7 @@
     const int* first;
     const int* list;
     const int* list_n;
+    const unsigned char* need;
     double *rsum, *rsq;
     float *rmn, *rmx;
     float* pool_out;
@@ -521,7 +522,7 @@
     const int z0 = (mt / (p.nTx * p.nTy)) * p.TD, y0 = ((mt / p.nTx) % p.nTy) * p.TH, x0 = (mt % p.nTx) * p.TW;
     const int rz0 = (rp / (p.nTx * p.nTy)) * p.TD, ry0 = ((rp / p.nTx) % p.nTy) * p.TH, rx0 = (rp % p.nTx) * p.TW;
     const int c4 = tid & 15;
-    {
+    if (p.need == nullptr || p.need[mt] != 0) {
         const size_t dbase = (((size_t)z0 * p.H + y0) * p.W + x0) * p.Cout + nt * 64 + c4 * 4;
         const size_t sbase = (((size_t)rz0 * p.H + ry0) * p.W + rx0) * p.Cout + nt * 64 + c4 * 4;
         for (int r = 0; r < 4; ++r) {
@@ -639,15 +640,20 @@
     }
 }
 
+constexpr int UL_COMP_WORDS = 4096;
 template <bool AGENT>
-__device__ __forceinline__ void uniform_lists_body(const unsigned char* flags, int n, int* __restrict__ first,
-                                                   int* __restrict__ cnt, int* __restrict__ rest, int* __restrict__ uni,
-                                                   int* sh, int* fst) {
+__device__ __forceinline__ void uniform_lists_body(const unsigned char* flags, int n, int nTz, int nTy, int nTx,
+                                                   int* __restrict__ first, int* __restrict__ cnt, int* __restrict__ rest,
+                                                   int* __restrict__ uni, int* __restrict__ ncnt, int* __restrict__ nlist,
+                                                   unsigned char* __restrict__ need, int* sh, int* fst, unsigned* comp) {
     auto flag = [&](int i) -> int {
         if constexpr (AGENT) return __hip_atomic_load(flags + i, __ATOMIC_RELAXED, __HIP_MEMORY_SCOPE_AGENT);
         else return flags[i];
     };
+    const bool table = n <= UL_COMP_WORDS * 32;
     if (threadIdx.x < 27) fst[threadIdx.x] = n;
+    if (table)
+        for (int i = threadIdx.x; i < (n + 31) / 32; i += 1024) comp[i] = 0u;
     __syncthreads();
     for (int i = threadIdx.x; i < n; i += 1024) {
         const int f = flag(i);
@@ -655,19 +661,49 @@
     }
     __syncthreads();
     if (threadIdx.x < 27) first[threadIdx.x] = fst[threadIdx.x];
-    const int n0 = wino_compact(n, [&](int mt) { const int f = flag(mt); return f == 0 || fst[f - 1] == mt; }, rest, sh);
+    const int n0 = wino_compact(n, [&](int mt) {
+        const int f = flag(mt);
+        const bool c = f == 0 || fst[f - 1] == mt;
+        if (c && table) atomicOr(&comp[mt >> 5], 1u << (mt & 31));
+        return c;
+    }, rest, sh);
     if (threadIdx.x == 0) cnt[0] = n0;
     __syncthreads();
-    const int n1 = wino_compact(n, [&](int mt) { const int f = flag(mt); return f != 0 && fst[f - 1] != mt; }, uni, sh);
+    auto computed = [&](int i) -> bool {
+        if (table) return ((comp[i >> 5] >> (i & 31)) & 1u) != 0u;
+        const int f = flag(i);
+        return f == 0 || fst[f - 1] == i;
+    };
+    const int n1 = wino_compact(n, [&](int mt) { return !computed(mt); }, uni, sh);
     if (threadIdx.x == 0) cnt[1] = n1;
-}
-
-__global__ void __launch_bounds__(1024) uniform_lists_kernel(const unsigned char* __restrict__ flags, int n,
-                                                             int* __restrict__ first, int* __restrict__ cnt,
-                                                             int* __restrict__ rest, int* __restrict__ uni) {
+    __syncthreads();
+    const int n2 = wino_compact(n, [&](int mt) {
+        bool nd = false;
+        if (!computed(mt)) {
+            const int tx = mt % nTx, ty = (mt / nTx) % nTy, tz = mt / (nTx * nTy);
+            for (int dz = -1; dz <= 1; ++dz)
+                for (int dy = -1; dy <= 1; ++dy)
+                    for (int dx = -1; dx <= 1; ++dx) {
+                        const int z = tz + dz, y = ty + dy, x = tx + dx;
+                        if (z >= 0 && z < nTz && y >= 0 && y < nTy && x >= 0 && x < nTx)
+                            nd = nd || computed((z * nTy + y) * nTx + x);
+                    }
+        }
+        need[mt] = nd ? 1 : 0;
+        return nd;
+    }, nlist, sh);
+    if (threadIdx.x == 0) ncnt[0] = n2;
+}
+
+__global__ void __launch_bounds__(1024) uniform_lists_kernel(const unsigned char* __restrict__ flags, int n, int nTz, int nTy,
+                                                             int nTx, int* __restrict__ first, int* __restrict__ cnt,
+                                                             int* __restrict__ rest, int* __restrict__ uni,
+                                                             int* __restrict__ ncnt, int* __restrict__ nlist,
+                                                             unsigned char* __restrict__ need) {
     __shared__ int sh[17];
     __shared__ int fst[27];
-    uniform_lists_body<false>(flags, n, first, cnt, rest, uni, sh, fst);
+    __shared__ unsigned comp[UL_COMP_WORDS];
+    uniform_lists_body<false>(flags, n, nTz, nTy, nTx, first, cnt, rest, uni, ncnt, nlist, need, sh, fst, comp);
 }
 
 constexpr int UL_MAX = 4;
@@ -690,6 +726,7 @@
     __shared__ int fst[27];
     __shared__ int bad_w[16];
     __shared__ int is_last;
+    __shared__ unsigned comp[UL_COMP_WORDS];
     const int tid = threadIdx.x, grp = tid >> 8, t = tid & 255;
     int li = 0;
     for (int i = 1; i < p.nlev; ++i)
@@ -758,8 +795,9 @@
     __builtin_amdgcn_fence(__ATOMIC_ACQUIRE, "agent");
     for (int i = 0; i < p.nlev; ++i) {
         const int n = p.lv[i].n;
-        int* const first = p.lv[i].first;
-        uniform_lists_body<true>(p.lv[i].flags, n, first, first + 27, first + 29, first + 29 + n, sh, fst);
+        const UniformFlagBuf fb{p.lv[i].flags, (size_t)n};
+        uniform_lists_body<true>(fb.flags, n, p.lv[i].nTz, p.lv[i].nTy, p.lv[i].nTx, fb.first(), fb.counts(), fb.rest_list(),
+                                 fb.uniform_list(), fb.need_count(), fb.need_list(), fb.need(), sh, fst, comp);
         __syncthreads();
     }
 }
@@ -936,8 +974,8 @@
     if ((TD << level) < radius || (TH << level) < radius || (TW << level) < radius) return BFM_E_SHAPE;
     hipLaunchKernelGGL(uniform_boxes_kernel, dim3((unsigned)fb.n), dim3(256), 0, bfm_s(stream), image, D, H, W, TD, TH, TW, nTz,
                        nTy, nTx, level, radius, flags);
-    hipLaunchKernelGGL(uniform_lists_kernel, dim3(1), dim3(1024), 0, bfm_s(stream), flags, (int)fb.n, fb.first(), fb.counts(),
-                       fb.rest_list(), fb.uniform_list());
+    hipLaunchKernelGGL(uniform_lists_kernel, dim3(1), dim3(1024), 0, bfm_s(stream), flags, (int)fb.n, nTz, nTy, nTx, fb.first(),
+                       fb.counts(), fb.rest_list(), fb.uniform_list(), fb.need_count(), fb.need_list(), fb.need());
     return bfm_launch_status();
 }
 
@@ -1062,6 +1100,7 @@
             f.TD = p.TD; f.TH = p.TH; f.TW = p.TW; f.nTy = p.nTy; f.nTx = p.nTx;
             f.tw_shift = ilog2i(p.TW); f.thw_shift = ilog2i(p.TH * p.TW);
             f.flags = fb.flags; f.first = fb.first(); f.list = p.list; f.list_n = p.list_n;
+            f.need = (a.flags & 2) ? fb.need() : nullptr;
             f.rsum = p.rsum; f.rsq = p.rsq; f.rmn = p.rmn; f.rmx = p.rmx;
             f.pool_out = p.pool_out; f.prsum = p.prsum; f.prsq = p.prsq; f.prmn = p.prmn; f.prmx = p.prmx;
             hipLaunchKernelGGL(class_fill, grid, block, 0, st, f);
@@ -1073,6 +1112,23 @@
     }
     if (a.pool.out) bfm_launch_by_passes(passes, conv_wino_pool<3>, conv_wino_pool<1>, grid, block, smem, st, p);
     else bfm_launch_by_passes(passes, conv_wino<3>, conv_wino<1>, grid, block, smem, st, p);
+    return bfm_launch_status();
+}
+
+extern "C" int bfm_uniform_fill(float* out, int D, int H, int W, int Cout, int passes, const unsigned char* uniform_flags,
+                                bfm_stream_t stream) {
+    if (!out || !uniform_flags || D <= 0 || H <= 0 || W <= 0 || Cout <= 0 || Cout % 64) return BFM_E_ARG;
+    if ((reinterpret_cast<uintptr_t>(out) & 15) || (reinterpret_cast<uintptr_t>(uniform_flags) & 3)) return BFM_E_ARG;
+    FillParams f{};
+    if (!choose_box(D, H, W, passes == 3 ? 2 : 1, f.TD, f.TH, f.TW)) return BFM_E_SHAPE;
+    f.out = out; f.D = D; f.H = H; f.W = W; f.Cout = Cout; f.NT = Cout / 64;
+    f.nTy = bfm_cdiv(H, f.TH); f.nTx = bfm_cdiv(W, f.TW);
+    f.tw_shift = ilog2i(f.TW); f.thw_shift = ilog2i(f.TH * f.TW);
+    const int64_t nMt = (int64_t)bfm_cdiv(D, f.TD) * f.nTy * f.nTx;
+    if (nMt * f.NT > 0x7fffffff) return BFM_E_SHAPE;
+    const UniformFlagBuf fb{uniform_flags, (size_t)nMt};
+    f.flags = fb.flags; f.first = fb.first(); f.list = fb.uniform_list(); f.list_n = fb.counts() + 1;
+    hipLaunchKernelGGL(class_fill, dim3((unsigned)(nMt * f.NT)), dim3(NTHR), 0, bfm_s(stream), f);
     return bfm_launch_status();
 }
 
@@ -1097,7 +1153,7 @@
                                           const float* shift, const float* bound, int G, const void* wpacked, int wexp,
                                           int Cout, float slope, int passes, int flags, float* out, void* moment_rows,
                                           const unsigned char* uniform_flags, void* scratch, bfm_stream_t stream) {
-    if (!uniform_flags || !scratch || (flags & ~1)) return BFM_E_ARG;
+    if (!uniform_flags || !scratch || (flags & ~3)) return BFM_E_ARG;
     if ((reinterpret_cast<uintptr_t>(uniform_flags) & 3) || (reinterpret_cast<uintptr_t>(scratch) & 15)) return BFM_E_ARG;
     WinoLaunch a{A, CA, D, H, W, scale, shift, bound, G, wpacked, wexp, Cout, slope, passes, flags, out, moment_rows, stream};
     a.uniform = {uniform_flags, static_cast<float*>(scratch)};
@@ -1109,7 +1165,7 @@
                                                int wexp, int Cout, float slope, int passes, int flags, float* out,
                                                void* moment_rows, const unsigned char* uniform_flags, void* scratch,
                                                float* pooled, void* pooled_rows, bfm_stream_t stream) {
-    if (!uniform_flags || !scratch || !pooled || (flags & ~1)) return BFM_E_ARG;
+    if (!uniform_flags || !scratch || !pooled || (flags & ~3)) return BFM_E_ARG;
     if ((reinterpret_cast<uintptr_t>(uniform_flags) & 3) || (reinterpret_cast<uintptr_t>(scratch) & 15)) return BFM_E_ARG;
     WinoLaunch a{A, CA, D, H, W, scale, shift, bound, G, wpacked, wexp, Cout, slope, passes, flags, out, moment_rows, stream};
     a.uniform = {uniform_flags, static_cast<float*>(scratch)};
diff --git a/brainfm_amd/csrc/conv3d_wino4.hip b/brainfm_amd/csrc/conv3d_wino4.hip
--- a/brainfm_amd/csrc/conv3d_wino4.hip
+++ b/brainfm_amd/csrc/conv3d_wino4.hip
@@ -34,6 +34,8 @@
     const int* list_n;
     const unsigned char* uni_flags;
     float* uni_acc;
+    const unsigned char* uni_need;
+    const float* uni_keep;
     int nMtS, saff;
     int64_t sA, sO;
     int dbg_sleep;
@@ -489,6 +491,13 @@
     const bool rep = MODE == 2 && cls != 0;
     float4* const ybuf = BY_FLAG && cls ? reinterpret_cast<float4*>(p.uni_acc) + ((size_t)(cls - 1) * p.NT + nt) * (2 * 8 * NTHR) + tid
                                         : nullptr;
+    bool store = true;
+    if constexpr (UNI) {
+        if (p.uni_need != nullptr) {
+            store = p.uni_need[mt] != 0;
+            if (!store && p.uni_keep != nullptr) store = p.uni_keep[((int64_t)z0 * p.H + y0) * p.W + x0] != 0.f;
+        }
+    }
 
     float bmax = 0.f;
     for (int g = 0; g < p.G; ++g) bmax = fmaxf(bmax, p.bound[g]);
@@ -797,7 +806,7 @@
                     float r = y[k];
                     if (p.accum) r = r + prev[it][k];
                     r = r >= 0.f ? r : r * p.slope;
-                    if constexpr ((ABL & 128) == 0) o[off_t + (unsigned)(k * p.Cout)] = r;
+                    if constexpr ((ABL & 128) == 0) { if (!UNI || store) o[off_t + (unsigned)(k * p.Cout)] = r; }
                     fs += r; fq = fmaf(r, r, fq); fmn = fminf(fmn, r); fmx = fmaxf(fmx, r);
                 }
             }
@@ -829,7 +838,7 @@
                         float r = y[k];
                         if (p.accum) r = r + o[off_t + (unsigned)(k * p.Cout)];
                         r = r >= 0.f ? r : r * p.slope;
-                        o[off_t + (unsigned)(k * p.Cout)] = r;
+                        if (!UNI || store) o[off_t + (unsigned)(k * p.Cout)] = r;
                         fs += r; fq = fmaf(r, r, fq); fmn = fminf(fmn, r); fmx = fmaxf(fmx, r);
                     }
                 }
@@ -1017,6 +1026,8 @@
         if (!bfm_wino_choose_box(D, H, W, npl, bd, bh, bw) || bd != p.TD || bh != p.TH || bw != p.TW) return BFM_E_SHAPE;
         p.uni_flags = fb.flags;
         p.uni_acc = a.uniform.scratch;
+        if (a.uniform.keep && !(a.flags & 2)) return BFM_E_ARG;
+        if ((a.flags & 3) == 3) { p.uni_need = fb.need(); p.uni_keep = a.uniform.keep; }
     }
     if (dma) {
         static bool attr = false;
@@ -1114,3 +1125,16 @@
     a.uniform = {uniform_flags, static_cast<float*>(scratch)};
     return w4_launch(a);
 }
+
+extern "C" int bfm_conv3x3x3_wino4_uniform_keep(const float* A, int CA, int D, int H, int W, const float* scale,
+                                                const float* shift, const float* bound, int G, const void* wpacked, int wexp,
+                                                int Cout, float slope, int passes, int flags, float* out, void* moment_rows,
+                                                const unsigned char* uniform_flags, void* scratch, const float* keep_image,
+                                                bfm_stream_t stream) {
+    if (!uniform_flags || !scratch || !keep_image || flags != 3 || (reinterpret_cast<uintptr_t>(uniform_flags) & 3) ||
+        (reinterpret_cast<uintptr_t>(scratch) & 15))
+        return BFM_E_ARG;
+    WinoLaunch a{A, CA, D, H, W, scale, shift, bound, G, wpacked, wexp, Cout, slope, passes, flags, out, moment_rows, stream};
+    a.uniform = {uniform_flags, static_cast<float*>(scratch), keep_image};
+    return w4_launch(a);
+}
diff --git a/brainfm_amd/csrc/wino_shared.h b/brainfm_amd/csrc/wino_shared.h
--- a/brainfm_amd/csrc/wino_shared.h
+++ b/brainfm_amd/csrc/wino_shared.h
@@ -3,7 +3,7 @@
 
 bool bfm_wino_choose_box(int D, int H, int W, int npl, int& TD, int& TH, int& TW);
 
-static inline size_t bfm_pad4(size_t n) { return (n + 3) & ~(size_t)3; }
+__host__ __device__ static inline size_t bfm_pad4(size_t n) { return (n + 3) & ~(size_t)3; }
 
 struct MaskListBuf {
     void* ws;
@@ -17,11 +17,14 @@
 struct UniformFlagBuf {
     const unsigned char* flags;
     size_t n;
-    static size_t bytes(size_t n) { return bfm_pad4(n) + 27 * 4 + 2 * 4 + 2 * n * 4; }
-    int* first() const { return reinterpret_cast<int*>(const_cast<unsigned char*>(flags) + bfm_pad4(n)); }
-    int* counts() const { return first() + 27; }
-    int* rest_list() const { return counts() + 2; }
-    int* uniform_list() const { return rest_list() + n; }
+    static size_t bytes(size_t n) { return bfm_pad4(n) + 27 * 4 + 2 * 4 + 2 * n * 4 + 4 + n * 4 + bfm_pad4(n); }
+    __host__ __device__ int* first() const { return reinterpret_cast<int*>(const_cast<unsigned char*>(flags) + bfm_pad4(n)); }
+    __host__ __device__ int* counts() const { return first() + 27; }
+    __host__ __device__ int* rest_list() const { return counts() + 2; }
+    __host__ __device__ int* uniform_list() const { return rest_list() + n; }
+    __host__ __device__ int* need_count() const { return uniform_list() + n; }
+    __host__ __device__ int* need_list() const { return need_count() + 1; }
+    __host__ __device__ unsigned char* need() const { return reinterpret_cast<unsigned char*>(need_list() + n); }
 };
 
 int bfm_wino_mask_list(const float* mask_img, int D, int H, int W, int TD, int TH, int TW, int nTy, int nTx, int nMt, void* ws,
@@ -40,13 +43,13 @@
     void* moment_rows;
     bfm_stream_t stream;
     struct { const float* img = nullptr; void* ws = nullptr; } mask;
-    struct { const unsigned char* flags = nullptr; float* scratch = nullptr; } uniform;
+    struct { const unsigned char* flags = nullptr; float* scratch = nullptr; const float* keep = nullptr; } uniform;
     struct { float* out = nullptr; void* rows = nullptr; } pool;
     struct { int S = 1, affine_stride = 0; } batch;
 };
 
 static inline int bfm_wino_check(const WinoLaunch& a, int KC) {
-    if (a.flags & ~1) return BFM_E_ARG;
+    if (a.flags & ~(a.uniform.flags ? 3 : 1)) return BFM_E_ARG;
     if (!a.A || a.CA <= 0 || a.D <= 0 || a.H <= 0 || a.W <= 0 || !a.scale || !a.shift || !a.bound || a.G <= 0 || !a.wpacked ||
         !a.out)
         return BFM_E_ARG;
diff --git a/brainfm_amd/engine.py b/brainfm_amd/engine.py
--- a/brainfm_amd/engine.py
+++ b/brainfm_amd/engine.py
@@ -407,15 +407,11 @@
 
     def _autotune(self, ly, key, launch, vers=None):
         cfg = self._plan_cache[key]
-        if key in self._tuned or os.environ.get("BFM_CONV_VER") or os.environ.get("BFM_CONV_TUNE", "1") == "0":
+        if self._variant_pinned(key):
             return cfg
         gkey = (torch.cuda.current_device(), getattr(self, "passes", None), key)
-        if gkey not in _TUNE_CHOICES:
-            saved = _tune_lookup(gkey[0], gkey[1], key)
-            if saved is not None and not (key[3] and saved in (3, 4)) and (vers is None or saved in vers):
-                _TUNE_CHOICES[gkey] = int(saved)
-        if gkey in _TUNE_CHOICES and (vers is None or _TUNE_CHOICES[gkey] in vers or (_TUNE_CHOICES[gkey] == 4 and 3 in vers)):
-            c = _TUNE_CHOICES[gkey]
+        c = self._settled_variant(key, vers)
+        if c is not None:
             if vers is None or c in vers:
                 cfg[6] = c
                 self._tuned.add(key)
@@ -460,6 +456,22 @@
         _tune_store(gkey[0], gkey[1], key, best)
         return cfg
 
+    def _variant_pinned(self, key):
+        return bool(key in self._tuned or os.environ.get("BFM_CONV_VER") or os.environ.get("BFM_CONV_TUNE", "1") == "0")
+
+    def _settled_variant(self, key, vers=None):
+        if self._variant_pinned(key):
+            return int(self._plan_cache[key][6])
+        gkey = (torch.cuda.current_device(), getattr(self, "passes", None), key)
+        if gkey not in _TUNE_CHOICES:
+            saved = _tune_lookup(gkey[0], gkey[1], key)
+            if saved is not None and not (key[3] and saved in (3, 4)) and (vers is None or saved in vers):
+                _TUNE_CHOICES[gkey] = int(saved)
+        c = _TUNE_CHOICES.get(gkey)
+        if c is not None and (vers is None or c in vers or (c == 4 and 3 in vers)):
+            return int(c)
+        return None
+
     def conv_choices(self):
         dev, ps = torch.cuda.current_device(), getattr(self, "passes", None)
         return {k[2]: v for k, v in _TUNE_CHOICES.items() if k[0] == dev and k[1] == ps}
@@ -508,6 +520,7 @@
                                                      L.ptr(self._gn_ticket()) if self.gn_one_launch else None, st),
                     "gn_stats_rows " + ly.name)
             return ws
+        self._complete(A, dims)
         wsb = self.lib.bfm_gn_stats_workspace(ca, cb, D, H, W, upp)
         ws = self._workspace(max(wsb, ws_min))
         L.check(self.lib.bfm_gn_stats_train(L.ptr(A), ca, L.ptr(B), cb, D, H, W, upp, L.ptr(ly.gamma), L.ptr(ly.beta),
@@ -522,15 +535,26 @@
                                   scale=scale, shift=shift, bound=bound, mean=mean, rstd=rstd, out=out))
 
     def _conv_launch(self, ly, A, ca, B, cb, dims, upp, scale, shift, bound, groups, cfg, out, ws, rows=None, slope=None,
-                     mask_img=None, uni_flags=None, pool=None):
+                     mask_img=None, uni_flags=None, pool=None, need=None):
         D, H, W = dims
         st = L.stream_ptr()
         slope = self.slope if slope is None else float(slope)
         self._pack(ly, True, cfg[6])
         v = self._variant(cfg[6])
+        tag = getattr(A, "_bfm_need", None)
+        if B is not None and getattr(B, "_bfm_need", None) is not None:
+            raise L.BfmError("%s: an upsampled source that was stored by need" % ly.name)
+
+        def reads(route, ok=False):
+            if tag is not None and not ok:
+                raise L.BfmError("%s: its input was stored by need for %s, and this launch (%s) would read boxes that were "
+                                 "never written" % (ly.name, "the uniform-box pair on its flags" if tag[1] is None else
+                                                    "the masked convolution", route))
+        fbit = (cfg[7] & 1) | (2 if need is not None else 0)
         if mask_img is not None:
             if v.masked is None or cb or rows is not None:
                 raise L.BfmError("a masked launch is a one-source Winograd kernel without moment rows")
+            reads("masked", tag is not None and tag[1] is mask_img and (cfg[6] == 3 or self._same_boxes(dims)))
             nws = v.masked_workspace(D, H, W, self.passes)
             mws = torch.empty(nws, dtype=torch.uint8, device=self.device)
             L.check(v.masked(L.ptr(A), ca, D, H, W, L.ptr(scale), L.ptr(shift), L.ptr(bound), groups, L.ptr(ly.wpacked),
@@ -542,28 +566,44 @@
                 raise L.BfmError("the fused pooling is the one-source F(2,3) kernel's")
             pooled, prow = pool
             if uni_flags is not None:
+                reads("uniform, pool", tag is not None and tag[1] is None and tag[0] is uni_flags)
                 scratch = torch.empty(self.lib.bfm_conv3x3x3_wino_uniform_scratch(ly.cout), dtype=torch.uint8,
                                       device=self.device)
                 L.check(self.lib.bfm_conv3x3x3_wino_uniform_pool(
                     L.ptr(A), ca, D, H, W, L.ptr(scale), L.ptr(shift), L.ptr(bound), groups, L.ptr(ly.wpacked), ly.wexp,
-                    ly.cout, slope, self.passes, cfg[7] & 1, L.ptr(out), L.ptr(rows[0]) if rows is not None else None,
+                    ly.cout, slope, self.passes, fbit, L.ptr(out), L.ptr(rows[0]) if rows is not None else None,
                     L.ptr(uni_flags), L.ptr(scratch), L.ptr(pooled), L.ptr(prow[0]) if prow is not None else None, st),
                         "conv_wino(uniform, pool) " + ly.name)
             else:
+                if need is not None:
+                    raise L.BfmError("%s: stores by need without the uniform-box pair" % ly.name)
+                reads("pool")
                 L.check(self.lib.bfm_conv3x3x3_wino_pool(
                     L.ptr(A), ca, D, H, W, L.ptr(scale), L.ptr(shift), L.ptr(bound), groups, L.ptr(ly.wpacked), ly.wexp,
                     ly.cout, slope, self.passes, cfg[7] & 1, L.ptr(out), L.ptr(rows[0]) if rows is not None else None,
                     L.ptr(pooled), L.ptr(prow[0]) if prow is not None else None, st), "conv_wino(pool) " + ly.name)
             return
-        if uni_flags is not None and cfg[6] == 4 and not self._same_boxes(dims):
+        if uni_flags is not None and not self._pair_ok(cfg[6], dims, cb):
             uni_flags = None
-        if uni_flags is not None and v.uniform is not None and not cb:
+        if uni_flags is not None and v.uniform is not None:
+            reads("uniform", tag is not None and tag[1] is None and tag[0] is uni_flags)
             scratch = torch.empty(v.uniform_scratch(ly.cout), dtype=torch.uint8, device=self.device)
+            if need is not None and need is not True:
+                if cfg[6] != 4 or fbit != 3:
+                    raise L.BfmError("stores for a masked reader are the accumulating F(4,3) pair's")
+                L.check(self.lib.bfm_conv3x3x3_wino4_uniform_keep(
+                    L.ptr(A), ca, D, H, W, L.ptr(scale), L.ptr(shift), L.ptr(bound), groups, L.ptr(ly.wpacked), ly.wexp,
+                    ly.cout, slope, self.passes, fbit, L.ptr(out), L.ptr(rows[0]) if rows is not None else None,
+                    L.ptr(uni_flags), L.ptr(scratch), L.ptr(need), st), "conv_wino4(uniform, keep) " + ly.name)
+                return
             L.check(v.uniform(L.ptr(A), ca, D, H, W, L.ptr(scale), L.ptr(shift), L.ptr(bound), groups, L.ptr(ly.wpacked),
-                              ly.wexp, ly.cout, slope, self.passes, cfg[7] & 1, L.ptr(out),
+                              ly.wexp, ly.cout, slope, self.passes, fbit, L.ptr(out),
                               L.ptr(rows[0]) if rows is not None else None, L.ptr(uni_flags), L.ptr(scratch), st),
                     "conv_wino(uniform) " + ly.name)
             return
+        if need is not None:
+            raise L.BfmError("%s: stores by need without the uniform-box pair" % ly.name)
+        reads("dense")
         if v.dense is not None:
             if cb:
                 raise L.BfmError("the Winograd variant takes one source" if cfg[6] == 3 else
@@ -594,6 +634,50 @@
             cache[key] = ok and list(b3) == list(b4)
         return cache[key]
 
+    def _pair_ok(self, ver, dims, cb=0, mask_img=None):
+        return ver in (3, 4) and not cb and mask_img is None and (ver != 4 or self._same_boxes(dims))
+
+    def _known_variant(self, ly, tune_ly, key):
+        self._plan(key[0], key[1], key[2], key[3], key[4])
+        ver = self._settled_variant(key)
+        if ver is None:
+            return None
+        cfg = (C.c_int * 8)()
+        cfg[6] = ver
+        return int(self._f23_cfg(ly, cfg)[6])
+
+    def _need_reader(self, reader, flags, dims, ca):
+        if (reader is None or flags is None or not self.uniform_need or self.tape is not None or not self.fuse_stats
+                or self.force_direct):
+            return False
+        kind, ly, arg = reader
+        if kind == "skip":
+            cb = ly.cin - ca
+            lo = tuple(v // 2 for v in dims)
+            if not (arg is flags and self._mfma_ok(ly, ca, cb) and self.use_upfold and all(v % 2 == 0 for v in dims)
+                    and lo[0] * lo[1] * lo[2] >= self.upfold_min):
+                return False
+            return self._pair_ok(self._known_variant(ly, self._skip_layer(ly, ca), (ca, ly.cout, tuple(dims), False, True)),
+                                 dims)
+        if not (ly.cin == ca and self._mfma_ok(ly, ca, 0)):
+            return False
+        ver = self._known_variant(ly, ly, (ly.cin, ly.cout, tuple(dims), False, False))
+        if kind == "conv":
+            return arg is flags and self._pair_ok(ver, dims)
+        return (arg is not None and self.mask_skip and ver in (3, 4) and (ver == 3 or self._same_boxes(dims))
+                and self._variant(ver).masked is not None)
+
+    def _complete(self, t, dims):
+        tag = getattr(t, "_bfm_need", None)
+        if tag is None:
+            return
+        if tag[1] is not None:
+            raise L.BfmError("a tensor stored by need for the masked convolution cannot be completed")
+        L.check(self.lib.bfm_uniform_fill(L.ptr(t), dims[0], dims[1], dims[2], t.shape[-1], self.passes, L.ptr(tag[0]),
+                                          L.stream_ptr()), "uniform_fill")
+        t._bfm_need = None
+        self.need_completed += 1
+
     def _f23_cfg(self, ly, cfg):
         if cfg[6] == 4 and ((self.tape is not None and not TRAIN_F43) or self._needs_f23(ly)):
             cfg = (C.c_int * 8)(*list(cfg))
@@ -631,7 +715,7 @@
         flops, nbytes, tag, cin, cout, dims, cfg = record()
         self.prof.append((ev[0], ev[1], flops, nbytes, reps, (tag, cin, cout, tuple(dims), tuple(cfg))))
 
-    def single_conv(self, ly, A, dims, B=None, lo_dims=None, mask_img=None, uni_flags=None, pool=False):
+    def single_conv(self, ly, A, dims, B=None, lo_dims=None, mask_img=None, uni_flags=None, pool=False, reader=None):
         D, H, W = dims
         ca = A.shape[-1]
         cb = 0 if B is None else B.shape[-1]
@@ -645,7 +729,8 @@
         mfma = self._mfma_ok(ly, ca, cb)
         if (mfma and B is not None and self.use_upfold and tuple(dims) == tuple(2 * v for v in lo_dims)
                 and lo_dims[0] * lo_dims[1] * lo_dims[2] >= self.upfold_min):
-            return self._single_conv_upfold(ly, A, dims, B, lo_dims, upp, scale, shift, bound, uni_flags=uni_flags)
+            return self._single_conv_upfold(ly, A, dims, B, lo_dims, upp, scale, shift, bound, uni_flags=uni_flags,
+                                            reader=reader)
         cfg = None
         wsc = 0
         if mfma:
@@ -661,7 +746,7 @@
         if mfma:
             if mask_img is not None and not (cfg[6] in (3, 4) and B is None and self.tape is None):
                 mask_img = None
-            if uni_flags is not None and not (cfg[6] in (3, 4) and B is None and mask_img is None):
+            if uni_flags is not None and not self._pair_ok(cfg[6], dims, cb, mask_img):
                 uni_flags = None
             rows = self._rows_for(ly.cin, ly.cout, dims, cfg) if mask_img is None else None
             pl = None
@@ -669,6 +754,13 @@
                     and min(dims) >= 2 and self.lib.bfm_conv3x3x3_wino_pool_ok(D, H, W, self.passes)):
                 pooled = torch.empty((D // 2, H // 2, W // 2, ly.cout), dtype=torch.float32, device=self.device)
                 pl = (pooled, self._rows_buf(ly.cout, 1, self.lib.bfm_conv3x3x3_wino_rows, D, H, W, self.passes))
+
+            need = None
+            if (uni_flags is not None and cfg[6] == 3 and rows is not None and (pl is not None or not pool)
+                    and reader is not None and reader[0] != "masked" and self._need_reader(reader, uni_flags, dims, ly.cout)):
+                need = True
+                if self.poison_skipped:
+                    out.fill_(float("nan"))
 
             def _record():
                 nv = D * H * W
@@ -681,7 +773,9 @@
                         self._tag(ly) + ("[masked]" if mask_img is not None else "[uniform]" if uni_flags is not None else ""),
                         ly.cin, ly.cout, dims, cfg)
             self._bracket(lambda: self._conv_launch(ly, A, ca, B, cb, dims, upp, scale, shift, bound, ly.groups, cfg, out, ws,
-                                                    rows, mask_img=mask_img, uni_flags=uni_flags, pool=pl), _record)
+                                                    rows, mask_img=mask_img, uni_flags=uni_flags, pool=pl, need=need), _record)
+            if need is not None:
+                out._bfm_need = (uni_flags, None)
             if rows is not None:
                 out._bfm_rows = rows
             if pl is not None:
@@ -795,7 +889,7 @@
             ly.skip = sk
         return ly.skip
 
-    def _single_conv_upfold(self, ly, A, dims, B, lo_dims, upp, scale, shift, bound, uni_flags=None):
+    def _single_conv_upfold(self, ly, A, dims, B, lo_dims, upp, scale, shift, bound, uni_flags=None, reader=None):
         D, H, W = dims
         ca, cb = A.shape[-1], B.shape[-1]
         st = L.stream_ptr()
@@ -828,13 +922,19 @@
         self._bracket(_launch_up, lambda: (2.0 * 27 * cb * ly.cout * nv, 4.0 * (lo * cb + nv * ly.cout),
                                            self._tag(ly) + "up", cb, ly.cout, dims, (0,) * 8))
         rows = self._rows_for(ca, ly.cout, dims, cfg)
-        if uni_flags is not None and (cfg[6] not in (3, 4) or (cfg[6] == 4 and not self._same_boxes(dims))):
+        if uni_flags is not None and not self._pair_ok(cfg[6], dims):
             uni_flags = None
+        need = None
+        if (uni_flags is not None and cfg[6] == 4 and rows is not None and reader is not None and reader[0] == "masked"
+                and self._need_reader(reader, uni_flags, dims, ly.cout)):
+            need = reader[2]
         self._bracket(lambda: self._conv_launch(sk, A, ca, None, 0, dims, None, scale, shift, bound, ly.groups, cfg, out, ws,
-                                                rows, uni_flags=uni_flags),
+                                                rows, uni_flags=uni_flags, need=need),
                       lambda: (2.0 * 27 * ca * ly.cout * (nv if uni_flags is None else self.uniform_voxels(uni_flags, dims)),
                                4.0 * (nv * ca + 2 * nv * ly.cout),
                                self._tag(ly) + ("sk[uniform]" if uni_flags is not None else "sk"), ca, ly.cout, dims, cfg))
+        if need is not None:
+            out._bfm_need = (uni_flags, need)
         if rows is not None:
             out._bfm_rows = rows
         self._record(ly, A, B, dims, lo_dims, scale, shift, bound, out)
@@ -848,6 +948,7 @@
             return fused
         if out is None:
             out = torch.empty((D // 2, H // 2, W // 2, c), dtype=torch.float32, device=self.device)
+        self._complete(X, dims)
         rows = self._rows_buf(c, 1, self.lib.bfm_maxpool2_rows, c, D, H, W)
         L.check(self.lib.bfm_maxpool2_ex(L.ptr(X), c, D, H, W, L.ptr(out), L.ptr(rows[0]) if rows is not None else None,
                                          L.stream_ptr()), "maxpool2")
@@ -882,6 +983,9 @@
     tap_max = 64
     mask_skip = os.environ.get("BFM_MASK_SKIP", "1") != "0"
     uniform_skip = os.environ.get("BFM_UNIFORM_SKIP", "1") != "0"
+    uniform_need = os.environ.get("BFM_UNIFORM_NEED", "1") != "0"
+    poison_skipped = os.environ.get("BFM_POISON_SKIPPED", "0") == "1"
+    need_completed = 0
 
     deep_vox = int(os.environ.get("BFM_DEEP_VOX", "16000"))
 
@@ -1191,9 +1295,12 @@
                 if min(d) < 2:
                     raise L.BfmError("volume %s too small for %d pooling levels" % (dims, len(self.enc) - 1))
                 x, d = self.maxpool(x, d)
-            x = self.single_conv(l1, x, d, uni_flags=self._layer_flags(("enc", i, 0), x_cl, dims))
-            x = self.single_conv(l2, x, d, uni_flags=self._layer_flags(("enc", i, 1), x_cl, dims),
-                                 pool=i + 1 < nlev)
+            f1, f2 = (self._layer_flags(("enc", i, j), x_cl, dims) for j in (0, 1))
+            x = self.single_conv(l1, x, d, uni_flags=f1, reader=("conv", l2, f2))
+            rd = None
+            if i + 1 < nlev and i < len(self.dec):
+                rd = ("skip", self.dec[len(self.dec) - 1 - i][0], self._layer_flags(("dec", i), x_cl, dims))
+            x = self.single_conv(l2, x, d, uni_flags=f2, pool=i + 1 < nlev, reader=rd)
             skips.append((x, d))
         return skips
 
@@ -1204,8 +1311,10 @@
         for k, ((l1, l2), (skip, sd_)) in enumerate(zip(self.dec[ndeep:], reversed(skips))):
             lvl = nd - 1 - k
             uf = self._layer_flags(("dec", lvl), image, tuple(image.shape[:3])) if image is not None else None
-            y = self.single_conv(l1, skip, sd_, B=x, lo_dims=d, uni_flags=uf)
-            x = self.single_conv(l2, y, sd_, mask_img=mask_img if k == nd - 1 else None)
+            mk = mask_img if k == nd - 1 else None
+            y = self.single_conv(l1, skip, sd_, B=x, lo_dims=d, uni_flags=uf,
+                                 reader=("masked", l2, mk) if (mk is not None and mk is image) else None)
+            x = self.single_conv(l2, y, sd_, mask_img=mk)
             d = sd_
             feats.append((x, d))
         return feats
diff --git a/include/brainfm_hip.h b/include/brainfm_hip.h
--- a/include/brainfm_hip.h
+++ b/include/brainfm_hip.h
@@ -69,6 +69,8 @@
                             bfm_stream_t stream);
 int bfm_uniform_boxes_levels(const float* image, int D, int H, int W, int nlevels, const int* levels, const int* radii,
                              int passes, unsigned char* const* flags, int* ticket, bfm_stream_t stream);
+int bfm_uniform_fill(float* out, int D, int H, int W, int Cout, int passes, const unsigned char* uniform_flags,
+                     bfm_stream_t stream);
 size_t bfm_conv3x3x3_wino_uniform_scratch(int Cout);
 int bfm_conv3x3x3_wino_uniform(const float* A, int CA, int D, int H, int W, const float* scale, const float* shift,
                                const float* bound, int G, const void* wpacked, int wexp, int Cout, float slope, int passes,
@@ -169,6 +171,10 @@
                                 const float* bound, int G, const void* wpacked, int wexp, int Cout, float slope, int passes,
                                 int flags, float* out, void* moment_rows, const unsigned char* uniform_flags, void* scratch,
                                 bfm_stream_t stream);
+int bfm_conv3x3x3_wino4_uniform_keep(const float* A, int CA, int D, int H, int W, const float* scale, const float* shift,
+                                     const float* bound, int G, const void* wpacked, int wexp, int Cout, float slope,
+                                     int passes, int flags, float* out, void* moment_rows, const unsigned char* uniform_flags,
+                                     void* scratch, const float* keep_image, bfm_stream_t stream);
 int bfm_conv3x3x3_wino4_masked(const float* A, int CA, int D, int H, int W, const float* scale, const float* shift,
                                const float* bound, int G, const void* wpacked, int wexp, int Cout, float slope, int passes,
                                int flags, float* out, const float* mask_image, void* workspace, size_t workspace_bytes,
```

Result: faster. 217.8 million voxels/s, median of 6 (+2.0%).
